# Aaron20127/human-3d-reconstruction

Hardware: AMD Instinct MI355X
Metric: images/sec whole-node, DLA-34+SMPL batch-64 512x512; top-k index bit-match (higher is better)
Workload: dtype bf16; 1 GPU; DLA-34+DCNv2 multi_pose + pose/shape heads -> sigmoid/NMS/top-100 decode -> SMPL 6890-vert LBS; 512x512, batch 64 per GPU (BASELINE configs[2]); batch_per_gpu=64, global_batch=64, K=100, smpl_people_per_image=100, parallelism=dp1 (image shards, one all-gather of dets), collective=none (one rank), steps_in_flight=3, hip_graph=False, dcn_margin=auto, images=64 distinct synthetic images (h3d_amd.synth.synth_image_batch, seed 317), weights=synthetic (h3d_amd.synth, seed 0, gain 1.25, offset_scale 0.5)

## Files before the change

human-3d-reconstruction_amd/_lib.py:

```python
import ctypes
import os

_HERE = os.path.dirname(os.path.abspath(__file__))
LIB_PATH = os.path.join(_HERE, "csrc", "libh3d_hip.so")

H3D_F32, H3D_BF16, H3D_F16, H3D_F16X3 = 0, 1, 2, 3
OP_STEM, OP_CONV, OP_DCN, OP_MAXPOOL, OP_UPADD, OP_COPY, OP_HEADS, OP_DCN_V1, OP_DCN_FUSED = 1, 2, 3, 4, 5, 6, 7, 8, 9
OP_CONV_STREAM, OP_DCN_FUSED_F16, OP_DCN_FUSED_STREAM, OP_STEM3, OP_UPDCN_F16 = 10, 11, 12, 13, 14
OP_IM2COL, OP_MAXPOOL3, OP_DEPTH2SPACE = 15, 16, 17
HEADS_MAX = 16
OUT_NHWC, OUT_NCHW_F32, OUT_NHWC_F32, OUT_NHWC_F16 = 0, 1, 2, 3
DCN_INPUT_NHWC, DCN_OUTPUT_NHWC, DCN_F32_MFMA = 1, 2, 4
ABI_VERSION = 4

DCN_AUX_BYTES = 256
DCN_FUSED_BIAS_WMAX, DCN_FUSED_BIAS_AMAX = 32, 34
OPF_DCN_MASK_FINAL, OPF_DCN_RAW_PACK, OPF_DCN_ACT_MAXIMA, TUNE_DCN_ABLATE_MASK = 0x800, 0x100000, 0x200000, 0x1f
OPF_DCN_FUSED_RAW_PACK, OPF_DCN_FUSED_SCALED_INPUT = 0x100000, 0x200000
TUNE_DCN_FUSED_X3_MARGIN2, TUNE_DCN_FUSED_X3_MARGIN6, TUNE_DCN_FUSED_X3_MARGIN4, TUNE_DCN_FUSED_X3_ABLATE_MASK = 0x2000, 0x4000, 0x8000, 0x1f
OPF_DCN_STREAM_NO_SLOTS, OPF_DCN_STREAM_WIDE_MARGIN, OPF_DCN_STREAM_SLOTS512, OPF_DCN_STREAM_F16_INPUT = 0x1000, 0x8000, 0x10000, 0x40000
OPF_DCN_STREAM_STATS, OPF_DCN_STREAM_VARIANT_MASK = 0x20000, 0x58600
TUNE_DCN_STREAM_FORCE_NARROW_WG, TUNE_DCN_STREAM_FORCE_WIDE_WG = 0x200, 0x400
TUNE_DCN_STREAM_F16_DCN5, TUNE_DCN_STREAM_F16_KEEP_DCN3, TUNE_DCN_STREAM_ABLATE_MASK = 0x4000, 0x2000, 0x1f
TUNE_DCN_STREAM_X3_MARGIN2, TUNE_DCN_STREAM_X3_MARGIN3, TUNE_DCN_STREAM_X3_MARGIN4, TUNE_DCN_STREAM_X3_ABLATE_MASK = 0x4000, 0x8000, 0x10000, 0x1f
TUNE_DCN_F16_ONE_WG_PER_CU, TUNE_DCN_F16_ABLATE_MASK = 0x100, 0xff
TUNE_CONV_STREAM_TILE_MASK, TUNE_CONV_STREAM_AUTO, TUNE_CONV_STREAM_ROUND4_RULE, TUNE_CONV_STREAM_ABLATE_MASK = 0xffff, 1, 0x10000000, 0x1f0000
TUNE_CONV_TILE, TUNE_CONV_HALO_TILE, TUNE_CONV_FORCE_GEMM, TUNE_CONV_GEMM_TILE_MASK = 0x1000, 0x2000, 0x4000, 0xf00
TUNE_CONV_X3_TILED, TUNE_CONV_X3_TILE_MASK, TUNE_CONV_X3_CK16, TUNE_CONV_X3_MT2 = 0x1000, 0x1fff, 0x2000, 0x4000
TUNE_UPADD_TAPS_GLOBAL, TUNE_UPADD_TAPS_LDS = 1, 2
TUNE_HEADS_SEPARATE_BIAS, TUNE_HEADS_ABLATE_MASK = 0x200, 0xff
TUNE_HEADS_SPARSE_LDS_PATCH, TUNE_HEADS_SPARSE_WAVES4 = 0x400, 0x800


def TUNE_DCN_STREAM_DCN5_XP(xp):
    return xp << 16


def TUNE_DCN_STREAM_DCN5_XP_OF(reserved):
    return (reserved >> 16) & 0xff


def TUNE_CONV_STREAM_TILE(variant, mt, waves):
    return variant << 12 | mt << 8 | waves


def TUNE_CONV_STREAM_ABLATE(bits):
    return bits << 16


def TUNE_CONV_STREAM_ABLATE_OF(reserved):
    return (reserved & TUNE_CONV_STREAM_ABLATE_MASK) >> 16


def TUNE_CONV_1X1_TILE(mt, th):
    return TUNE_CONV_TILE | mt << 4 | th >> 3


def TUNE_CONV_1X1_TILE_MT(reserved):
    return (reserved >> 4) & 15


def TUNE_CONV_1X1_TILE_TH(reserved):
    return (reserved & 15) * 8


def TUNE_CONV_GEMM_TILE(n):
    return n << 8


def TUNE_CONV_X3_TILE(mt, waves, th):
    return TUNE_CONV_X3_TILED | mt << 8 | waves << 4 | th >> 3

c_vp, c_i, c_fp = ctypes.c_void_p, ctypes.c_int, ctypes.c_void_p


class H3dOp(ctypes.Structure):
    _fields_ = [
        ("kind", ctypes.c_int32), ("dtype", ctypes.c_int32),
        ("in_", c_vp), ("in2", c_vp), ("w", c_vp), ("bias", c_vp), ("out", c_vp),
        ("B", ctypes.c_int32), ("H", ctypes.c_int32), ("W", ctypes.c_int32),
        ("Cin", ctypes.c_int32), ("in_cs", ctypes.c_int32), ("in2_cs", ctypes.c_int32),
        ("Ho", ctypes.c_int32), ("Wo", ctypes.c_int32),
        ("Cout", ctypes.c_int32), ("out_cs", ctypes.c_int32),
        ("ksize", ctypes.c_int32), ("stride", ctypes.c_int32), ("relu", ctypes.c_int32),
        ("out_mode", ctypes.c_int32), ("wrows", ctypes.c_int32), ("reserved", ctypes.c_int32),
        ("wexp", ctypes.c_int32), ("wexp2", ctypes.c_int32),
    ]


class _HeadEntry(ctypes.Structure):
    _fields_ = [("w2", c_vp), ("b2", c_vp), ("out", c_vp), ("C", ctypes.c_int32), ("wexp2", ctypes.c_int32)]


class H3dHeadsDesc(ctypes.Structure):
    _fields_ = [("nheads", ctypes.c_int32), ("wexp", ctypes.c_int32), ("head", _HeadEntry * HEADS_MAX)]


HEADS_LISTS_MAX = 4


class H3dHeadsList(ctypes.Structure):
    _fields_ = [("inds", c_vp), ("K", ctypes.c_int32), ("head_mask", ctypes.c_uint32)]


class H3dUpdcnDesc(ctypes.Structure):
    _fields_ = [("skip", c_vp), ("w_up", c_vp), ("w_off", c_vp), ("skip_cs", ctypes.c_int32), ("reserved", ctypes.c_int32)]


TRAIN_BRIGHTNESS, TRAIN_CONTRAST, TRAIN_SATURATION = 0, 1, 2
TRAIN_INPUT_NO_COLOR_AUG = 1


class H3dTrainImage(ctypes.Structure):
    _fields_ = [("minv", ctypes.c_double * 6), ("light", ctypes.c_double * 3), ("offset", ctypes.c_int64),
                ("h", ctypes.c_int32), ("w", ctypes.c_int32), ("row_bytes", ctypes.c_int32), ("flipped", ctypes.c_int32),
                ("order", ctypes.c_int32 * 3), ("alpha", ctypes.c_float * 3), ("one_minus_alpha", ctypes.c_float * 3),
                ("reserved", ctypes.c_int32)]


SMPL_KP_MAX_K, SMPL_KP_MAX_NV = 32, 16
RENDER_NEGATE_Z, RENDER_CULL_BACK = 1, 2
RENDER_MAX_V, RENDER_MAX_SIDE = 13120, 16384
COCO_BBOX, COCO_KEYPOINTS, COCO_ROUND2 = 0, 1, 1
COCO_MAX_D, COCO_MAX_G, COCO_SCAN_CHUNK = 128, 1024, 1024
MESH_EVAL_MAX_SWEEPS = 30
CONV_BWD_RELU, CONV_BWD_MFMA_CMAX = 1, 2048
ADAM_CAPACITY, ADAM_CHUNK = 48, 2048


class H3dAdamTensor(ctypes.Structure):
    _fields_ = [("param", c_vp), ("grad", c_vp), ("exp_avg", c_vp), ("exp_avg_sq", c_vp), ("n", ctypes.c_int64),
                ("one_minus_b1", ctypes.c_float), ("b2", ctypes.c_float), ("one_minus_b2", ctypes.c_float), ("bc2_sqrt", ctypes.c_float),
                ("eps", ctypes.c_float), ("neg_step_size", ctypes.c_float), ("weight_decay", ctypes.c_float)]


SIGNATURES = {
    "h3d_dcn_v2_forward": [c_vp] * 6 + [c_i] * 14 + [c_vp],
    "h3d_dcn_v2_forward_ws": [c_vp] * 6 + [c_i] * 14 + [c_vp, ctypes.c_size_t, c_vp],
    "h3d_dcn_v2_pack_weights": [c_vp, c_vp, c_i, c_i, c_i, c_vp, c_vp],
    "h3d_dcn_v2_pack_weights_cached": [c_vp, c_vp, c_i, c_i, c_i, c_vp, c_vp, c_vp],
    "h3d_dcn_fused_pack_f32_cached": [c_vp, c_vp, c_vp, c_vp, c_i, c_i, c_vp, c_vp, c_vp, c_vp, c_vp],
    "h3d_dcn_v2_forward_packed": [c_vp] * 5 + [c_i] * 7 + [c_vp, ctypes.c_size_t, c_vp],
    "h3d_dcn_nchw_to_nhwc_scaled": [c_vp, c_vp] + [c_i] * 4 + [c_vp, c_vp],
    "h3d_dcn_v2_backward_workspace_bytes": [c_i] * 14 + [ctypes.POINTER(ctypes.c_size_t)],
    "h3d_dcn_v2_backward": [c_vp] * 11 + [c_i] * 14 + [c_vp, ctypes.c_size_t, c_vp],
    "h3d_dcn_v2_backward_general": [c_vp] * 11 + [c_i] * 14 + [c_vp, ctypes.c_size_t, c_vp],
    "h3d_dcn_offset_mask": [c_vp] * 5 + [c_i] * 11 + [c_vp],
    "h3d_dcn_v2_psroi_pooling_forward": [c_vp] * 5 + [c_i] * 7 + [ctypes.c_float] + [c_i] * 5 + [ctypes.c_float, c_vp],
    "h3d_dcn_pooling_modulated": [c_vp] * 4 + [c_i] * 5 + [ctypes.c_float] + [c_i] * 5 + [ctypes.c_float, c_vp],
    "h3d_build_flags": [],
    "h3d_dcn_fused_ck": [c_i, c_i],
    "h3d_dcn_far_samples": [ctypes.POINTER(H3dOp), c_vp, c_vp],
    "h3d_smpl_pose_heads": [c_vp, c_vp, c_vp, c_i, c_i, c_i, c_i, c_vp, c_vp, c_vp, c_vp, c_vp, c_vp, c_vp, c_vp, c_i, c_vp],
    "h3d_smpl_coef_pack": [c_vp, c_vp, c_i, c_i, c_vp, c_vp],
    "h3d_smpl_verts3": [c_vp] * 6 + [c_i] * 5 + [c_vp, c_vp],
    "h3d_smpl_verts3_exact": [c_vp] * 6 + [c_i] * 5 + [c_vp, c_vp],
    "h3d_preprocess": [c_vp, c_i, c_i, c_i, c_i, c_vp, c_vp, c_vp, c_i, c_i, c_vp, c_vp],
    "h3d_train_input_workspace_bytes": [c_i] * 4 + [ctypes.POINTER(ctypes.c_size_t)],
    "h3d_train_input": [c_vp, ctypes.c_size_t, c_vp, c_vp, c_i, c_vp, c_vp, c_i, c_i, c_i, c_vp, ctypes.c_size_t, c_vp, c_vp, c_vp],
    "h3d_run_ops": [ctypes.POINTER(H3dOp), c_i, c_vp],
    "h3d_run_ops_timed": [ctypes.POINTER(H3dOp), c_i, c_vp, c_vp],
    "h3d_op_kernel_name": [ctypes.POINTER(H3dOp), ctypes.c_char_p, c_i],
    "h3d_heads_sparse": [ctypes.POINTER(H3dOp), c_vp, c_i, c_vp],
    "h3d_heads_sparse_lists": [ctypes.POINTER(H3dOp), c_i, ctypes.POINTER(H3dHeadsList), c_vp],
    "h3d_nchw_f32_to_nhwc": [c_vp, c_vp, c_i, c_i, c_i, c_i, c_i, c_i, c_vp],
    "h3d_nhwc_to_nchw_f32": [c_vp, c_i, c_vp, c_i, c_i, c_i, c_i, c_i, c_vp],
    "h3d_nms_topk": [c_vp, c_i, c_i, c_i, c_i, c_i, c_i, c_vp, c_vp, c_vp, c_vp, c_vp],
    "h3d_nms_topk2": [c_vp, c_i, c_vp, c_vp, c_vp, c_vp, c_vp, c_i, c_vp, c_vp, c_vp, c_vp, c_i, c_i, c_i, c_i, c_i, c_vp],
    "h3d_nms_topk_large": [c_vp, c_i, c_i, c_i, c_i, c_i, c_i, c_vp, c_vp, c_vp, c_vp, c_vp, ctypes.c_size_t, c_vp],
    "h3d_nms": [c_vp, c_i, c_i, c_i, c_i, c_vp, c_vp],
    "h3d_topk_merge": [c_vp] * 4 + [c_i] * 3 + [c_vp] * 5 + [c_vp],
    "h3d_gather_feat": [c_vp, c_vp, c_i, c_i, c_i, c_i, c_i, c_vp, c_vp],
    "h3d_multi_pose_assemble": [c_vp] * 13 + [c_i] * 5 + [c_vp, c_vp],
    "h3d_ctdet_assemble": [c_vp] * 7 + [c_i] * 6 + [c_vp, c_vp],
    "h3d_multi_pose_post_process": [c_vp] * 3 + [c_i] * 5 + [c_vp, c_vp],
    "h3d_smpl_pose": [c_vp] * 5 + [c_i] + [c_vp] * 4 + [c_i, c_vp],
    "h3d_smpl_verts": [c_vp] * 8 + [c_i] * 4 + [c_vp, c_vp],
    "h3d_smpl_verts2": [c_vp] * 7 + [c_i] * 5 + [c_vp, c_vp],
    "h3d_sigmoid_clamp": [c_vp, c_vp, ctypes.c_size_t, c_vp],
    "h3d_loss_workspace_bytes": [c_vp, c_i, ctypes.POINTER(ctypes.c_size_t)],
    "h3d_loss_forward": [c_vp, c_i, c_vp, c_vp, ctypes.c_size_t, c_vp],
    "h3d_loss_backward": [c_vp, c_i, c_vp, c_vp, c_vp],
    "h3d_smpl_backward_workspace_bytes": [c_i] * 5 + [ctypes.POINTER(ctypes.c_size_t)],
    "h3d_smpl_backward": [c_vp] * 12 + [c_i] * 4 + [c_vp, c_vp, c_vp, ctypes.c_size_t, c_vp],
    "h3d_smpl_heads_backward": [c_vp] * 3 + [c_i] * 4 + [c_vp] * 10 + [c_i] * 3 + [c_vp, c_vp, c_vp, ctypes.c_size_t, c_vp],
    "h3d_smpl_kp_loss_workspace_bytes": [c_i, c_i, ctypes.POINTER(ctypes.c_size_t)],
    "h3d_smpl_kp_loss_forward": [c_vp] * 6 + [c_i] + [c_vp] * 3 + [c_i] * 7 + [c_vp] * 4 + [ctypes.c_size_t, c_vp],
    "h3d_smpl_kp_loss_backward": [c_vp] * 6 + [c_i] + [c_vp] * 7 + [c_i] * 7 + [c_vp] * 4,
    "h3d_render_workspace_bytes": [c_i] * 3 + [ctypes.POINTER(ctypes.c_size_t)],
    "h3d_render_rasterize": [c_vp] * 6 + [c_i] * 9 + [c_vp, c_vp, c_vp, ctypes.c_size_t, c_vp],
    "h3d_render_shade": [c_vp] * 5 + [c_i] * 6 + [ctypes.c_float, ctypes.c_float, c_i, c_i, c_vp, c_vp],
    "h3d_heads_backward_workspace_bytes": [c_i] * 5 + [c_vp, ctypes.POINTER(ctypes.c_size_t)],
    "h3d_heads_backward": [c_vp] + [c_i] * 6 + [c_vp, c_vp, c_vp, ctypes.c_size_t, c_vp],
    "h3d_conv2d_backward_workspace_bytes": [c_i] * 14 + [ctypes.POINTER(ctypes.c_size_t)],
    "h3d_conv2d_backward": [c_vp, c_i, c_vp, c_vp, c_i, c_vp, c_i] + [c_vp] * 4 + [c_i] * 14 + [c_vp, ctypes.c_size_t, c_vp],
    "h3d_conv2d_backward_general": [c_vp, c_i, c_vp, c_vp, c_i, c_vp, c_i] + [c_vp] * 4 + [c_i] * 14 + [c_vp, ctypes.c_size_t, c_vp],
    "h3d_targets_workspace_bytes": [c_i] * 3 + [ctypes.POINTER(ctypes.c_size_t)],
    "h3d_multi_pose_targets": [c_vp] * 8 + [c_i] * 7 + [c_vp] * 13 + [c_i, c_vp, ctypes.c_size_t, c_vp],
    "h3d_ctdet_targets": [c_vp] * 6 + [c_i] * 6 + [c_vp] * 9 + [c_i, c_vp, ctypes.c_size_t, c_vp],
    "h3d_adam_step": [ctypes.POINTER(H3dAdamTensor), c_i, c_vp],
    "h3d_coco_match_workspace_bytes": [c_i] * 3 + [ctypes.POINTER(ctypes.c_size_t)],
    "h3d_coco_match": [c_vp, c_i] + [c_vp] * 8 + [c_i] * 6 + [c_vp, c_i, c_vp, c_i] + [c_vp] * 11 + [ctypes.c_size_t, c_vp],
    "h3d_coco_accumulate_workspace_bytes": [c_i, c_i, ctypes.POINTER(ctypes.c_size_t)],
    "h3d_coco_accumulate": [c_vp] * 8 + [c_i] * 6 + [ctypes.POINTER(ctypes.c_int32), c_i, c_vp, c_i, c_vp, c_vp, c_vp, ctypes.c_size_t, c_vp],
    "h3d_pointset_errors": [c_vp, c_i, c_vp, c_i, c_i, c_vp, c_vp, c_i, c_vp, c_vp, c_vp, c_i, c_i, c_i, c_vp, c_vp, c_vp, c_vp],
    "h3d_metric_means": [c_vp, c_vp, c_i, c_vp, c_vp, c_vp],
}

_lib = None


def lib():
    global _lib
    if _lib is None:
        if not os.path.exists(LIB_PATH):
            raise RuntimeError(
                "h3d_amd: HIP library not built (%s). Run `python -c 'import __graft_entry__ as g; "
                "g.build()'` or `make -C human-3d-reconstruction_amd/csrc`. There is no CPU fallback."
                % LIB_PATH)
        import torch
        L = ctypes.CDLL(LIB_PATH)
        L.h3d_last_error.restype = ctypes.c_char_p
        L.h3d_last_error.argtypes = []
        L.h3d_abi_version.restype = c_i
        if L.h3d_abi_version() != ABI_VERSION:
            raise RuntimeError("h3d_amd: libh3d_hip.so ABI %d != binding ABI %d"
                               % (L.h3d_abi_version(), ABI_VERSION))
        for name, args in SIGNATURES.items():
            fn = getattr(L, name)
            fn.argtypes = args
            fn.restype = c_i
        L.h3d_dcn_v2_workspace_bytes.argtypes = [c_i] * 5
        L.h3d_dcn_v2_workspace_bytes.restype = ctypes.c_size_t
        L.h3d_dcn_v2_packed_weight_bytes.argtypes = [c_i] * 3
        L.h3d_dcn_v2_packed_weight_bytes.restype = ctypes.c_size_t
        L.h3d_dcn_v2_packed_workspace_bytes.argtypes = [c_i] * 5
        L.h3d_dcn_v2_packed_workspace_bytes.restype = ctypes.c_size_t
        L.h3d_nms_topk_large_workspace_bytes.argtypes = [c_i] * 5
        L.h3d_nms_topk_large_workspace_bytes.restype = ctypes.c_size_t
        _lib = L
    return _lib


def has_extra():
    return bool(lib().h3d_build_flags() & 1)


_ERR_NAMES = {-1: "shape", -2: "dtype", -3: "launch", -4: "unsupported", -5: "argument"}


def check(rc, what):
    if rc != 0:
        msg = lib().h3d_last_error().decode("utf-8", "replace")
        raise RuntimeError("%s failed (%s error): %s" % (what, _ERR_NAMES.get(rc, rc), msg))


def workspace(size_fn, *args, device, min_bytes=0, what=None):
    import torch
    n = ctypes.c_size_t(0)
    check(size_fn(*args, ctypes.byref(n)), what or size_fn.__name__)
    nbytes = max(n.value, min_bytes)
    return torch.empty(nbytes, dtype=torch.uint8, device=device) if nbytes else None


def stream_ptr():
    import torch
    return ctypes.c_void_p(torch.cuda.current_stream().cuda_stream)


def ptr(t):
    return ctypes.c_void_p(0 if t is None else t.data_ptr())


def require_cuda(*tensors):
    for t in tensors:
        if t is not None and not t.is_cuda:
            raise RuntimeError("Not implemented on the CPU")
```

human-3d-reconstruction_amd/csrc/conv.hip:

```cpp
#include "common.h"
#include "epilogue.h"

struct ConvArgs {
    const char *in;
    const char *w;
    const float *bias;
    const char *res;
    char *out;
    int B, H, W, Cin, in_cs;
    int Ho, Wo, Cout, out_cs, res_cs;
    int relu, out_mode;
    int tiles_x, tiles_y;
    float wscale;
};

template <typename T, int KS, int STRIDE, int MT, int CK, int TH, int WAVES = 4>
struct ConvCfg {
    static constexpr int TW = 16;
    static constexpr int ES = sizeof(T);
    static constexpr int PAD = KS / 2;
    static constexpr int IN_H = (TH - 1) * STRIDE + KS;
    static constexpr int IN_W = (TW - 1) * STRIDE + KS;
    static constexpr int SB = CK * ES + 16;
    static constexpr int RB = ((IN_W * SB + 255) / 256) * 256;
// ... 316 lines not shown
int h3d_launch_gemm1(const h3d_op &op, hipStream_t st);

int h3d_launch_conv(const h3d_op &op, hipStream_t st)
{
    if (!op.in || !op.w || !op.bias || !op.out) H3D_FAIL(H3D_ERR_ARG, "conv: null pointer");
    const int es = h3d_dtype_bytes(op.dtype);
    if (!es) H3D_FAIL(H3D_ERR_DTYPE, "conv: dtype %d", op.dtype);
    if (op.Cin % 16 || op.in_cs % (16 / es) || op.Cin > op.in_cs)
        H3D_FAIL(H3D_ERR_SHAPE, "conv: Cin=%d (stride %d) must be a multiple of 16", op.Cin, op.in_cs);
    const int pad = op.ksize / 2;
    const int ho = (op.H + 2 * pad - op.ksize) / op.stride + 1;
    const int wo = (op.W + 2 * pad - op.ksize) / op.stride + 1;
    if (ho != op.Ho || wo != op.Wo)
        H3D_FAIL(H3D_ERR_SHAPE, "conv: output %dx%d does not match (H+2p-k)/s+1 = %dx%d", op.Ho, op.Wo, ho, wo);
    if (op.wrows < ((op.Cout + 127) / 128) * 128)
        H3D_FAIL(H3D_ERR_SHAPE, "conv: packed weight rows %d < Cout %d padded to 128", op.wrows, op.Cout);
    if (op.out_mode != H3D_OUT_NCHW_F32 && (op.out_cs % 4 || op.Cout > op.out_cs))
        H3D_FAIL(H3D_ERR_SHAPE, "conv: out channel stride %d must be a multiple of 4 and >= Cout %d", op.out_cs, op.Cout);
    if (op.in2 && (op.in2_cs % 4)) H3D_FAIL(H3D_ERR_SHAPE, "conv: residual channel stride %d", op.in2_cs);
    ConvArgs a;
    a.in = (const char *)op.in; a.w = (const char *)op.w; a.bias = op.bias;
    a.res = (const char *)op.in2; a.out = (char *)op.out;
    a.B = op.B; a.H = op.H; a.W = op.W; a.Cin = op.Cin; a.in_cs = op.in_cs;
    a.Ho = op.Ho; a.Wo = op.Wo; a.Cout = op.Cout; a.out_cs = op.out_cs; a.res_cs = op.in2_cs;
    a.relu = op.relu; a.out_mode = op.out_mode; a.tiles_x = a.tiles_y = 0;
    if (op.wexp < -60 || op.wexp > 60 || (op.wexp && op.dtype != H3D_F16X3)) H3D_FAIL(H3D_ERR_ARG, "conv: wexp %d (an H3D_F16X3 filter exponent)", op.wexp);
    a.wscale = ldexpf(1.f, -op.wexp);
    if (h3d_gemm1_takes(op)) return h3d_launch_gemm1(op, st);
    return h3d_by_dtype<bf16_t, f16_t, float, x3_t>(op.dtype, "conv: dtype %d", [&](auto t) { return launch_conv_t<typename decltype(t)::type>(op, a, st); });
}

template <typename T>
__global__ __launch_bounds__(256) void stem_kernel(const float *__restrict__ img, const float *__restrict__ w,
                                                   const float *__restrict__ bias, T *__restrict__ out,
                                                   int B, int H, int W, int out_cs, int tiles_x, int tiles_y)
{
    constexpr int TS = 16, HS = TS + 6;
    __shared__ float s[3][HS][HS + 1];
    const int tiles = tiles_x * tiles_y;
    const int b = blockIdx.x / tiles;
    const int t = blockIdx.x - b * tiles;
    const int ty = t / tiles_x, tx = t - ty * tiles_x;
    const int oy0 = ty * TS, ox0 = tx * TS;
    for (int i = threadIdx.x; i < 3 * HS * HS; i += 256) {
        const int c = i / (HS * HS), rem = i - c * HS * HS;
        const int iy = rem / HS, ix = rem - iy * HS;
        const int gy = oy0 - 3 + iy, gx = ox0 - 3 + ix;
        float v = 0.f;
        if (gy >= 0 && gy < H && gx >= 0 && gx < W) v = img[(((size_t)b * 3 + c) * H + gy) * W + gx];
        s[c][iy][ix] = v;
    }
    __syncthreads();
    const int py = threadIdx.x >> 4, px = threadIdx.x & 15;
    float acc[16];
#pragma unroll
    for (int o = 0; o < 16; ++o) acc[o] = bias[o];
    for (int c = 0; c < 3; ++c)
        for (int dy = 0; dy < 7; ++dy)
#pragma unroll
            for (int dx = 0; dx < 7; ++dx) {
                const float x = s[c][py + dy][px + dx];
#pragma unroll
                for (int o = 0; o < 16; ++o) acc[o] = fmaf(w[((o * 3 + c) * 7 + dy) * 7 + dx], x, acc[o]);
            }
    const int oy = oy0 + py, ox = ox0 + px;
    if (oy < H && ox < W) {
        T *op = out + (((size_t)b * H + oy) * W + ox) * out_cs;
#pragma unroll
        for (int o = 0; o < 16; o += 4)
            store4<T>(op + o, fmaxf(acc[o], 0.f), fmaxf(acc[o + 1], 0.f), fmaxf(acc[o + 2], 0.f),
                      fmaxf(acc[o + 3], 0.f));
    }
}

typedef __attribute__((ext_vector_type(4))) float f32x4_t;
template <typename T>
__global__ __launch_bounds__(256) void stem_mfma_kernel(const float *__restrict__ img, const T *__restrict__ w,
                                                        const float *__restrict__ bias, T *__restrict__ out, int B,
                                                        int H, int W, int out_cs, int tiles_x, int tiles_y)
{
    constexpr int TH = 16, TW = 64, IH = TH + 6, IW = TW + 6 + 2;
    __shared__ __attribute__((aligned(16))) uint2 s[IH][IW];
    const int tid = threadIdx.x, wv = tid >> 6, l = tid & 63, p = l & 15, q = l >> 4;
    const int tiles = tiles_x * tiles_y;
    const int b = blockIdx.x / tiles;
    const int t = blockIdx.x - b * tiles;
    const int ty = t / tiles_x, tx = t - ty * tiles_x;
    const int oy0 = ty * TH, ox0 = tx * TW;
    u32x4 fa[7];
#pragma unroll
    for (int dy = 0; dy < 7; ++dy) fa[dy] = *reinterpret_cast<const u32x4 *>(w + (p * 7 + dy) * 32 + 8 * q);
    const size_t plane = (size_t)H * W;
    const float *im = img + (size_t)b * 3 * plane;
    for (int i = tid; i < IH * IW; i += 256) {
        const int iy = i / IW, ix = i - iy * IW;
        const int gy = oy0 - 3 + iy, gx = ox0 - 3 + ix;
        float c0 = 0.f, c1 = 0.f, c2 = 0.f;
        if (gy >= 0 && gy < H && gx >= 0 && gx < W) {
            const size_t o = (size_t)gy * W + gx;
            c0 = im[o]; c1 = im[plane + o]; c2 = im[2 * plane + o];
        }
        s[iy][ix] = uint2{EP<T>::pack2(c0, c1), EP<T>::pack2(c2, 0.f)};
    }
    __syncthreads();
    float bs[4];
#pragma unroll
    for (int i = 0; i < 4; ++i) bs[i] = bias[4 * q + i];
#pragma unroll 1
    for (int g = 0; g < 16; ++g) {
        const int py = wv * 4 + (g >> 2), px0 = (g & 3) * 16;
        f32x4_t acc = {0.f, 0.f, 0.f, 0.f};
#pragma unroll
        for (int dy = 0; dy < 7; ++dy) {
            const uint2 lo = s[py + dy][px0 + p + 2 * q], hi = s[py + dy][px0 + p + 2 * q + 1];
            const u32x4 fb = {lo.x, lo.y, hi.x, hi.y};
            if constexpr (std::is_same_v<T, f16_t>)
                acc = __builtin_amdgcn_mfma_f32_16x16x32_f16(__builtin_bit_cast(f16x8_t, fa[dy]), __builtin_bit_cast(f16x8_t, fb), acc, 0, 0, 0);
            else
                acc = __builtin_amdgcn_mfma_f32_16x16x32_bf16(__builtin_bit_cast(bf16x8_t, fa[dy]), __builtin_bit_cast(bf16x8_t, fb), acc, 0, 0, 0);
        }
        const int oy = oy0 + py, ox = ox0 + px0 + p;
        if (oy < H && ox < W)
            store4<T>(out + ((size_t)(b * H + oy) * W + ox) * out_cs + 4 * q, fmaxf(acc[0] + bs[0], 0.f),
                           fmaxf(acc[1] + bs[1], 0.f), fmaxf(acc[2] + bs[2], 0.f), fmaxf(acc[3] + bs[3], 0.f));
    }
}

__global__ __launch_bounds__(256) void stem_x3_kernel(const float *__restrict__ img, const char *__restrict__ w, const float *__restrict__ bias,
                                                      float *__restrict__ out, int B, int H, int W, int out_cs, int tiles_x, int tiles_y, float wscale)
{
    constexpr int TH = 16, TW = 64, IH = TH + 6, IW = TW + 6 + 2;
    __shared__ __attribute__((aligned(16))) uint2 s_hi[IH][IW], s_lo[IH][IW];
    const int tid = threadIdx.x, wv = tid >> 6, l = tid & 63, p = l & 15, q = l >> 4;
    const int tiles = tiles_x * tiles_y;
    const int b = blockIdx.x / tiles;
    const int t = blockIdx.x - b * tiles;
    const int ty = t / tiles_x, tx = t - ty * tiles_x;
    const int oy0 = ty * TH, ox0 = tx * TW;
    u32x4 fah[7], fal[7];
#pragma unroll
    for (int dy = 0; dy < 7; ++dy) {
        const char *g = w + ((size_t)(p * 7 + dy) * 32 + 8 * q) * 4;
        fah[dy] = *reinterpret_cast<const u32x4 *>(g);
        fal[dy] = *reinterpret_cast<const u32x4 *>(g + 16);
    }
    const size_t plane = (size_t)H * W;
    const float *im = img + (size_t)b * 3 * plane;
    for (int i = tid; i < IH * IW; i += 256) {
        const int iy = i / IW, ix = i - iy * IW;
        const int gy = oy0 - 3 + iy, gx = ox0 - 3 + ix;
        u32x4 raw = {0u, 0u, 0u, 0u};
        if (gy >= 0 && gy < H && gx >= 0 && gx < W) {
            const size_t o = (size_t)gy * W + gx;
            raw = u32x4{__float_as_uint(im[o]), __float_as_uint(im[plane + o]), __float_as_uint(im[2 * plane + o]), 0u};
        }
        u32x2 hi, lo;
        x3_split4(raw, hi, lo);
        s_hi[iy][ix] = uint2{hi[0], hi[1]};
        s_lo[iy][ix] = uint2{lo[0], lo[1]};
    }
    __syncthreads();
    float bs[4];
#pragma unroll
    for (int i = 0; i < 4; ++i) bs[i] = bias[4 * q + i];
#pragma unroll 1
    for (int g = 0; g < 16; ++g) {
        const int py = wv * 4 + (g >> 2), px0 = (g & 3) * 16;
        f32x4_t acc = {0.f, 0.f, 0.f, 0.f};
#pragma unroll
        for (int dy = 0; dy < 7; ++dy) {
            const uint2 h0 = s_hi[py + dy][px0 + p + 2 * q], h1 = s_hi[py + dy][px0 + p + 2 * q + 1];
            const uint2 l0 = s_lo[py + dy][px0 + p + 2 * q], l1 = s_lo[py + dy][px0 + p + 2 * q + 1];
            const u32x4 fbh = {h0.x, h0.y, h1.x, h1.y}, fbl = {l0.x, l0.y, l1.x, l1.y};
            acc = __builtin_amdgcn_mfma_f32_16x16x32_f16(__builtin_bit_cast(f16x8_t, fal[dy]), __builtin_bit_cast(f16x8_t, fbh), acc, 0, 0, 0);
            acc = __builtin_amdgcn_mfma_f32_16x16x32_f16(__builtin_bit_cast(f16x8_t, fah[dy]), __builtin_bit_cast(f16x8_t, fbl), acc, 0, 0, 0);
            acc = __builtin_amdgcn_mfma_f32_16x16x32_f16(__builtin_bit_cast(f16x8_t, fah[dy]), __builtin_bit_cast(f16x8_t, fbh), acc, 0, 0, 0);
        }
        const int oy = oy0 + py, ox = ox0 + px0 + p;
        if (oy < H && ox < W)
            store4<float>(out + ((size_t)(b * H + oy) * W + ox) * out_cs + 4 * q, fmaxf(fmaf(acc[0], wscale, bs[0]), 0.f), fmaxf(fmaf(acc[1], wscale, bs[1]), 0.f),
                          fmaxf(fmaf(acc[2], wscale, bs[2]), 0.f), fmaxf(fmaf(acc[3], wscale, bs[3]), 0.f));
    }
}

int h3d_launch_stem_s2(const h3d_op &op, hipStream_t st);

int h3d_launch_stem(const h3d_op &op, hipStream_t st)
{
    if (!op.in || !op.w || !op.bias || !op.out) H3D_FAIL(H3D_ERR_ARG, "stem: null pointer");
    if (op.stride == 2) return h3d_launch_stem_s2(op, st);
    if (op.Cin != 3 || op.Cout != 16 || op.ksize != 7 || op.Ho != op.H || op.Wo != op.W || op.out_cs % 4)
        H3D_FAIL(H3D_ERR_SHAPE, "stem: expects 7x7 3->16 stride 1 (got k=%d %d->%d)", op.ksize, op.Cin, op.Cout);
    const int tx = cdiv(op.W, 16), ty = cdiv(op.H, 16);
    dim3 grid(op.B * tx * ty);
    if (op.dtype == H3D_BF16 || op.dtype == H3D_F16) {
        const int mx = cdiv(op.W, 64), my = cdiv(op.H, 16);
        return h3d_by_dtype<bf16_t, f16_t>(op.dtype, "stem: dtype %d", [&](auto t) {
            using T = typename decltype(t)::type;
            return h3d_launch({"stem_mfma_kernel", t}, stem_mfma_kernel<T>, dim3(op.B * mx * my), dim3(256), 0, st, (const float *)op.in, (const T *)op.w,
                              op.bias, (T *)op.out, op.B, op.H, op.W, op.out_cs, mx, my);
        });
    }
    if (op.dtype == H3D_F16X3) {
        if (op.wexp < -60 || op.wexp > 60) H3D_FAIL(H3D_ERR_ARG, "stem: wexp %d", op.wexp);
        const int mx = cdiv(op.W, 64), my = cdiv(op.H, 16);
        return h3d_launch({"stem_x3_kernel"}, stem_x3_kernel, dim3(op.B * mx * my), dim3(256), 0, st, (const float *)op.in, (const char *)op.w, op.bias, (float *)op.out,
                          op.B, op.H, op.W, op.out_cs, mx, my, ldexpf(1.f, -op.wexp));
    }
    if (op.dtype != H3D_F32 && h3d_kname{"stem_kernel", h3d_tag<float>{}}.dry()) return H3D_OK;
    return h3d_by_dtype<bf16_t, float>(op.dtype, "stem: dtype %d", [&](auto t) {
        using T = typename decltype(t)::type;
        return h3d_launch({"stem_kernel", t}, stem_kernel<T>, grid, dim3(256), 0, st, (const float *)op.in, (const float *)op.w, op.bias, (T *)op.out, op.B, op.H,
                          op.W, op.out_cs, tx, ty);
    });
}

template <typename T> struct Vec16 { static constexpr int N = 16 / sizeof(T); };

template <typename T>
__global__ void maxpool_kernel(const T *__restrict__ in, T *__restrict__ out, int B, int H, int W, int C,
                               int in_cs, int Ho, int Wo, int out_cs)
{
    constexpr int N = Vec16<T>::N;
    const int vpc = C / N;
    const size_t total = (size_t)B * Ho * Wo * vpc;
    for (size_t i = (size_t)blockIdx.x * blockDim.x + threadIdx.x; i < total; i += (size_t)gridDim.x * blockDim.x) {
        const int v = i % vpc;
        const size_t p = i / vpc;
        const int ox = p % Wo;
        const size_t q = p / Wo;
        const int oy = q % Ho, b = q / Ho;
        float m[N], x[N];
        const T *base = in + (((size_t)b * H + oy * 2) * W + ox * 2) * in_cs + v * N;
        unpack16<T>(*reinterpret_cast<const u32x4 *>(base), m);
        unpack16<T>(*reinterpret_cast<const u32x4 *>(base + in_cs), x);
#pragma unroll
        for (int k = 0; k < N; ++k) m[k] = fmaxf(m[k], x[k]);
        unpack16<T>(*reinterpret_cast<const u32x4 *>(base + (size_t)W * in_cs), x);
#pragma unroll
        for (int k = 0; k < N; ++k) m[k] = fmaxf(m[k], x[k]);
        unpack16<T>(*reinterpret_cast<const u32x4 *>(base + (size_t)W * in_cs + in_cs), x);
#pragma unroll
        for (int k = 0; k < N; ++k) m[k] = fmaxf(m[k], x[k]);
        *reinterpret_cast<u32x4 *>(out + p * out_cs + v * N) = pack16<T>(m);
    }
}

constexpr int UP_ROWS = 8;
template <typename T, bool F16OUT = false, bool WLDS = true>
__global__ __launch_bounds__(256) void upadd_kernel(const T *__restrict__ in, const T *__restrict__ skip,
                                                    const float *__restrict__ w, T *__restrict__ out, int B, int H, int W,
                                                    int C, int in_cs, int skip_cs, int Ho, int Wo, int out_cs, int f)
{
    constexpr int N = Vec16<T>::N;
    extern __shared__ __attribute__((aligned(16))) float s_w[];
    const int vpc = C / N, k = 2 * f, p = f / 2;
    const int wrow = WLDS ? C + 4 : C;
    if constexpr (WLDS) {
        const int c4 = C / 4;
        for (int i = threadIdx.x; i < k * k * c4; i += 256) {
            const int t = i / c4, j = i - t * c4;
            *reinterpret_cast<f32x4 *>(s_w + t * wrow + 4 * j) = *reinterpret_cast<const f32x4 *>(w + 4 * i);
        }
        __syncthreads();
    }
    const int ppb = 256 / vpc;
    const int v = threadIdx.x % vpc, pxl = threadIdx.x / vpc;
    const int ox = blockIdx.x * ppb + pxl;
    const int rows_per_img = (Ho + UP_ROWS - 1) / UP_ROWS;
    const int b = blockIdx.y / rows_per_img, oy0 = (blockIdx.y - b * rows_per_img) * UP_ROWS;
    if (pxl >= ppb || ox >= Wo) return;
    const int rx = (ox + p) % f;
    int ixs[2], kjs[2];
    bool xok[2];
#pragma unroll
    for (int c2 = 0; c2 < 2; ++c2) {
        kjs[c2] = rx + c2 * f;
        const int num = ox + p - kjs[c2];
        ixs[c2] = num / f;
        xok[c2] = num >= 0 && ixs[c2] < W;
    }
    for (int oy = oy0; oy < min(oy0 + UP_ROWS, Ho); ++oy) {
        const size_t pix = ((size_t)b * Ho + oy) * Wo + ox;
        const int ry = (oy + p) % f;
        u32x4 xv[4], sv;
        bool ok[4];
        int tap[4];
#pragma unroll
        for (int a = 0; a < 2; ++a) {
            const int ki = ry + a * f;
            const int num = oy + p - ki;
            const int iy = num / f;
            const bool yok = num >= 0 && iy < H;
#pragma unroll
            for (int c2 = 0; c2 < 2; ++c2) {
                const int q = a * 2 + c2;
                ok[q] = yok && xok[c2];
                tap[q] = ki * k + kjs[c2];
                xv[q] = u32x4{0u, 0u, 0u, 0u};
                if (ok[q]) xv[q] = *reinterpret_cast<const u32x4 *>(in + (((size_t)b * H + iy) * W + ixs[c2]) * in_cs + v * N);
            }
        }
        sv = *reinterpret_cast<const u32x4 *>(skip + pix * skip_cs + v * N);
        float acc[N], x[N];
#pragma unroll
        for (int n = 0; n < N; ++n) acc[n] = 0.f;
#pragma unroll
        for (int q = 0; q < 4; ++q) {
            if (!ok[q]) continue;
            unpack16<T>(xv[q], x);
            const float *wp;
            if constexpr (WLDS) wp = s_w + tap[q] * wrow + v * N;
            else wp = w + tap[q] * C + v * N;
#pragma unroll
            for (int n = 0; n < N; ++n) acc[n] = fmaf(wp[n], x[n], acc[n]);
        }
        unpack16<T>(sv, x);
#pragma unroll
        for (int n = 0; n < N; ++n) acc[n] += x[n];
        if constexpr (F16OUT) *reinterpret_cast<u32x4 *>(out + pix * out_cs + v * N) = pack16_f16(acc);
        else *reinterpret_cast<u32x4 *>(out + pix * out_cs + v * N) = pack16<T>(acc);
    }
}

template <typename T>
__global__ void copy_kernel(const T *__restrict__ in, T *__restrict__ out, size_t npix, int C, int in_cs, int out_cs)
{
    constexpr int N = Vec16<T>::N;
    const int vpc = C / N;
    const size_t total = npix * vpc;
    for (size_t i = (size_t)blockIdx.x * blockDim.x + threadIdx.x; i < total; i += (size_t)gridDim.x * blockDim.x) {
        const int v = i % vpc;
        const size_t p = i / vpc;
        *reinterpret_cast<u32x4 *>(out + p * out_cs + v * N) = *reinterpret_cast<const u32x4 *>(in + p * in_cs + v * N);
    }
}

static inline int ew_grid(size_t total) { size_t g = (total + 255) / 256; return (int)(g > 2048 * 8 ? 2048 * 8 : (g ? g : 1)); }

int h3d_launch_elementwise(const h3d_op &op, hipStream_t st)
{
    if (!op.in || !op.out) H3D_FAIL(H3D_ERR_ARG, "elementwise: null pointer");
    const int es = h3d_dtype_bytes(op.dtype);
    if (!es) H3D_FAIL(H3D_ERR_DTYPE, "elementwise: dtype %d", op.dtype);
    const int n = 16 / es;
    if (op.Cin % n || op.in_cs % n || op.out_cs % n || op.Cin != op.Cout)
        H3D_FAIL(H3D_ERR_SHAPE, "elementwise: channels %d/%d strides %d/%d must be multiples of %d", op.Cin, op.Cout,
                 op.in_cs, op.out_cs, n);
    const size_t total = (size_t)op.B * op.Ho * op.Wo * (op.Cin / n);
    dim3 grid(ew_grid(total)), blk(256);
    const bool f16out = op.kind == H3D_OP_UPADD && op.out_mode == H3D_OUT_NHWC_F16;
    if (f16out && op.dtype != H3D_BF16) H3D_FAIL(H3D_ERR_DTYPE, "upadd: fp16 output is an option of bf16 plans (fp16 plans write fp16 anyway)");
    const size_t up_wbytes = (size_t)op.ksize * op.ksize * op.Cin * sizeof(float);
    const bool up_wlds = op.reserved == H3D_TUNE_UPADD_TAPS_GLOBAL ? false : op.reserved == H3D_TUNE_UPADD_TAPS_LDS ? up_wbytes <= 64 * 1024 : (up_wbytes <= 8192 || (up_wbytes <= 16384 && op.Cin <= 64));
    return h3d_by_store_dtype<bf16_t, f16_t, float, x3_t>(op.dtype, "elementwise: dtype %d", [&](auto t) {
        using T = typename decltype(t)::type;
        const T *in = (const T *)op.in;
        T *out = (T *)op.out;
        if (op.kind == H3D_OP_MAXPOOL) {
            const auto k = h3d_bind({"maxpool_kernel", t}, maxpool_kernel<T>);
            if (k.name.dry()) return H3D_OK;
            if (op.Ho != op.H / 2 || op.Wo != op.W / 2) H3D_FAIL(H3D_ERR_SHAPE, "maxpool: output must be floor(H/2) x floor(W/2)");
            return k.launch(grid, blk, 0, st, in, out, op.B, op.H, op.W, op.Cin, op.in_cs, op.Ho, op.Wo, op.out_cs);
        }
        if (op.kind != H3D_OP_UPADD) {
            const auto k = h3d_bind({"copy_kernel", t}, copy_kernel<T>);
            if (k.name.dry()) return H3D_OK;
            if (op.Ho != op.H || op.Wo != op.W) H3D_FAIL(H3D_ERR_SHAPE, "copy: shape");
            return k.launch(grid, blk, 0, st, in, out, (size_t)op.B * op.H * op.W, op.Cin, op.in_cs, op.out_cs);
        }
        return h3d_by_values([&](auto f16o, auto wlds) {
            const auto k = h3d_bind({"upadd_kernel", t, f16o, wlds},
                                    upadd_kernel<T, f16o, wlds>);
            if (k.name.dry()) return H3D_OK;
            const int f = op.stride;
            if (!op.in2 || !op.w) H3D_FAIL(H3D_ERR_ARG, "upadd: null pointer");
            if (op.ksize != 2 * f || op.Ho != op.H * f || op.Wo != op.W * f || op.in2_cs % n)
                H3D_FAIL(H3D_ERR_SHAPE, "upadd: expects k=2f, out = f*in (k=%d f=%d)", op.ksize, f);
            const int vpc = op.Cin / n;
            if (vpc > 256) H3D_FAIL(H3D_ERR_UNSUPPORTED, "upadd: C=%d", op.Cin);
            const size_t wfl = (size_t)op.ksize * op.ksize * op.Cin;
            const size_t lds = wlds ? (wfl + 4 * (size_t)op.ksize * op.ksize) * sizeof(float) : 0;
            const dim3 ugrid(cdiv(op.Wo, 256 / vpc), op.B * cdiv(op.Ho, UP_ROWS));
            return k.launch(ugrid, blk, lds, st, in, (const T *)op.in2, (const float *)op.w, out, op.B, op.H, op.W, op.Cin, op.in_cs, op.in2_cs, op.Ho, op.Wo,
                            op.out_cs, f);
        }, std::conditional_t<std::is_same_v<T, bf16_t>, h3d_vals<false, true>, h3d_vals<false>>{}, f16out, h3d_vals<false, true>{}, up_wlds);
    });
}

template <typename T>
__global__ void nchw_to_nhwc_kernel(const float *__restrict__ src, T *__restrict__ dst, int B, int C, int HW, int dst_cs)
{
    __shared__ float tile[32][33];
    const int b = blockIdx.z, p0 = blockIdx.x * 32, c0 = blockIdx.y * 32;
    const int tx = threadIdx.x & 31, ty = threadIdx.x >> 5;
    for (int k = ty; k < 32; k += 8) {
        const int c = c0 + k, p = p0 + tx;
        tile[k][tx] = (c < C && p < HW) ? src[((size_t)b * C + c) * HW + p] : 0.f;
    }
    __syncthreads();
    for (int k = ty; k < 32; k += 8) {
        const int p = p0 + k, c = c0 + tx;
        if (p < HW && c < C) dst[((size_t)b * HW + p) * dst_cs + c] = ET<T>::from_f32(tile[tx][k]);
    }
}
template <typename T>
__global__ void nhwc_to_nchw_kernel(const T *__restrict__ src, float *__restrict__ dst, int B, int C, int HW, int src_cs)
{
    __shared__ float tile[32][33];
    const int b = blockIdx.z, p0 = blockIdx.x * 32, c0 = blockIdx.y * 32;
    const int tx = threadIdx.x & 31, ty = threadIdx.x >> 5;
    for (int k = ty; k < 32; k += 8) {
        const int p = p0 + k, c = c0 + tx;
        tile[k][tx] = (p < HW && c < C) ? ET<T>::to_f32(src[((size_t)b * HW + p) * src_cs + c]) : 0.f;
    }
    __syncthreads();
    for (int k = ty; k < 32; k += 8) {
        const int c = c0 + k, p = p0 + tx;
        if (c < C && p < HW) dst[((size_t)b * C + c) * HW + p] = tile[tx][k];
    }
}

extern "C" int h3d_nchw_f32_to_nhwc(const float *src, void *dst, int dtype, int B, int C, int H, int W, int dst_cs,
                                    void *stream)
{
    if (!src || !dst) H3D_FAIL(H3D_ERR_ARG, "nchw_to_nhwc: null pointer");
    if (B <= 0 || C <= 0 || H <= 0 || W <= 0 || dst_cs < C) H3D_FAIL(H3D_ERR_SHAPE, "nchw_to_nhwc: bad shape");
    dim3 grid(cdiv(H * W, 32), cdiv(C, 32), B);
    return h3d_by_dtype<bf16_t, f16_t, float>(dtype, "nchw_to_nhwc: dtype %d", [&](auto t) {
        using T = typename decltype(t)::type;
        return h3d_launch({"nchw_to_nhwc_kernel", t}, nchw_to_nhwc_kernel<T>, grid, dim3(256), 0, (hipStream_t)stream, src, (T *)dst, B, C, H * W, dst_cs);
    });
}

extern "C" int h3d_nhwc_to_nchw_f32(const void *src, int dtype, float *dst, int B, int C, int H, int W, int src_cs,
                                    void *stream)
{
    if (!src || !dst) H3D_FAIL(H3D_ERR_ARG, "nhwc_to_nchw: null pointer");
    if (B <= 0 || C <= 0 || H <= 0 || W <= 0 || src_cs < C) H3D_FAIL(H3D_ERR_SHAPE, "nhwc_to_nchw: bad shape");
    dim3 grid(cdiv(H * W, 32), cdiv(C, 32), B);
    return h3d_by_dtype<bf16_t, f16_t, float>(dtype, "nhwc_to_nchw: dtype %d", [&](auto t) {
        using T = typename decltype(t)::type;
        return h3d_launch({"nhwc_to_nchw_kernel", t}, nhwc_to_nchw_kernel<T>, grid, dim3(256), 0, (hipStream_t)stream, (const T *)src, dst, B, C, H * W, src_cs);
    });
}
```

human-3d-reconstruction_amd/csrc/dcn3.hip:

```cpp
#include "common.h"
#include "epilogue.h"
#include "dcn_tile.h"

struct Dcn3Args {
    const char *in;
    const char *w;
    const char *woff;
    const float *bias;
    char *out;
    int B, H, W, Cin, in_cs;
    int Cout, out_cs, relu, out_mode, wrows;
    int tiles_x, tiles_y;
    int dbg;
    int G;
    float wscale, oscale;
    const unsigned *wmax;
    int xscaled;
    int xcd;
    unsigned long long *stamps;
};

#if defined(H3D_ABLATE) && defined(DCN3_STAMP_B)
#undef H3D_STAMP
#define H3D_STAMP(wg, k) do { if ((k) == 6 && threadIdx.x == 0 && (wg) < 65536 && a.stamps) a.stamps[(wg) * H3D_NSTAMP + 6] = __builtin_readcyclecounter(); } while (0)
#define H3D_STAMP_B(s, k) do { if ((s) == nchunks + 1 && threadIdx.x == 0 && blockIdx.x < 65536 && a.stamps) a.stamps[blockIdx.x * H3D_NSTAMP + (k)] = __builtin_readcyclecounter(); } while (0)
#else
#define H3D_STAMP_B(s, k) do { } while (0)
#endif

template <typename T, int MT, int CK, int MARGIN, bool WDMA = false, int NP = 0, bool PK = false>
struct Dcn3Cfg {
    static constexpr int ES = sizeof(T);
    static constexpr int SS = SE<T>::SS;
    static constexpr int HH = 16 + 2 + 2 * MARGIN;
    static constexpr int SBH = PK ? CK * SS : CK * SS + 16;
    static constexpr int RBH = PK ? HH * SBH : ((HH * SBH + 255) / 256) * 256;
    static_assert(!PK || (CK == 16 && SS == 2 && WDMA && NP > 0 && (RBH / 16) % 2 == 0 && (RBH & 16) == 0), "packed apron: fp16 samples, 16-channel stages");
    static constexpr int WB = 9 * CK * SS + 16;
    static constexpr int BN = 32 * MT;
    static constexpr int THREADS = 512;
    static constexpr int VPP = CK * SS / 16;
    static constexpr int LDS_H = HH * RBH;
    static constexpr int WGRP = 32 * WB;
    static constexpr int WPIECES = (MT * WGRP + 1023) / 1024;
    static constexpr int OPIECES = (WGRP + 1023) / 1024;
    static constexpr int WSLOT = WDMA ? WPIECES * 1024 : BN * WB;
    static constexpr int PSLOT = CK * SS;
    static constexpr int PB = NP ? (NP * PSLOT + 255) / 256 * 256 : 0;
    static constexpr int STAGE = PB + LDS_H + WSLOT;
    static constexpr bool SINGLE = !WDMA && SS == 4 && MARGIN > 2;
    static constexpr int LDS_MAIN = WDMA ? PB + LDS_H + 2 * WSLOT : SINGLE ? STAGE : 2 * STAGE;
    static constexpr int DESC_B = SS == 4 ? 32 : 16;
    static constexpr int LDS_DESC = NP ? NP * DESC_B + 32 : 0;
    static constexpr int LDS_EPI = 8 * ((32 * (64 * MT + 16) + 1023) / 1024 * 1024);
    static constexpr int LDS = LDS_MAIN + LDS_DESC > LDS_EPI ? LDS_MAIN + LDS_DESC : LDS_EPI;
    static_assert(NP == 0 || (WDMA && (sizeof(T) == 2 || std::is_same_v<T, x3_t>)), "patches: plans with DMA'd filters (bf16 / fp16 / f16x3)");
    static_assert(NP * (CK * SS / 16) <= 1024, "at most two 16-byte patch units per thread (the second one in a second fill round)");
};


template <typename T, int MT, int CK, int MARGIN, int EPI = 0, bool WDMA = false, int NP = 0, bool PK = false, bool F16IN = false, bool STATS = false>
__global__ __launch_bounds__(512, (WDMA && MT <= 2 && sizeof(T) == 2) ? 4 : 2) void dcn3_kernel(Dcn3Args a)
{
    using C = Dcn3Cfg<T, MT, CK, MARGIN, WDMA, NP, PK>;
    using X = SE<std::conditional_t<F16IN, f16_t, T>>;
    static_assert(!F16IN || (std::is_same<T, bf16_t>::value && WDMA && NP > 0), "fp16 input: an option of the bf16 patch-slot variants");
    constexpr int ES = C::ES, SS = C::SS;
    constexpr bool ONEBUF = WDMA || C::SINGLE;
    __shared__ __attribute__((aligned(256))) char smem[C::LDS];
    char *s_w = smem + C::PB + C::LDS_H;

    const int tid = threadIdx.x;
    const int wv = tid >> 6, l = tid & 63, r = l & 31, h = l >> 5;
    const int tiles = a.tiles_x * a.tiles_y;
    const int bid = h3d_tile_id(blockIdx.x, gridDim.x, a.xcd);
    const int b = bid / tiles;
    const int t = bid - b * tiles;
    const int ty = t / a.tiles_x, tx = t - ty * a.tiles_x;
    const int oy0 = ty * 16, ox0 = tx * 16;
    const int hy0 = oy0 - 1 - MARGIN, hx0 = ox0 - 1 - MARGIN;
    const int cout0 = blockIdx.y * C::BN;
    const int py = wv * 2 + (r >> 4), px = r & 15;
    const int oy = oy0 + py, ox = ox0 + px;
    const bool live = (oy < a.H && ox < a.W);
    const char *img = a.in + (size_t)b * a.H * a.W * a.in_cs * ES;
    const int aoff = r * C::WB + 8 * h * SS;
    const int nchunks = a.Cin / CK;
    [[maybe_unused]] float wsc[2] = {1.f, 1.f}, wun = a.wscale, oun = a.oscale;
    [[maybe_unused]] bool rawf = false;
    if constexpr (std::is_same_v<T, x3_t> && !WDMA) {
        rawf = a.wmax != nullptr;
        if (rawf) {
#pragma unroll
            for (int q = 0; q < 2; ++q) {
                const float m = __uint_as_float(a.wmax[q]);
                int k = 14;
                if (m > 0.f && m < __builtin_inff()) (void)frexpf(m, &k);
                const int e = min(60, max(-60, 14 - k));
                wsc[q] = ldexpf(1.f, e);
                (q ? oun : wun) = ldexpf(1.f, -e);
            }
            if (a.xscaled) {
                const float xun = ldexpf(1.f, -dcn_act_exp(a.wmax[2], 0u));
                wun *= xun;
                oun *= xun;
            }
        }
    }
    [[maybe_unused]] const bool xraw = std::is_same_v<T, x3_t> && !WDMA && a.xscaled;
    [[maybe_unused]] auto corner_mem = [&](const char *p) {
        typename X::frag f = X::global8(p);
        if constexpr (std::is_same_v<T, x3_t>) {
            if (!xraw) {
                f.lo = __builtin_bit_cast(f32x4, X::convert16(__builtin_bit_cast(u32x4, f.lo)));
                f.hi = __builtin_bit_cast(f32x4, X::convert16(__builtin_bit_cast(u32x4, f.hi)));
            }
        }
        return f;
    };
    [[maybe_unused]] auto store_w = [&](char *dst_row_tap, int v, u32x4 raw, int which) {
        if constexpr (std::is_same_v<T, x3_t> && !WDMA) {
            if (rawf) {
#pragma unroll
                for (int i = 0; i < 4; ++i) raw[i] = __float_as_uint(__uint_as_float(raw[i]) * wsc[which]);
                x3_store4(dst_row_tap + (v >> 1) * 32, v & 1, raw);
                return;
            }
        }
        *reinterpret_cast<u32x4 *>(dst_row_tap + v * 16) = raw;
    };
    const int wvu = __builtin_amdgcn_readfirstlane(wv);
    const int off_bytes = nchunks * C::WGRP, main_bytes = nchunks * a.G * C::WGRP;
    auto issue_w = [&](int s) {
        if constexpr (WDMA) {
            char *dst = s_w + (s & 1) * C::WSLOT;
            if (s < nchunks) dcn_lds_dma<C::OPIECES>(a.woff, off_bytes, dst, s * C::WGRP, l * 16, wvu);
            else dcn_lds_dma<C::WPIECES>(a.w, main_bytes, dst, ((s - nchunks) * a.G + (int)blockIdx.y * MT) * C::WGRP, l * 16, wvu);
        }
    };

    constexpr int WV = 9 * C::VPP;
    constexpr int NH = C::HH * C::HH * C::VPP, NW = WDMA ? 0 : C::BN * WV;
    constexpr int NV = (NH + NW + C::THREADS - 1) / C::THREADS;
    u32x4 stg[NV];
    auto load_stage = [&](int s) {
        if ((H3D_DBG(a) & 8) && s > 0) return;
        const bool phaseA = s < nchunks;
        const int c0 = (phaseA ? s : s - nchunks) * CK;
        const char *wsrc = phaseA ? a.woff : a.w;
        const int wr0 = phaseA ? 0 : cout0;
        const int nrows = phaseA ? 32 : C::BN;
#pragma unroll
        for (int j = 0; j < NV; ++j) {
            const int i = tid + j * C::THREADS;
            u32x4 val = {0u, 0u, 0u, 0u};
            if (i < NH) {
                const int v = i % C::VPP, pix = i / C::VPP;
                const int iy = pix / C::HH, ix = pix - iy * C::HH;
                const int gy = hy0 + iy, gx = hx0 + ix;
                if (gy >= 0 && gy < a.H && gx >= 0 && gx < a.W)
                    val = *reinterpret_cast<const u32x4 *>(img + ((size_t)(gy * a.W + gx) * a.in_cs + c0) * ES + v * 16);
            } else if (i < NH + NW) {
                const int q0 = i - NH;
                const int row = q0 / WV, q = q0 - row * WV;
                const int tap = q / C::VPP, v = q - tap * C::VPP;
                if (row < nrows)
                    val = *reinterpret_cast<const u32x4 *>(wsrc + (((size_t)(wr0 + row) * 9 + tap) * a.Cin + c0) * SS + v * 16);
            }
            stg[j] = val;
        }
    };
    auto store_stage = [&](int s) {
        if ((H3D_DBG(a) & 8) && s > 0) return;
        char *s_h = smem + C::PB + (ONEBUF ? 0 : (s & 1) * C::STAGE);
        char *s_w = s_h + C::LDS_H;
#pragma unroll
        for (int j = 0; j < NV; ++j) {
            const int i = tid + j * C::THREADS;
            if (i < NH) {
                const int v = i % C::VPP, pix = i / C::VPP;
                const int iy = pix / C::HH, ix = pix - iy * C::HH;
                if constexpr (X::SPLIT_A) {
                    if (s < nchunks) {
                        if (xraw) x3_store4<false>(s_h + iy * C::RBH + ix * C::SBH + (v >> 1) * 32, v & 1, stg[j]);
                        else x3_store4(s_h + iy * C::RBH + ix * C::SBH + (v >> 1) * 32, v & 1, stg[j]);
                        continue;
                    }
                }
                *reinterpret_cast<u32x4 *>(s_h + iy * C::RBH + ix * C::SBH + ((PK ? (v ^ (iy & 1)) : v) * 16)) = xraw ? stg[j] : X::convert16(stg[j]);
            } else if (i < NH + NW) {
                const int q0 = i - NH;
                const int row = q0 / WV, q = q0 - row * WV;
                const int tap = q / C::VPP, v = q - tap * C::VPP;
                store_w(s_w + row * C::WB + tap * CK * SS, v, stg[j], s < nchunks ? 1 : 0);
            }
        }
    };

    constexpr bool D2 = WDMA && NP > 0;
#ifndef DCN3_TAPAHEAD
#define DCN3_TAPAHEAD 1
#endif
    constexpr bool TAPAHEAD = DCN3_TAPAHEAD && D2 && MT >= 4 && CK == 16;
    [[maybe_unused]] int avoff[NV], adst[NV];
    [[maybe_unused]] u32x4 stg2[D2 ? 2 : 1][NV];
    if constexpr (D2) {
#pragma unroll
        for (int j = 0; j < NV; ++j) {
            const int i = tid + j * C::THREADS;
            const int v = i % C::VPP, pix = i / C::VPP;
            const int iy = pix / C::HH, ix = pix - iy * C::HH;
            const int gy = hy0 + iy, gx = hx0 + ix;
            avoff[j] = (i < NH && gy >= 0 && gy < a.H && gx >= 0 && gx < a.W) ? ((gy * a.W + gx) * a.in_cs) * ES + v * 16 : 0x7ffffff0;
            adst[j] = i < NH ? iy * C::RBH + ix * C::SBH + ((PK ? (v ^ (iy & 1)) : v) * 16) : -1;
        }
    }
    [[maybe_unused]] const int img_bytes = (int)((size_t)a.H * a.W * a.in_cs * ES);
    auto load2 = [&](int s, auto P) {
        if constexpr (D2) {
            constexpr int q = decltype(P)::value;
            const int c0 = (s < nchunks ? s : s - nchunks) * CK;
#pragma unroll
            for (int j = 0; j < NV; ++j) stg2[q][j] = dcn_corner16(img, img_bytes, avoff[j], c0 * ES);
        }
    };
    auto store2 = [&](auto P, auto PHASE_A) {
        if constexpr (D2) {
            constexpr int q = decltype(P)::value;
#pragma unroll
            for (int j = 0; j < NV; ++j) {
                if constexpr (X::SPLIT_A && decltype(PHASE_A)::value) {
                    if (adst[j] >= 0) x3_store4(smem + C::PB + adst[j] - (tid & 1) * 16, tid & 1, stg2[q][j]);
                } else {
                    if (adst[j] >= 0) *reinterpret_cast<u32x4 *>(smem + C::PB + adst[j]) = X::convert16(stg2[q][j]);
                }
            }
        }
    };
    [[maybe_unused]] constexpr std::integral_constant<int, 0> I0{};
    [[maybe_unused]] constexpr std::integral_constant<int, 1> I1{};
    [[maybe_unused]] constexpr int WAIT_NV = 0x0f70 | (NV & 15) | ((NV >> 4) << 14);

    H3D_STAMP(blockIdx.x, 6);
    if constexpr (NP > 0) {
        for (int i = tid * 16; i < C::PB + C::LDS_H; i += C::THREADS * 16) *reinterpret_cast<u32x4 *>(smem + i) = u32x4{0u, 0u, 0u, 0u};
        __syncthreads();
    }
    H3D_STAMP(blockIdx.x, 0);
    f32x16 aoffs;
#pragma unroll
    for (int i = 0; i < 16; ++i) aoffs[i] = 0.f;
    const int bconv = PK ? (MARGIN + py) * C::RBH + (MARGIN + px) * C::SBH + ((h ^ ((MARGIN + py) & 1)) << 4)
                         : (MARGIN + py) * C::RBH + (MARGIN + px) * C::SBH + 8 * h * SS;
    [[maybe_unused]] const int bconv1 = (bconv ^ 16) + C::RBH;
    auto computeA = [&](int s) {
        const char *s_h = smem + C::PB + (ONEBUF ? 0 : (s & 1) * C::STAGE);
        const char *s_w = s_h + C::LDS_H + (WDMA ? (s & 1) * C::WSLOT : 0);
#pragma unroll
        for (int tap = 0; tap < 9; ++tap) {
            const int dy = tap / 3, dx = tap - dy * 3;
#pragma unroll
            for (int kk = 0; kk < CK / 16; ++kk) {
                const typename X::wfrag fa = X::lds_w(s_w + aoff + (tap * CK + kk * 16) * SS);
                const typename X::bfrag fb = X::lds_a(s_h + ((PK && dy == 1) ? bconv1 : bconv + dy * C::RBH) + dx * C::SBH + kk * 16 * SS);
                if (H3D_DBG(a) & 1) { X::keep(fa); X::keep(fb); } else X::mma(aoffs, fa, fb);
            }
        }
#ifndef DCN3_ADEPTH
#define DCN3_ADEPTH 4
#endif
        if constexpr (DCN3_ADEPTH > 0 && CK == 16 && sizeof(T) == 2) {
            constexpr int RPT = 2, MPT = 1;
            __builtin_amdgcn_sched_group_barrier(0x100, RPT * DCN3_ADEPTH, 0);
#pragma unroll
            for (int tap = 0; tap < 9; ++tap) {
                __builtin_amdgcn_sched_group_barrier(0x008, MPT, 0);
                if (tap + DCN3_ADEPTH < 9) __builtin_amdgcn_sched_group_barrier(0x100, RPT, 0);
            }
        }
    };
    if constexpr (D2) {
        issue_w(0);
        load2(0, I0);
        load2(1, I1);
        auto stepA = [&](int s, auto P) {
            if (s) __syncthreads();
            store2(P, std::true_type{});
            __builtin_amdgcn_s_waitcnt(WAIT_NV);
            __syncthreads();
            issue_w(s + 1);
            load2(s + 2, P);
            computeA(s);
        };
        for (int s = 0; s < nchunks; s += 2) { stepA(s, I0); stepA(s + 1, I1); }
    } else {
    issue_w(0);
    load_stage(0);
    for (int s = 0; s < nchunks; ++s) {
        if (ONEBUF && s) __syncthreads();
        store_stage(s);
        if constexpr (WDMA) __builtin_amdgcn_s_waitcnt(0x0f70);
        __syncthreads();
        issue_w(s + 1);
        load_stage(s + 1);
        computeA(s);
    }
    }
    {
        const float *bo = a.bias + a.wrows;
        if constexpr (std::is_same_v<T, x3_t>) {
#pragma unroll
            for (int i = 0; i < 16; ++i) aoffs[i] = fmaf(aoffs[i], oun, bo[(i & 3) + 8 * (i >> 2) + 4 * h]);
        } else {
#pragma unroll
            for (int i = 0; i < 16; ++i) aoffs[i] += bo[(i & 3) + 8 * (i >> 2) + 4 * h];
        }
    }

    H3D_STAMP(blockIdx.x, 1);
    int boff[9];
    typename X::geo geo[9];
    bool slow = false;
    [[maybe_unused]] int pmask = 0;
    {
        int my_off[5];
        typename X::geo my_geo[5];
        bool my_want[5];
        uint32_t my_hw[5];
        int my_pm = 0;
#pragma unroll
        for (int u = 0; u < 5; ++u) {
            const int ti = h ? (5 + u) / 3 : u / 3, tj = h ? (5 + u) % 3 : u % 3;
            const float h_im = (float)(oy - 1 + ti) + aoffs[3 * u];
            const float w_im = (float)(ox - 1 + tj) + aoffs[3 * u + 1];
            const bool inside = live & (u < 4 || h == 0) & (h_im > -1.f) & (w_im > -1.f) & (h_im < (float)a.H) & (w_im < (float)a.W);
            const float fh = floorf(h_im), fw = floorf(w_im);
            const int hl = (int)fh, wl = (int)fw;
            const int ry = hl - hy0, rx = wl - hx0;
            float w4[4];
            dcn_bilinear_w(h_im, w_im, fh, fw, w4);
            const float w4g[4] = {inside ? w4[0] : 0.f, inside ? w4[1] : 0.f, inside ? w4[2] : 0.f, inside ? w4[3] : 0.f};
            typename X::geo g = X::make_geo(w4g, dcn2_sigmoid(aoffs[3 * u + 2]));
            const bool inap = (unsigned)ry < (unsigned)(C::HH - 1) && (unsigned)rx < (unsigned)(C::HH - 1);
            const int ry0 = py + ti + MARGIN, rx0 = px + tj + MARGIN;
            const int off = (inside && inap) ? ry * C::RBH + rx * C::SBH + (PK ? ((ry & 1) << 4) : 0)
                                             : ry0 * C::RBH + rx0 * C::SBH + (PK ? ((ry0 & 1) << 4) : 0);
            const bool want = inside && !inap;
            my_want[u] = want;
            my_hw[u] = ((uint32_t)hl << 16) | ((uint32_t)wl & 0xffffu);
            my_off[u] = off;
            my_geo[u] = g;
        }
        if constexpr (NP > 0) {
            unsigned long long m[5];
            int cnt = 0;
#pragma unroll
            for (int u = 0; u < 5; ++u) { m[u] = __ballot(my_want[u]); cnt += __popcll(m[u]); }
            int *s_cnt = reinterpret_cast<int *>(smem + C::LDS_MAIN + NP * C::DESC_B);
            if (l == 0) s_cnt[wv] = cnt;
            __syncthreads();
            int base = 0;
#pragma unroll
            for (int w8 = 0; w8 < 8; ++w8) base += (w8 < wv) ? s_cnt[w8] : 0;
            if (cnt) {
#pragma unroll
                for (int u = 0; u < 5; ++u) {
                    const int slot = base + (int)__builtin_amdgcn_mbcnt_hi((unsigned)(m[u] >> 32), __builtin_amdgcn_mbcnt_lo((unsigned)m[u], 0u));
                    base += __popcll(m[u]);
                    if (my_want[u] && slot < NP) {
// ... 150 lines not shown
                const int voff = base2 + ((k & 1) + (k >> 1) * a.W) * a.in_cs * ES;
                v[k].v = __builtin_bit_cast(half8_t, X::convert16(dcn_corner16(img, img_bytes, ok ? voff : 0x7ffffff0, c0 * ES)));
            }
            const typename X::frag o = X::blend(v, g2);
            *reinterpret_cast<half8_t *>(s_h - C::PB + (R * C::VPP + tid) * 16) = o.v;
        }
    };

    auto tail = [&](auto P2) {
    H3D_STAMP(blockIdx.x, 2);
    f32x16 acc[MT][1];
#pragma unroll
    for (int m = 0; m < MT; ++m)
#pragma unroll
        for (int i = 0; i < 16; ++i) acc[m][0][i] = 0.f;
    auto computeB = [&](int s) {
        const char *s_h = smem + C::PB + (ONEBUF ? 0 : (s & 1) * C::STAGE);
        const char *s_w = s_h + C::LDS_H + (WDMA ? (s & 1) * C::WSLOT : 0);
#ifndef DCN3_X3_PIPE
#define DCN3_X3_PIPE 1
#endif
        if constexpr (DCN3_X3_PIPE && std::is_same_v<T, x3_t> && CK == 16 && WDMA) {
            typename X::frag v[4];
            typename X::bfrag pb[2];
            auto gather = [&](int tap) {
                const char *p00 = s_h + boff[tap], *p10 = p00 + C::RBH;
                v[0] = X::lds(p00);
                v[1] = X::lds(p00 + C::SBH);
                v[2] = X::lds(p10);
                v[3] = X::lds(p10 + C::SBH);
            };
            gather(0);
            {
                const typename X::frag fb = X::blend(v, geo[0]);
                __builtin_amdgcn_sched_barrier(0);
                gather(1);
                pb[0] = X::prep(fb);
            }
            __builtin_amdgcn_sched_barrier(0);
#pragma unroll
            for (int tap = 0; tap < 9; ++tap) {
                typename X::wfrag fa[MT];
#pragma unroll
                for (int m = 0; m < MT; ++m) fa[m] = X::lds_w(s_w + aoff + m * 32 * C::WB + tap * CK * SS);
                if (tap + 1 < 9) {
                    const typename X::frag fb = X::blend(v, geo[tap + 1]);
                    if (tap + 2 < 9) gather(tap + 2);
                    pb[(tap + 1) & 1] = X::prep(fb);
                }
#pragma unroll
                for (int m = 0; m < MT; ++m) X::mma(acc[m][0], fa[m], pb[tap & 1]);
                __builtin_amdgcn_sched_group_barrier(0x100, 2 * MT, 0);
                if (tap + 1 < 9) {
#pragma unroll
                    for (int i = 0; i < 3 * MT; ++i) {
                        __builtin_amdgcn_sched_group_barrier(0x008, 1, 0);
                        if (i == 3 * MT - 1) __builtin_amdgcn_sched_group_barrier(0x002, 24, 0);
                        else __builtin_amdgcn_sched_group_barrier(0x002, 36 / (3 * MT - 1) + 1, 0);
                        if (i == (MT > 1 ? 2 : 1) && tap + 2 < 9) __builtin_amdgcn_sched_group_barrier(0x100, 8, 0);
                    }
                } else {
                    __builtin_amdgcn_sched_group_barrier(0x008, 3 * MT, 0);
                }
            }
            return;
        }
        if constexpr (TAPAHEAD) {
            static_assert(CK == 16, "one 16-channel fragment per tap");
            typename X::frag v[2][4];
            auto gather = [&](int tap, int q) {
                const char *p00 = s_h + boff[tap];
                const char *p10 = PK ? s_h + ((boff[tap] ^ 16) + C::RBH) : p00 + C::RBH;
                v[q][0] = X::lds(p00);
                v[q][1] = X::lds(p00 + C::SBH);
                v[q][2] = X::lds(p10);
                v[q][3] = X::lds(p10 + C::SBH);
            };
            gather(0, 0);
#pragma unroll
            for (int tap = 0; tap < 9; ++tap) {
                typename X::wfrag fa[MT];
#pragma unroll
                for (int m = 0; m < MT; ++m) fa[m] = X::lds_w(s_w + aoff + m * 32 * C::WB + tap * CK * SS);
                if (tap + 1 < 9) gather(tap + 1, (tap + 1) & 1);
                __builtin_amdgcn_sched_barrier(0);
                const typename X::frag fb = X::blend(v[tap & 1], geo[tap]);
#pragma unroll
                for (int m = 0; m < MT; ++m) X::mma(acc[m][0], fa[m], fb);
            }
            return;
        }
#pragma unroll
        for (int tap = 0; tap < 9; ++tap) {
            typename X::frag fb[CK / 16];
            const char *p00 = s_h + boff[tap];
            const char *p10 = PK ? s_h + ((boff[tap] ^ 16) + C::RBH) : p00 + C::RBH;
#pragma unroll
            for (int kk = 0; kk < CK / 16; ++kk) {
                if (H3D_DBG(a) & 2) { fb[kk] = X::lds(p00 + kk * 16 * SS); continue; }
                typename X::frag v[4];
                v[0] = X::lds(p00 + kk * 16 * SS);
                v[1] = X::lds(p00 + C::SBH + kk * 16 * SS);
                v[2] = X::lds(p10 + kk * 16 * SS);
                v[3] = X::lds(p10 + C::SBH + kk * 16 * SS);
                fb[kk] = X::blend(v, geo[tap]);
            }
#pragma unroll
            for (int kk = 0; kk < CK / 16; ++kk) {
                typename X::wfrag fa[MT];
#pragma unroll
                for (int m = 0; m < MT; ++m) fa[m] = X::lds_w(s_w + aoff + m * 32 * C::WB + (tap * CK + kk * 16) * SS);
                if (H3D_DBG(a) & 4) {
#pragma unroll
                    for (int m = 0; m < MT; ++m) { X::keep(fa[m]); X::keep(fb[kk]); }
                    continue;
                }
                const typename X::bfrag pb = X::prep(fb[kk]);
#pragma unroll
                for (int m = 0; m < MT; ++m) X::mma(acc[m][0], fa[m], pb);
            }
        }
    };
    if constexpr (D2) {
        auto stepB = [&](int s, auto P, auto Q) {
            H3D_STAMP_B(s, 0);
            patch_issue(s);
            __syncthreads();
            H3D_STAMP_B(s, 1);
            store2(P, std::false_type{});
            patch_commit(smem + C::PB);
            patch_round2(s, smem + C::PB);
            __builtin_amdgcn_s_waitcnt(0x0f70);
            H3D_STAMP_B(s, 2);
            __syncthreads();
            H3D_STAMP_B(s, 3);
            if (s + 1 < 2 * nchunks) {
                issue_w(s + 1);
                if (s != nchunks) load2(s + 1, Q);
            }
            H3D_STAMP_B(s, 4);
            computeB(s);
            H3D_STAMP_B(s, 5);
        };
        for (int s = nchunks; s < 2 * nchunks; s += 2) { stepB(s, I0, I1); stepB(s + 1, I1, I0); }
    } else {
    for (int s = nchunks; s < 2 * nchunks; ++s) {
        patch_issue(s);
        if (ONEBUF) __syncthreads();
        store_stage(s);
        patch_commit(smem + C::PB + (ONEBUF ? 0 : (s & 1) * C::STAGE));
        if constexpr (WDMA) __builtin_amdgcn_s_waitcnt(0x0f70);
        __syncthreads();
        if (s + 1 < 2 * nchunks) { issue_w(s + 1); load_stage(s + 1); }
        computeB(s);
    }
    }

    H3D_STAMP(blockIdx.x, 3);
    bool do_p2 = false;
    if constexpr (decltype(P2)::value) do_p2 = NP > 0 ? overflow : (bool)__syncthreads_or(slow ? 1 : 0);
    if constexpr (decltype(P2)::value) if (do_p2) {
        if constexpr (D2 && MT < 4) {
#pragma unroll
            for (int i = 0; i < 16; ++i) aoffs[i] = 0.f;
            for (int s = 0; s < nchunks; ++s) {
                __syncthreads();
                issue_w(s);
                load2(s, I0);
                store2(I0, std::true_type{});
                __builtin_amdgcn_s_waitcnt(0x0f70);
                __syncthreads();
                computeA(s);
            }
            const float *bo = a.bias + a.wrows;
            if constexpr (std::is_same_v<T, x3_t>) {
#pragma unroll
                for (int i = 0; i < 16; ++i) aoffs[i] = fmaf(aoffs[i], oun, bo[(i & 3) + 8 * (i >> 2) + 4 * h]);
            } else {
#pragma unroll
                for (int i = 0; i < 16; ++i) aoffs[i] += bo[(i & 3) + 8 * (i >> 2) + 4 * h];
            }
        }
        if constexpr (D2) {
            constexpr int TB = SS == 4 ? 1 : 3;
            constexpr int CV = SS == 4 ? 2 : 1;
            int qb[9], qok[9], wmask = 0;
            typename X::geo qg[9];
#pragma unroll
            for (int tap = 0; tap < 9; ++tap) {
                const int ti = tap / 3, tj = tap - ti * 3;
                const DcnTapOffset d = dcn_tap_offset(aoffs, tap, r);
                const float h_im = (float)(oy - 1 + ti) + d.d_h, w_im = (float)(ox - 1 + tj) + d.d_w;
                qb[tap] = 0; qok[tap] = 0; qg[tap] = X::zero_geo();
                bool pend = false;
                if (live && h_im > -1.f && w_im > -1.f && h_im < (float)a.H && w_im < (float)a.W) {
                    const int hl = (int)floorf(h_im), wl = (int)floorf(w_im);
                    const int ry = hl - hy0, rx = wl - hx0;
                    if (!(ry >= 0 && ry + 1 < C::HH && rx >= 0 && rx + 1 < C::HH) && !((pmask >> tap) & 1)) {
                        pend = true;
                        const DcnFar fs = dcn_far(h_im, w_im, hl, wl, a.H, a.W);
                        qg[tap] = X::make_geo(fs.w, dcn2_sigmoid(d.d_m));
                        qb[tap] = ((hl * a.W + wl) * a.in_cs + 8 * h) * ES;
                        qok[tap] = fs.ok;
                    }
                }
                if (__any(pend)) wmask |= 1 << tap;
            }
            const int pxb = a.in_cs * ES, rowb = a.W * pxb;
            u32x4 pv[TB][4][CV];
            for (int c0 = 0; c0 < a.Cin; c0 += CK) {
                auto fetch = [&](int t0) {
#pragma unroll
                    for (int j = 0; j < TB; ++j) {
                        if (!((wmask >> (t0 + j)) & 1)) continue;
#pragma unroll
                        for (int k = 0; k < 4; ++k)
#pragma unroll
                            for (int cv = 0; cv < CV; ++cv)
                                pv[j][k][cv] = dcn_corner16(img, img_bytes, ((qok[t0 + j] >> k) & 1) ? qb[t0 + j] + (k & 1) * pxb + (k >> 1) * rowb + cv * 16 : 0x7ffffff0, c0 * ES);
                    }
                };
                __syncthreads();
                dcn_lds_dma<C::WPIECES>(a.w, main_bytes, s_w, ((c0 / CK) * a.G + (int)blockIdx.y * MT) * C::WGRP, l * 16, wvu);
                fetch(0);
                __builtin_amdgcn_s_waitcnt(0x0f70);
                __syncthreads();
#pragma unroll
                for (int t0 = 0; t0 < 9; t0 += TB) {
                    typename X::bfrag fbs[TB];
#pragma unroll
                    for (int j = 0; j < TB; ++j) {
                        if (!((wmask >> (t0 + j)) & 1)) continue;
                        typename X::frag v[4];
                        if constexpr (SS == 4) {
#pragma unroll
                            for (int k = 0; k < 4; ++k) { v[k].lo = __builtin_bit_cast(f32x4, X::convert16(pv[j][k][0])); v[k].hi = __builtin_bit_cast(f32x4, X::convert16(pv[j][k][CV - 1])); }
                        } else {
#pragma unroll
                            for (int k = 0; k < 4; ++k) v[k].v = __builtin_bit_cast(half8_t, X::convert16(pv[j][k][0]));
                        }
                        fbs[j] = X::prep(X::blend(v, qg[t0 + j]));
                    }
                    if (t0 + TB < 9) fetch(t0 + TB);
#pragma unroll
                    for (int j = 0; j < TB; ++j) {
                        if (!((wmask >> (t0 + j)) & 1)) continue;
                        typename X::wfrag fa[MT];
#pragma unroll
                        for (int m = 0; m < MT; ++m) fa[m] = X::lds_w(s_w + aoff + m * 32 * C::WB + ((t0 + j) * CK) * SS);
#pragma unroll
                        for (int m = 0; m < MT; ++m) X::mma(acc[m][0], fa[m], fbs[j]);
                    }
                }
            }
        } else
        for (int c0 = 0; c0 < a.Cin; c0 += CK) {
            __syncthreads();
            if constexpr (WDMA) {
                dcn_lds_dma<C::WPIECES>(a.w, main_bytes, s_w, ((c0 / CK) * a.G + (int)blockIdx.y * MT) * C::WGRP, l * 16, wvu);
                __builtin_amdgcn_s_waitcnt(0x0f70);
            } else {
                for (int i = tid; i < C::BN * WV; i += C::THREADS) {
                    const int row = i / WV, q = i - row * WV;
                    const int tap = q / C::VPP, v = q - tap * C::VPP;
                    store_w(s_w + row * C::WB + tap * CK * SS, v, *reinterpret_cast<const u32x4 *>(
                        a.w + (((size_t)(cout0 + row) * 9 + tap) * a.Cin + c0) * SS + v * 16), 0);
                }
            }
            __syncthreads();
#pragma unroll
            for (int tap = 0; tap < 9; ++tap) {
                const int ti = tap / 3, tj = tap - ti * 3;
                const DcnTapOffset d = dcn_tap_offset(aoffs, tap, r);
                typename X::frag fb[CK / 16];
#pragma unroll
                for (int kk = 0; kk < CK / 16; ++kk) fb[kk] = X::zero();
                const bool any = dcn_far_gather<X, C::HH>(fb, live && !((pmask >> tap) & 1), (float)(oy - 1 + ti) + d.d_h, (float)(ox - 1 + tj) + d.d_w, hy0, hx0, a.H, a.W,
                    [&] { return dcn2_sigmoid(d.d_m); },
                    [&](int kk, int y, int x) { return corner_mem(img + ((size_t)(y * a.W + x) * a.in_cs + c0 + kk * 16 + 8 * h) * ES); });
                if (!__any(any)) continue;
#pragma unroll
                for (int kk = 0; kk < CK / 16; ++kk) {
                    typename X::wfrag fa[MT];
#pragma unroll
                    for (int m = 0; m < MT; ++m) fa[m] = X::lds_w(s_w + aoff + m * 32 * C::WB + (tap * CK + kk * 16) * SS);
                    const typename X::bfrag pb = X::prep(fb[kk]);
#pragma unroll
                    for (int m = 0; m < MT; ++m) X::mma(acc[m][0], fa[m], pb);
                }
            }
        }
    }

    H3D_STAMP(blockIdx.x, 4);
    if constexpr (std::is_same_v<T, x3_t>) {
#pragma unroll
        for (int m = 0; m < MT; ++m)
#pragma unroll
            for (int i = 0; i < 16; ++i) acc[m][0][i] *= wun;
    }
    const EpiArgs e = dcn_epi_args(a);
    if constexpr (EPI == 2) {
        __syncthreads();
        tile_epilogue_lds<T, MT>(acc, e, b, oy0, ox0, cout0, wv, l, smem + wv * epi_lds_stride<MT>());
    } else {
        tile_epilogue<typename StoreT<T>::type, MT, 1, EPI == 1>(acc, e, b, oy0, ox0, cout0, wv, r, h);
    }
    };
    if constexpr (NP > 0 && MT >= 4) {
        if (overflow) tail(std::true_type{});
        else tail(std::false_type{});
    } else {
        tail(std::true_type{});
    }
    H3D_STAMP(blockIdx.x, 5);
}

template <typename T, int MT, int CK, int MARGIN, bool WDMA = false, int NP = 0, bool PK = false, bool F16IN = false>
static int launch_dcn3_cfg(const Dcn3Args &a0, hipStream_t st, bool stats = false)
{
    using C = Dcn3Cfg<T, MT, CK, MARGIN, WDMA, NP, PK>;
    static_assert(!(WDMA && MT <= 2 && sizeof(T) == 2) || C::LDS * 2 <= 160 * 1024, "two workgroups per CU");
    static_assert(C::LDS <= 160 * 1024, "LDS budget");
    Dcn3Args a = a0;
    a.tiles_x = cdiv(a.W, 16);
    a.tiles_y = cdiv(a.H, 16);
    a.xcd = h3d_xcd_mode();
#ifdef H3D_ABLATE
    a.stamps = h3d_stamp_buffer();
#else
    a.stamps = nullptr;
#endif
    dim3 grid(a.B * a.tiles_x * a.tiles_y, cdiv(a.Cout, C::BN));
    return dcn_by_epi<sizeof(T) == 2 && MT >= 2>(a, [&](auto e) {
        const h3d_kname name{"dcn3_kernel", h3d_tag<T>{}, MT, CK, MARGIN, e, WDMA, NP, h3d_opt(PK), h3d_opt(F16IN)};
        if constexpr (NP > 0 && sizeof(T) == 2) {
            if (stats) {
                if (name.dry()) return H3D_OK;
                return h3d_bind({"dcn3_kernel<stats>"}, dcn3_kernel<T, MT, CK, MARGIN, 1, WDMA, NP, PK, F16IN, true>).launch(dim3(grid.x), dim3(C::THREADS), 0, st, a);
            }
        }
        if constexpr (F16IN && e != 2) {
            if (name.dry()) return H3D_OK;
            H3D_FAIL(H3D_ERR_UNSUPPORTED, "dcn_fused_stream with an fp16 input: needs an NHWC output with Cout %% 8 == 0 (Cout=%d)", a.Cout);
        } else {
            return h3d_launch(name, dcn3_kernel<T, MT, CK, MARGIN, e, WDMA, NP, PK, F16IN>, grid, dim3(C::THREADS), 0, st, a);
        }
    });
}

extern "C" int h3d_dcn_fused_ck(int Cin, int Cout) { (void)Cin; (void)Cout; return 16; }

struct Dcn3Flags {
    bool no_slots, wide_margin, slots512;
    bool f16_input;
    bool narrow_wg;
    bool stats;
    bool dcn5;
    int margin;
    bool raw_pack, scaled_input;
};
static Dcn3Flags dcn3_decode(const h3d_op &op, bool wdma)
{
    const int r = op.reserved;
    Dcn3Flags f = {};
    if (op.dtype == H3D_BF16 || op.dtype == H3D_F16) {
        f.no_slots = r & H3D_OPF_DCN_STREAM_NO_SLOTS;
        f.wide_margin = r & H3D_OPF_DCN_STREAM_WIDE_MARGIN;
        f.slots512 = r & H3D_OPF_DCN_STREAM_SLOTS512;
        f.f16_input = op.dtype == H3D_BF16 && (r & H3D_OPF_DCN_STREAM_F16_INPUT);
        f.narrow_wg = h3d_dcn_narrow_wg(op);
        f.stats = r & H3D_OPF_DCN_STREAM_STATS;
        f.dcn5 = op.dtype == H3D_F16 && wdma && (r & H3D_TUNE_DCN_STREAM_F16_DCN5) && !f.no_slots && !(r & H3D_TUNE_DCN_STREAM_F16_KEEP_DCN3);
    } else if (op.dtype == H3D_F16X3 && wdma) {
        f.margin = (r & H3D_TUNE_DCN_STREAM_X3_MARGIN2) ? 2 : (r & H3D_TUNE_DCN_STREAM_X3_MARGIN3) ? 3 : (r & H3D_TUNE_DCN_STREAM_X3_MARGIN4) ? 4 : 0;
    } else if (op.dtype == H3D_F16X3) {
        f.margin = (r & H3D_TUNE_DCN_FUSED_X3_MARGIN2) ? 2 : (r & H3D_TUNE_DCN_FUSED_X3_MARGIN4) ? 4 : (r & H3D_TUNE_DCN_FUSED_X3_MARGIN6) ? 6 : 0;
        f.raw_pack = r & H3D_OPF_DCN_FUSED_RAW_PACK;
        f.scaled_input = r & H3D_OPF_DCN_FUSED_SCALED_INPUT;
    }
    return f;
}

template <typename T, bool F16IN = false>
static int launch_dcn3_lowp(const h3d_op &op, const Dcn3Flags &f, const Dcn3Args &a, bool wdma, hipStream_t st)
{
    if constexpr (F16IN) {
        if (!wdma || f.no_slots || op.Cin % 32 || op.Cout <= 32)
            H3D_FAIL(H3D_ERR_UNSUPPORTED, "dcn_fused_stream: the fp16-input option (H3D_OPF_DCN_STREAM_F16_INPUT) exists for the patch-slot variants with > 32 output channels");
    }
    if (wdma) {
        if (f.no_slots || op.Cin % 32) {
            return dcn_by_mt(op.Cout, op.Cout <= 64, [&](auto mt) { return launch_dcn3_cfg<T, decltype(mt)::value, 16, decltype(mt)::value == 4 ? 2 : 1, true>(a, st); });
        }
        const bool mt2 = op.Cout <= 64 || f.narrow_wg;
        if (f.wide_margin)
            return dcn_by_mt(op.Cout, mt2, [&](auto mt) {
                constexpr int MT = decltype(mt)::value;
                return launch_dcn3_cfg<T, MT, 16, 4, true, 256, MT < 4, MT >= 2 && F16IN>(a, st, f.stats);
            });
        if (f.slots512)
            return dcn_by_mt(op.Cout, mt2, [&](auto mt) {
                constexpr int MT = decltype(mt)::value;
                return launch_dcn3_cfg<T, MT, 16, MT < 4 ? 2 : 4, true, 512, MT < 4, MT >= 2 && F16IN>(a, st, f.stats);
            });
        return dcn_by_mt(op.Cout, mt2, [&](auto mt) {
            constexpr int MT = decltype(mt)::value;
            return launch_dcn3_cfg<T, MT, 16, MT < 4 ? 2 : 4, true, 256, false, MT >= 2 && F16IN>(a, st, f.stats);
        });
    }
    const bool mt2 = op.Cout <= 64 || f.narrow_wg;
    if (op.Cin % 32 == 0 && mt2) return dcn_by_mt<2>(op.Cout, true, [&](auto mt) { return launch_dcn3_cfg<T, decltype(mt)::value, 32, 2>(a, st); });
    return dcn_by_mt(op.Cout, mt2, [&](auto mt) { return launch_dcn3_cfg<T, decltype(mt)::value, 16, 2>(a, st); });
}

int h3d_launch_dcn5(const h3d_op &op, hipStream_t st);

int h3d_launch_dcn3(const h3d_op &op, hipStream_t st)
{
    const bool wdma = op.kind == H3D_OP_DCN_FUSED_STREAM;
    if (wdma && op.dtype != H3D_BF16 && op.dtype != H3D_F16 && op.dtype != H3D_F16X3) H3D_FAIL(H3D_ERR_DTYPE, "dcn_fused_stream: bf16 / fp16 / f16x3 plans only");
    const int es = h3d_dtype_bytes(op.dtype);
    if (const int rc = dcn_check_op(op, "dcn_fused", es, false)) return rc;
    Dcn3Args a;
    dcn_fill_args(op, a);
    a.w = (const char *)op.w; a.woff = (const char *)op.in2; a.Cin = op.Cin; a.wrows = op.wrows;
    a.dbg = op.reserved & H3D_TUNE_DCN_STREAM_ABLATE_MASK;
    a.G = op.wrows / 32;
    if (op.wexp < -60 || op.wexp > 60 || op.wexp2 < -60 || op.wexp2 > 60 || ((op.wexp || op.wexp2) && op.dtype != H3D_F16X3))
        H3D_FAIL(H3D_ERR_ARG, "dcn_fused: wexp %d / %d (H3D_F16X3 filter exponents)", op.wexp, op.wexp2);
    a.wscale = ldexpf(1.f, -op.wexp);
    a.oscale = ldexpf(1.f, -op.wexp2);
    a.wmax = nullptr;
    a.xscaled = 0;
    if (wdma && (size_t)op.H * op.W * op.in_cs * es >= 0x7ffffff0ull) H3D_FAIL(H3D_ERR_SHAPE, "dcn_fused_stream: image of 2 GiB or more");
    const Dcn3Flags f = dcn3_decode(op, wdma);
    if (f.f16_input) return launch_dcn3_lowp<bf16_t, true>(op, f, a, wdma, st);
    if (f.dcn5) {
#ifdef H3D_EXTRA
        return h3d_launch_dcn5(op, st);
#else
        H3D_FAIL(H3D_ERR_UNSUPPORTED, "dcn_fused_stream: the LDS-DMA apron variant (csrc/dcn5.hip, H3D_TUNE_DCN_STREAM_F16_DCN5) is built only by `make EXTRA=1`");
#endif
    }
    if (op.dtype == H3D_F32) {
        return dcn_by_mt<2>(op.Cout, true, [&](auto mt) { return launch_dcn3_cfg<float, decltype(mt)::value, 16, 2>(a, st); });
    }
    if (op.dtype == H3D_F16X3 && wdma) {
        if (op.Cin % 32) H3D_FAIL(H3D_ERR_UNSUPPORTED, "dcn_fused_stream (f16x3): Cin %d must be a multiple of 32 (two stages per pipeline turn); use H3D_OP_DCN_FUSED", op.Cin);
        const int margin = f.margin ? f.margin : (op.Cin == op.Cout && op.Cout > 64) ? 4 : 2;
        auto go = [&](auto m) { return dcn_by_mt<2>(op.Cout, true, [&](auto mt) { return launch_dcn3_cfg<x3_t, decltype(mt)::value, 16, decltype(m)::value, true, 256>(a, st); }); };
        if (margin == 4) return go(std::integral_constant<int, 4>{});
        if (margin == 3) return go(std::integral_constant<int, 3>{});
        return go(std::integral_constant<int, 2>{});
    }
    if (op.dtype == H3D_F16X3) {
        if (f.raw_pack) {
            if (op.wexp || op.wexp2) H3D_FAIL(H3D_ERR_ARG, "dcn_fused (f16x3, raw filters): wexp must be 0 (the scale comes from the pack's maxima)");
            a.wmax = (const unsigned *)(op.bias + op.wrows + H3D_DCN_FUSED_BIAS_WMAX);
            a.xscaled = f.scaled_input;
        }
        const int margin = f.margin ? f.margin : (op.Cout <= 64 && op.H >= 64) ? 6 : 4;
        auto go = [&](auto m) { return dcn_by_mt<2>(op.Cout, true, [&](auto mt) { return launch_dcn3_cfg<x3_t, decltype(mt)::value, 16, decltype(m)::value>(a, st); }); };
        if (margin == 2) return go(std::integral_constant<int, 2>{});
        if (margin == 6) return go(std::integral_constant<int, 6>{});
        return go(std::integral_constant<int, 4>{});
    }
    return h3d_by_dtype<bf16_t, f16_t>(op.dtype, "dcn_fused: dtype %d", [&](auto t) { return launch_dcn3_lowp<typename decltype(t)::type>(op, f, a, wdma, st); });
}

extern "C" int h3d_dcn_far_samples(const h3d_op *op_in, int32_t *per_tile, void *stream)
{
    if (!op_in || !per_tile) H3D_FAIL(H3D_ERR_ARG, "dcn_far_samples: null pointer");
    if (op_in->kind != H3D_OP_DCN_FUSED_STREAM || (op_in->dtype != H3D_BF16 && op_in->dtype != H3D_F16) || op_in->Cin % 32 || (op_in->reserved & H3D_OPF_DCN_STREAM_NO_SLOTS))
        H3D_FAIL(H3D_ERR_UNSUPPORTED, "dcn_far_samples: a 2-byte H3D_OP_DCN_FUSED_STREAM op of a patch-slot variant (Cin %% 32 == 0)");
    h3d_op op = *op_in;
    op.reserved = (op.reserved & H3D_OPF_DCN_STREAM_VARIANT_MASK) | H3D_OPF_DCN_STREAM_STATS;
    op.out = per_tile;
    op.out_mode = H3D_OUT_NHWC;
    return h3d_launch_dcn3(op, (hipStream_t)stream);
}
```

human-3d-reconstruction_amd/csrc/epilogue.h:

```cpp
#pragma once
#include "common.h"

struct EpiArgs {
    const float *bias;
    const char *res;
    char *out;
    int Ho, Wo, Cout, out_cs, res_cs, relu, out_mode;
};

template <typename T, int MT, int NT, bool FAST = false>
__device__ __forceinline__ void tile_epilogue(f32x16 (&acc)[MT][NT], const EpiArgs &a, int b, int oy0, int ox0,
                                              int cout0, int wv, int r, int h)
{
    using E = ET<T>;
    if constexpr (FAST) {
        const bool has_res = a.res != nullptr;
        const float lo = a.relu ? 0.f : -__builtin_inff();
#pragma unroll
        for (int n = 0; n < NT; ++n) {
            const int py = wv * (2 * NT) + n * 2 + (r >> 4), px = r & 15;
            const int oy = oy0 + py, ox = ox0 + px;
            if (oy >= a.Ho || ox >= a.Wo) continue;
            const size_t opix = ((size_t)b * a.Ho + oy) * a.Wo + ox;
            T *op = reinterpret_cast<T *>(a.out) + opix * a.out_cs + cout0 + 4 * h;
            const T *rp = reinterpret_cast<const T *>(a.res) + opix * a.res_cs + cout0 + 4 * h;
            const float *bp = a.bias + cout0 + 4 * h;
#pragma unroll
            for (int m = 0; m < MT; ++m) {
                float4 bias4[4];
#pragma unroll
                for (int g = 0; g < 4; ++g) bias4[g] = *reinterpret_cast<const float4 *>(bp + m * 32 + 8 * g);
#pragma unroll
                for (int g = 0; g < 4; ++g) {
                    const int co = m * 32 + 8 * g;
                    if (cout0 + co + 4 * h >= a.Cout) continue;
                    const float4 bv = bias4[g];
                    float v0 = acc[m][n][4 * g + 0] + bv.x, v1 = acc[m][n][4 * g + 1] + bv.y;
                    float v2 = acc[m][n][4 * g + 2] + bv.z, v3 = acc[m][n][4 * g + 3] + bv.w;
                    if (has_res) {
                        float rv[4];
                        load4<T>(rp + co, rv);
                        v0 += rv[0]; v1 += rv[1]; v2 += rv[2]; v3 += rv[3];
                    }
                    store4<T>(op + co, fmaxf(v0, lo), fmaxf(v1, lo), fmaxf(v2, lo), fmaxf(v3, lo));
                }
            }
        }
        return;
    }
#pragma unroll
    for (int n = 0; n < NT; ++n) {
        const int py = wv * (2 * NT) + n * 2 + (r >> 4), px = r & 15;
        const int oy = oy0 + py, ox = ox0 + px;
        if (oy >= a.Ho || ox >= a.Wo) continue;
        const size_t opix = ((size_t)b * a.Ho + oy) * a.Wo + ox;
#pragma unroll
        for (int m = 0; m < MT; ++m) {
#pragma unroll
            for (int g = 0; g < 4; ++g) {
                const int c = cout0 + m * 32 + 8 * g + 4 * h;
                if (c >= a.Cout) continue;
                float v[4];
#pragma unroll
                for (int i = 0; i < 4; ++i) v[i] = acc[m][n][4 * g + i] + a.bias[c + i];
                const bool full = (c + 4 <= a.Cout);
                if (a.res) {
                    const T *rp = reinterpret_cast<const T *>(a.res) + opix * a.res_cs + c;
                    if (full) {
                        float rv[4];
                        load4<T>(rp, rv);
#pragma unroll
                        for (int i = 0; i < 4; ++i) v[i] += rv[i];
                    } else {
                        for (int i = 0; i < 4 && c + i < a.Cout; ++i) v[i] += E::to_f32(rp[i]);
                    }
                }
                if (a.relu) {
#pragma unroll
                    for (int i = 0; i < 4; ++i) v[i] = fmaxf(v[i], 0.f);
                }
                if (a.out_mode == H3D_OUT_NHWC) {
                    T *op = reinterpret_cast<T *>(a.out) + opix * a.out_cs + c;
                    if (full) store4<T>(op, v[0], v[1], v[2], v[3]);
                    else for (int i = 0; i < 4 && c + i < a.Cout; ++i) op[i] = E::from_f32(v[i]);
                } else if (a.out_mode == H3D_OUT_NHWC_F32) {
                    float *op = reinterpret_cast<float *>(a.out) + opix * a.out_cs + c;
                    if (full) store4<float>(op, v[0], v[1], v[2], v[3]);
                    else for (int i = 0; i < 4 && c + i < a.Cout; ++i) op[i] = v[i];
                } else {
                    float *op = reinterpret_cast<float *>(a.out);
                    for (int i = 0; i < 4 && c + i < a.Cout; ++i)
                        op[(((size_t)b * a.Cout + c + i) * a.Ho + oy) * a.Wo + ox] = v[i];
                }
            }
        }
    }
}

template <int MT, int NT = 1> constexpr int epi_lds_stride() { return (NT * 32 * (64 * MT + 16) + 1023) / 1024 * 1024; }

template <typename T, int MT, int NT, bool HASRES>
__device__ __forceinline__ void tile_epilogue_lds_impl(f32x16 (&acc)[MT][NT], const EpiArgs &a, int b, int oy0, int ox0,
                                                       int cout0, int wv, int l, char *lw)
{
    constexpr int ROWB = 64 * MT + 16;
    constexpr int SPP = 4 * MT;
    constexpr int NPX = 32 * NT;
    const int r = l & 31, h = l >> 5;
    if constexpr (HASRES) {
        const size_t img_bytes = (size_t)a.Ho * a.Wo * a.res_cs * 2;
        const auto rs = __builtin_amdgcn_make_buffer_rsrc((void *)(a.res + (size_t)b * img_bytes), 0, (int)img_bytes, 0x00020000);
        constexpr int PIECES = (NPX * ROWB + 1023) / 1024;
#pragma unroll
        for (int pc = 0; pc < PIECES; ++pc) {
            const int q = pc * 64 + l;
            const int p = q / (SPP + 1), sl = q - p * (SPP + 1);
            const int oy = oy0 + 2 * NT * wv + (p >> 4), ox = ox0 + (p & 15);
            const bool ok = p < NPX && sl < SPP && oy < a.Ho && ox < a.Wo && cout0 + sl * 8 < a.Cout;
            const int voff = ok ? ((oy * a.Wo + ox) * a.res_cs + cout0 + sl * 8) * 2 : 0x7ffffff0;
            __builtin_amdgcn_raw_ptr_buffer_load_lds(rs, (__attribute__((address_space(3))) void *)(lw + pc * 1024), 16, voff, 0, 0, 0);
        }
        __builtin_amdgcn_s_waitcnt(0x0f70);
        __builtin_amdgcn_wave_barrier();
    }
    {
        const float *bp = a.bias + cout0 + 4 * h;
        const float lo = a.relu ? 0.f : -__builtin_inff();
#pragma unroll
        for (int m = 0; m < MT; ++m) {
            float4 bias4[4];
#pragma unroll
            for (int g = 0; g < 4; ++g) bias4[g] = *reinterpret_cast<const float4 *>(bp + m * 32 + 8 * g);
#pragma unroll
            for (int n = 0; n < NT; ++n)
#pragma unroll
                for (int g = 0; g < 4; ++g) {
                    const int co = m * 32 + 8 * g;
                    const float4 bv = bias4[g];
                    float v0 = acc[m][n][4 * g + 0] + bv.x, v1 = acc[m][n][4 * g + 1] + bv.y;
                    float v2 = acc[m][n][4 * g + 2] + bv.z, v3 = acc[m][n][4 * g + 3] + bv.w;
                    char *slot = lw + (n * 32 + r) * ROWB + (co + 4 * h) * 2;
                    if constexpr (HASRES) {
                        const u32x2 rr = *reinterpret_cast<const u32x2 *>(slot);
                        float r0, r1, r2, r3;
                        EP<T>::unpack2(rr[0], r0, r1);
                        EP<T>::unpack2(rr[1], r2, r3);
                        v0 += r0; v1 += r1; v2 += r2; v3 += r3;
                    }
                    const u32x2 pk = {EP<T>::pack2(EP<T>::clamp(v0, lo), EP<T>::clamp(v1, lo)), EP<T>::pack2(EP<T>::clamp(v2, lo), EP<T>::clamp(v3, lo))};
                    *reinterpret_cast<u32x2 *>(slot) = pk;
                }
        }
    }
    __builtin_amdgcn_s_waitcnt(0xc07f);
    __builtin_amdgcn_wave_barrier();
#pragma unroll
    for (int it = 0; it < NT * SPP / 2; ++it) {
        const int q = it * 64 + l;
        const int p = q / SPP, sl = q - p * SPP;
        const int oy = oy0 + 2 * NT * wv + (p >> 4), ox = ox0 + (p & 15);
        if (oy < a.Ho && ox < a.Wo && cout0 + sl * 8 < a.Cout) {
            const u32x4 v = *reinterpret_cast<const u32x4 *>(lw + p * ROWB + sl * 16);
            const size_t opix = ((size_t)b * a.Ho + oy) * a.Wo + ox;
            *reinterpret_cast<u32x4 *>(a.out + (opix * a.out_cs + cout0 + sl * 8) * 2) = v;
        }
    }
}

template <typename T, int MT, int NT = 1>
__device__ __forceinline__ void tile_epilogue_lds(f32x16 (&acc)[MT][NT], const EpiArgs &a, int b, int oy0, int ox0,
                                                  int cout0, int wv, int l, char *lw)
{
    static_assert(sizeof(T) == 2, "2-byte NHWC outputs");
    if (a.res) tile_epilogue_lds_impl<T, MT, NT, true>(acc, a, b, oy0, ox0, cout0, wv, l, lw);
    else tile_epilogue_lds_impl<T, MT, NT, false>(acc, a, b, oy0, ox0, cout0, wv, l, lw);
}
```

human-3d-reconstruction_amd/csrc/ops.hip:

```cpp
#include "common.h"
#include <stdlib.h>

static thread_local char g_err[512] = "";

void h3d_set_error(const char *fmt, ...)
{
    va_list ap;
    va_start(ap, fmt);
    vsnprintf(g_err, sizeof(g_err), fmt, ap);
    va_end(ap);
}

static thread_local char g_kname[160] = "";
static thread_local bool g_dry = false;

bool h3d_note_kernel(const char *fmt, ...)
{
    va_list ap;
    va_start(ap, fmt);
    vsnprintf(g_kname, sizeof(g_kname), fmt, ap);
    va_end(ap);
    return g_dry;
}

#ifdef H3D_ABLATE
unsigned long long *h3d_stamp_buffer()
{
    static unsigned long long *buf = [] { void *p = nullptr; (void)hipMalloc(&p, sizeof(unsigned long long) * 65536 * H3D_NSTAMP); return (unsigned long long *)p; }();
    return buf;
}
extern "C" int h3d_debug_stamps(unsigned long long *dst, int n)
{
    return hipMemcpy(dst, h3d_stamp_buffer(), sizeof(unsigned long long) * n, hipMemcpyDeviceToHost) == hipSuccess ? 0 : -1;
}
#endif

int h3d_xcd_mode()
{
    static const int mode = [] { const char *e = getenv("H3D_XCD"); return e ? atoi(e) : 1; }();
    return mode;
}

extern "C" const char *h3d_last_error(void) { return g_err; }
extern "C" int h3d_abi_version(void) { return H3D_ABI_VERSION; }
extern "C" int h3d_build_flags(void)
{
    int f = 0;
#ifdef H3D_EXTRA
    f |= H3D_BUILD_EXTRA;
#endif
#ifdef H3D_ABLATE
    f |= H3D_BUILD_ABLATE;
#endif
    return f;
}

int h3d_launch_conv(const h3d_op &op, hipStream_t st);
int h3d_launch_stem(const h3d_op &op, hipStream_t st);
int h3d_launch_elementwise(const h3d_op &op, hipStream_t st);
int h3d_launch_dcn(const h3d_op &op, hipStream_t st);
int h3d_launch_heads(const h3d_op &op, hipStream_t st);
int h3d_launch_dcn2(const h3d_op &op, hipStream_t st);
int h3d_launch_dcn3(const h3d_op &op, hipStream_t st);
int h3d_launch_conv_stream(const h3d_op &op, hipStream_t st);
int h3d_launch_dcn4(const h3d_op &op, hipStream_t st);
int h3d_launch_updcn(const h3d_op &op, hipStream_t st);
int h3d_launch_stem3(const h3d_op &op, hipStream_t st);
int h3d_launch_extra(const h3d_op &op, hipStream_t st);

static int run_one(const h3d_op &op, int i, hipStream_t st);

extern "C" int h3d_op_kernel_name(const h3d_op *op, char *buf, int buflen)
{
    if (!op || !buf || buflen <= 0) H3D_FAIL(H3D_ERR_ARG, "op_kernel_name: null argument");
    g_dry = true;
    g_kname[0] = 0;
    const int rc = run_one(*op, 0, nullptr);
    g_dry = false;
    snprintf(buf, buflen, "%s", g_kname);
    return rc;
}

extern "C" int h3d_run_ops_timed(const h3d_op *ops, int n, void *stream, float *ms)
{
    if (!ops || n <= 0 || !ms) H3D_FAIL(H3D_ERR_ARG, "run_ops_timed: null argument");
    hipStream_t st = (hipStream_t)stream;
    hipEvent_t *ev = (hipEvent_t *)malloc(sizeof(hipEvent_t) * (n + 1));
    if (!ev) H3D_FAIL(H3D_ERR_ARG, "run_ops_timed: out of host memory");
    for (int i = 0; i <= n; ++i) (void)hipEventCreate(&ev[i]);
    int rc = H3D_OK;
    (void)hipEventRecord(ev[0], st);
    for (int i = 0; i < n && rc == H3D_OK; ++i) {
        rc = run_one(ops[i], i, st);
        (void)hipEventRecord(ev[i + 1], st);
    }
    if (rc == H3D_OK) {
        (void)hipEventSynchronize(ev[n]);
        for (int i = 0; i < n; ++i) (void)hipEventElapsedTime(&ms[i], ev[i], ev[i + 1]);
    }
    for (int i = 0; i <= n; ++i) (void)hipEventDestroy(ev[i]);
    free(ev);
    return rc;
}

extern "C" int h3d_run_ops(const h3d_op *ops, int n, void *stream)
{
    if (!ops || n < 0) H3D_FAIL(H3D_ERR_ARG, "run_ops: null plan");
    hipStream_t st = (hipStream_t)stream;
    for (int i = 0; i < n; ++i) {
        const int rc = run_one(ops[i], i, st);
        if (rc != H3D_OK) return rc;
    }
    return H3D_OK;
}

static int run_one(const h3d_op &op, int i, hipStream_t st)
{
    int rc;
    if (op.B <= 0 || op.H <= 0 || op.W <= 0 || op.Ho <= 0 || op.Wo <= 0 || op.Cin <= 0 || op.Cout <= 0) {
        h3d_set_error("op %d (kind %d): non-positive dimension", i, op.kind);
        return H3D_ERR_SHAPE;
    }
    switch (op.kind) {
    case H3D_OP_STEM: rc = h3d_launch_stem(op, st); break;
    case H3D_OP_STEM3: rc = h3d_launch_stem3(op, st); break;
    case H3D_OP_CONV: rc = h3d_launch_conv(op, st); break;
    case H3D_OP_CONV_STREAM: rc = h3d_launch_conv_stream(op, st); break;
    case H3D_OP_DCN: rc = h3d_launch_dcn2(op, st); break;
#ifdef H3D_EXTRA
    case H3D_OP_DCN_V1: rc = h3d_launch_dcn(op, st); break;
    case H3D_OP_DCN_FUSED_F16: rc = h3d_launch_dcn4(op, st); break;
    case H3D_OP_UPDCN_F16: rc = h3d_launch_updcn(op, st); break;
#else
    case H3D_OP_DCN_V1:
    case H3D_OP_DCN_FUSED_F16:
    case H3D_OP_UPDCN_F16:
        h3d_set_error("op %d (kind %d): a superseded kernel generation, built only by `make EXTRA=1` (csrc/Makefile)", i, op.kind);
        return H3D_ERR_UNSUPPORTED;
#endif
    case H3D_OP_DCN_FUSED:
    case H3D_OP_DCN_FUSED_STREAM: rc = h3d_launch_dcn3(op, st); break;
    case H3D_OP_HEADS: rc = h3d_launch_heads(op, st); break;
    case H3D_OP_MAXPOOL:
    case H3D_OP_UPADD:
    case H3D_OP_COPY: rc = h3d_launch_elementwise(op, st); break;
    case H3D_OP_IM2COL:
    case H3D_OP_MAXPOOL3:
    case H3D_OP_DEPTH2SPACE: rc = h3d_launch_extra(op, st); break;
    default: h3d_set_error("op %d: unknown kind %d", i, op.kind); return H3D_ERR_ARG;
    }
    if (rc != H3D_OK) {
        char tmp[400];
        snprintf(tmp, sizeof(tmp), "%s", h3d_last_error());
        h3d_set_error("op %d (kind %d): %s", i, op.kind, tmp);
    }
    return rc;
}
```

human-3d-reconstruction_amd/detector.py:

```python
import torch

from . import _lib, decode, smpl as _smpl
from .model import create_model
from .utils import _transpose_and_gather_feat

MULTI_POSE_HEADS = {"hm": 1, "wh": 2, "hps": 34, "reg": 2, "hm_hp": 17, "hp_offset": 2}
CTDET_HEADS = {"hm": 80, "wh": 2, "reg": 2}
SMPL_HEADS = {"pose": 72, "shape": 10}
WHOLE_MAP_HEADS = ("hm", "hm_hp", "hp_offset")
PEAK_HEADS = ("hp_offset",)


class LazyHeads(dict):

    def __init__(self, maps, completer):
        super().__init__(maps)
        self._completer = completer

    @property
    def complete(self):
        return self._completer is None

    def rearm(self, completer):
        self._completer = completer

    def _complete(self):
        c = self._completer
        if c is not None:
            c()
            self._completer = None

    def __getitem__(self, k):
        self._complete()
        return super().__getitem__(k)

    def get(self, k, default=None):
        self._complete()
        return super().get(k, default)

    def items(self):
        self._complete()
        return super().items()

    def values(self):
        self._complete()
        return super().values()

    def __iter__(self):
        self._complete()
        return super().__iter__()

    def __contains__(self, k):
        self._complete()
        return super().__contains__(k)

    def copy(self):
        self._complete()
        return dict(super().items())


class Opt:

    def __init__(self, **kw):
        self.task = "multi_pose"
        self.arch = "dla_34"
        self.head_conv = 256
        self.down_ratio = 4
        self.K = 100
        self.not_use_dcn = False
        self.input_h = self.input_w = 512
        self.reg_offset = True
        self.hm_hp = True
        self.reg_hp_offset = True
        self.flip_test = False
        self.flip_idx = [[1, 2], [3, 4], [5, 6], [7, 8], [9, 10], [11, 12], [13, 14], [15, 16]]
        self.smpl = False
        self.smpl_people = None
        self.smpl_cam = False
        self.dtype = "bf16"
        for k, v in kw.items():
            setattr(self, k, v)
        self.output_h, self.output_w = self.input_h // self.down_ratio, self.input_w // self.down_ratio
        if self.task == "ctdet":
            self.num_classes = getattr(self, "num_classes", 80)
            self.cat_spec_wh = getattr(self, "cat_spec_wh", False)
            heads = {"hm": self.num_classes, "wh": 2 if not self.cat_spec_wh else 2 * self.num_classes}
            if self.reg_offset:
                heads["reg"] = 2
        elif self.task == "multi_pose":
            self.num_classes = 1
            heads = {"hm": 1, "wh": 2, "hps": 34}
            if self.reg_offset:
                heads["reg"] = 2
            if self.hm_hp:
                heads["hm_hp"] = 17
            if self.reg_hp_offset:
                heads["hp_offset"] = 2
            if self.smpl:
                heads.update(SMPL_HEADS)
                if self.smpl_cam:
                    heads["cam"] = 3
        else:
            raise ValueError("task not defined!")
        self.heads = heads


class MultiPoseDetector:
    def __init__(self, opt, state_dict=None, smpl_model=None, device="cuda"):
        if opt.task != "multi_pose":
            raise ValueError("task not defined!")
        self.opt = opt
        self.device = torch.device(device)
        self.model = create_model(opt.arch, opt.heads, opt.head_conv, opt.not_use_dcn, dtype=opt.dtype)
        if state_dict is not None:
            self.model.load_state_dict(state_dict, strict=True)
        self.model.to(self.device).eval()
        self.smpl_model = smpl_model
        self.fused_tail = True
        self.sparse_heads = True
        if opt.arch.replace("-", "_") in ("dla_34", "dla34") and opt.dtype in ("bf16", "f16"):
            self.model.engine_flags["split_heads"] = tuple(h for h in opt.heads if h in WHOLE_MAP_HEADS)
            self.model.engine_flags["peak_heads"] = tuple(h for h in opt.heads if h in PEAK_HEADS)
        if opt.smpl and smpl_model is None:
            self.smpl_model = _smpl.SMPLModel.synthetic()

    @torch.no_grad()
    def run(self, images, meta=None, slot=0, graph=False):
        if graph and meta is None:
            return self._run_graph(images, slot)
        opt = self.opt
        plan = None
        if self.sparse_heads and not opt.flip_test and images.is_cuda and not self.model.training:
            plan = self.model.engine(images.device).forward_eager(images, slot)
        if plan is not None:
            out = plan.outputs
            top = decode._multi_pose_topk(out["hm"], out.get("hm_hp") if opt.hm_hp else None, opt.K, logits=True)
            if plan.sparse_masks[1] and top["hm_inds"] is not None:
                plan.run_sparse_lists(top["inds"], opt.K, top["hm_inds"].view(top["inds"].shape[0], -1), top["hm_inds"].shape[1] * opt.K)
            else:
                plan.run_sparse(top["inds"], opt.K)
            dets, aux = decode._multi_pose_assemble(top, out["wh"], out["hps"], out.get("reg") if opt.reg_offset else None,
                                                    out.get("hp_offset") if opt.reg_hp_offset else None, return_aux=True)
            heads = LazyHeads(out, None)
        else:
            if opt.flip_test:
                out = self._flip_test_heads(images, slot)
            else:
                out = self.model(images, slot)[-1]
            dets, aux = decode.multi_pose_decode_logits(
                out["hm"], out["wh"], out["hps"], reg=out.get("reg") if opt.reg_offset else None,
                hm_hp=out.get("hm_hp") if opt.hm_hp else None,
                hp_offset=out.get("hp_offset") if opt.reg_hp_offset else None, K=opt.K, return_aux=True)
            heads = out
        res = {"dets": dets, "inds": aux["inds"], "heads": heads}
        if opt.smpl:
            n = opt.smpl_people or opt.K
            B = aux["inds"].shape[0]
            fusable = all(out[k].dtype == torch.float32 and out[k].is_contiguous() for k in ("pose", "shape"))
            if B * n >= 64 and self.fused_tail and fusable:
                verts, joints = _smpl.lbs_from_heads(self.smpl_model, out["pose"], out["shape"], aux["inds"], n, return_joints=True,
                                                     exact=opt.dtype in ("f32", "f16x3"))
            else:
                inds = aux["inds"][:, :n].contiguous()
                thetas = _transpose_and_gather_feat(out["pose"], inds).view(B * n, 72)
                betas = _transpose_and_gather_feat(out["shape"], inds).view(B * n, 10)
                verts, joints = _smpl.lbs(self.smpl_model, betas, thetas, return_joints=True,
                                          kernel="auto_exact" if opt.dtype in ("f32", "f16x3") else "auto")
            res["verts"] = verts.view(B, n, -1, 3)
            res["joints"] = joints.view(B, n, 24, 3)
        if meta is not None:
            res["results"] = multi_pose_post_process(dets, meta["c"], meta["s"], out["hm"].shape[2],
                                                     out["hm"].shape[3])
        if plan is not None and not torch.cuda.is_current_stream_capturing():
            heads.rearm(_heads_completer(plan))
        return res


def _heads_completer(plan):
    done = torch.cuda.Event()
    done.record()

    def complete():
        cur = torch.cuda.current_stream()
        cur.wait_event(done)
        plan.run_deferred()
        plan.pending = torch.cuda.Event()
        plan.pending.record(cur)
    return complete


def _run_graph(self, images, slot):
    _lib.require_cuda(images)
    if not hasattr(self, "_graphs"):
        self._graphs = {}
    key = (tuple(images.shape), slot)
    ent = self._graphs.get(key)
    if ent is None:
        static_in = images.detach().clone().float().contiguous()
        self.run(static_in, slot=slot)
        torch.cuda.current_stream().synchronize()
        g = torch.cuda.CUDAGraph()
        with torch.cuda.graph(g):
            res = self.run(static_in, slot=slot)
        ent = self._graphs[key] = (g, static_in, res)
    g, static_in, res = ent
    if images.data_ptr() != static_in.data_ptr():
        static_in.copy_(images)
    B, _, H, W = static_in.shape
    plan = self.model.engine(static_in.device).plans.get((B, H, W) if slot == 0 else (B, H, W, slot))
    if isinstance(res["heads"], LazyHeads) and plan is not None and plan.pending is not None:
        torch.cuda.current_stream().wait_event(plan.pending)
        plan.pending = None
    g.replay()
    if isinstance(res["heads"], LazyHeads):
        res["heads"].rearm(_heads_completer(plan))
    return res


MultiPoseDetector._run_graph = _run_graph


class CtdetDetector:

    def __init__(self, opt, state_dict=None, device="cuda"):
        if opt.task != "ctdet":
            raise ValueError("task not defined!")
        self.opt = opt
        self.device = torch.device(device)
        self.model = create_model(opt.arch, opt.heads, opt.head_conv, opt.not_use_dcn, dtype=opt.dtype)
        if state_dict is not None:
            self.model.load_state_dict(state_dict, strict=True)
        self.model.to(self.device).eval()

    @torch.no_grad()
    def run(self, images, meta=None, slot=0):
        from .utils import _sigmoid
        opt = self.opt
        out = self.model(images, slot)[-1]
        hm = _sigmoid(out["hm"].clone())
        dets = decode.ctdet_decode(hm, out["wh"], reg=out.get("reg") if opt.reg_offset else None,
                                   cat_spec_wh=opt.cat_spec_wh, K=opt.K)
        res = {"dets": dets, "heads": out}
        if meta is not None:
            res["results"] = ctdet_post_process(dets, meta["c"], meta["s"], out["hm"].shape[2], out["hm"].shape[3],
                                                out["hm"].shape[1])
        return res


def make_detector(opt, state_dict=None, device="cuda", **kw):
    if opt.task == "multi_pose":
        return MultiPoseDetector(opt, state_dict, device=device, **kw)
    if opt.task == "ctdet":
        return CtdetDetector(opt, state_dict, device=device)
    raise ValueError("task not defined!")


def ctdet_post_process(dets, c, s, h, w, num_classes):
    _lib.require_cuda(dets)
    dets = dets.contiguous().float()
    B, K, D = dets.shape
    if D != 6:
        raise RuntimeError("ctdet_post_process: dets [B,K,6] expected, got %s" % (tuple(dets.shape),))
    c = torch.as_tensor(c, dtype=torch.float32, device=dets.device).contiguous().view(B, 2)
    s = torch.as_tensor(s, dtype=torch.float32, device=dets.device).contiguous().view(-1)
    if s.numel() == 2 * B:
        s = s.view(B, 2)[:, 0].contiguous()
    out = torch.empty(B, K, 5, dtype=torch.float32, device=dets.device)
    _lib.check(_lib.lib().h3d_multi_pose_post_process(_lib.ptr(dets), _lib.ptr(c), _lib.ptr(s), B, K, 0, int(h), int(w),
                                                      _lib.ptr(out), _lib.stream_ptr()), "ctdet_post_process")
    boxes = out.cpu().numpy()
    classes = dets[:, :, 5].cpu().numpy()
    ret = []
    for i in range(B):
        ret.append({j + 1: boxes[i, classes[i] == j].tolist() for j in range(num_classes)})
    return ret


def _flip_test_heads(self, images, slot=0):
    from .utils import _sigmoid, flip_lr, flip_lr_off, flip_tensor
    B = images.shape[0]
    out = self.model(torch.cat([images, torch.flip(images, [3])], 0).contiguous(), slot)[-1]
    idx = self.opt.flip_idx
    res = {}
    for k, v in out.items():
        a, b = v[:B], v[B:]
        if k in ("hm", "hm_hp"):
            pa = _sigmoid(a.clone())
            pb = _sigmoid(b.clone())
            pb = flip_tensor(pb) if k == "hm" else flip_lr(pb, idx)
            p = (pa + pb) / 2
            res[k] = torch.log(p / (1 - p))
        elif k == "wh":
            res[k] = (a + flip_tensor(b)) / 2
        elif k == "hps":
            res[k] = (a + flip_lr_off(b, idx)) / 2
        else:
            res[k] = a.contiguous()
    return res


MultiPoseDetector._flip_test_heads = _flip_test_heads


def run_frames(detector, frames):
    from . import preprocess
    inp, c, s = preprocess.pre_process(frames, input_res=detector.opt.input_h)
    return detector.run(inp, meta={"c": c, "s": s})


def multi_pose_post_process(dets, c, s, h, w):
    _lib.require_cuda(dets)
    dets = dets.contiguous().float()
    B, K, D = dets.shape
    J = (D - 6) // 2
    c = torch.as_tensor(c, dtype=torch.float32, device=dets.device).contiguous().view(B, 2)
    s = torch.as_tensor(s, dtype=torch.float32, device=dets.device).contiguous().view(-1)
    if s.numel() == 2 * B:
        s = s.view(B, 2)[:, 0].contiguous()
    out = torch.empty(B, K, 5 + 2 * J, dtype=torch.float32, device=dets.device)
    _lib.check(_lib.lib().h3d_multi_pose_post_process(_lib.ptr(dets), _lib.ptr(c), _lib.ptr(s), B, K, J, int(h), int(w),
                                                      _lib.ptr(out), _lib.stream_ptr()), "multi_pose_post_process")
    return out


def gather_detections(dets, group=None, n_images=None, force=False):
    import torch.distributed as dist
    if not dist.is_available() or not dist.is_initialized() or (dist.get_world_size(group) == 1 and not force):
        return dets
    world = dist.get_world_size(group)
    dets = dets.contiguous()
    if n_images is None or n_images % world == 0:
        if n_images is not None and dets.shape[0] != n_images // world:
            raise RuntimeError("gather_detections: this rank holds %d images, shard_batch(%d, ., %d) gives %d"
                               % (dets.shape[0], n_images, world, n_images // world))
        out = torch.empty((world * dets.shape[0],) + tuple(dets.shape[1:]), dtype=dets.dtype, device=dets.device)
        dist.all_gather_into_tensor(out, dets, group=group)
        return out
    rows = -(-n_images // world)
    lo, hi = shard_batch(n_images, dist.get_rank(group), world)
    if dets.shape[0] != hi - lo:
        raise RuntimeError("gather_detections: this rank holds %d images, shard_batch(%d, %d, %d) gives %d"
                           % (dets.shape[0], n_images, dist.get_rank(group), world, hi - lo))
    mine = dets.new_zeros((rows,) + tuple(dets.shape[1:]))
    mine[:hi - lo] = dets
    out = torch.empty((world * rows,) + tuple(dets.shape[1:]), dtype=dets.dtype, device=dets.device)
    dist.all_gather_into_tensor(out, mine, group=group)
    out = out.view((world, rows) + tuple(dets.shape[1:]))
    sizes = [shard_batch(n_images, r, world) for r in range(world)]
    return torch.cat([out[r, :b - a] for r, (a, b) in enumerate(sizes)], 0)


def shard_batch(n_images, rank, world):
    base, rem = divmod(n_images, world)
    lo = rank * base + min(rank, rem)
    return lo, lo + base + (1 if rank < rem else 0)
```

human-3d-reconstruction_amd/plan.py:

```python
import ctypes

import torch

from . import _lib, arch, arch_hg, arch_res
from ._lib import H3dOp
from .weights import _TORCH_DT, LOWP

_H3D_DT = {"bf16": _lib.H3D_BF16, "f16": _lib.H3D_F16, "f32": _lib.H3D_F32, "f16x3": _lib.H3D_F16X3}
DCN_F16IN = _lib.OPF_DCN_STREAM_F16_INPUT


class View:
    __slots__ = ("buf", "H", "W", "C", "cs", "coff", "es")

    def __init__(self, buf, H, W, C, cs, coff, es):
        self.buf, self.H, self.W, self.C, self.cs, self.coff, self.es = buf, H, W, C, cs, coff, es

    @property
    def ptr(self):
        return self.buf.data_ptr() + self.coff * self.es

    def slice(self, c0, c):
        assert c0 + c <= self.C
        return View(self.buf, self.H, self.W, c, self.cs, self.coff + c0, self.es)


class Plan:

    FLAGS = dict(
        fuse_heads=True,
        fuse_offsets=True,
        stream_convs=True,
        stream_dcn=False,
        stream_s2=True,
        stream_dcn3=True,
        dcn_patches=True,
        dense_dcn3=True,
        dense_dcn3_min_tiles=512,
        fuse_upnode=True,
        fuse_upnode_min_f=2,
        dcn_slots512=0,
        dcn_wide_margin=0,
        node_f16=True,
        share_pool=True,
        fuse_stem=True,
        fuse_stem_proj=False,
        mixed_heads=0,
        wide_heads_m2=0,
        x3_dcn_patches=True,
        stem_s2_direct=True,
        conv1x1_th16_min_cin=0,
        lower_heads=True,
        split_heads=(),
        peak_heads=(),
    )

    def __init__(self, pw, B, H, W, **flags):
        unknown = set(flags) - set(self.FLAGS)
        if unknown:
            raise TypeError("unknown lowering flags: %s" % sorted(unknown))
        for k, v in self.FLAGS.items():
            setattr(self, k, flags.get(k, v))
        self.stream_s2_min_cin = 64
        if pw.arch == "hourglass" and (H % 128 or W % 128):
            raise RuntimeError("Hourglass-104: input height/width must be multiples of 128 (got %dx%d): the published test "
                               "code pads to (x|127)+1" % (H, W))
        if H % 32 or W % 32:
            raise RuntimeError("input height/width must be multiples of 32 (got %dx%d): the reference pads "
                               "to (x|31)+1 (datasets/coco.py:160-163)" % (H, W))
        self.pw, self.B, self.H, self.W = pw, B, H, W
        self.dtype = pw.dtype
        self.es = 2 if pw.dtype in LOWP else 4
        self.ops = []
        self.dcn_layers = []
        self.keep = []
        self.images = torch.empty(B, 3, H, W, dtype=torch.float32, device=pw.device)
        self.image = View(self.images, H, W, 3, 3, 0, 4)
        self.outputs = {}
        self.all_outputs = None
        self._out_at = {}
        self.n_eager = None
        self.sparse_op = None
        self._sparse_at = {}
        self.sparse_masks = (0, 0)
        self.pending = None
        if pw.arch == "hourglass":
            self._lower_hourglass()
        elif pw.arch == "resdcn101":
            self._lower_resdcn()
        else:
            self._lower()
        self.op_array = (H3dOp * len(self.ops))(*self.ops)

    def _alloc(self, H, W, C, dtype=None):
        td = _TORCH_DT[self.dtype] if dtype is None else dtype
        buf = torch.empty(self.B, H, W, C, dtype=td, device=self.pw.device)
        self.keep.append(buf)
        return View(buf, H, W, C, C, 0, buf.element_size())

    def _new_output(self, head, c, H, W, at):
        o = torch.empty(self.B, c, H, W, dtype=torch.float32, device=self.pw.device)
        self.outputs[head], self._out_at[head] = o, at
        return View(o, H, W, c, c, 0, 4)

    def _op(self, kind, x=None, out=None, x2=None, emit=True, **kw):
        op = H3dOp()
        op.kind, op.dtype, op.B = kind, _H3D_DT[self.dtype], self.B
        if x is not None:
            op.in_, op.H, op.W, op.Cin, op.in_cs = x.ptr, x.H, x.W, x.C, x.cs
        if out is not None:
            op.out, op.Ho, op.Wo, op.Cout, op.out_cs = out.ptr, out.H, out.W, out.C, out.cs
        if x2 is not None:
            op.in2, op.in2_cs = x2.ptr, x2.cs
        for k, v in kw.items():
            setattr(op, k, v)
        if not emit:
            return op
        self.ops.append(op)
        return len(self.ops) - 1

    def conv(self, x, wkey, out=None, bkey=None, bn=None, stride=1, relu=True, res=None, out_mode=_lib.OUT_NHWC,
             pad_cout_to=None):
        wshape = self.pw.sd[wkey].shape
        if (self.stream_convs and self.pw.dtype in LOWP and wshape[2] == 3 and wshape[1] % 16 == 0
                and (stride == 1 or (stride == 2 and wshape[1] >= self.stream_s2_min_cin and self.stream_s2))
                and out_mode == _lib.OUT_NHWC and pad_cout_to is None):
            return self._conv_stream(x, wkey, out, bkey, bn, relu, res, stride)
        wp, bp, cout, cin, k, rows = self.pw.conv(wkey, bkey, bn, pad_cout_to)
        assert cin == x.C, (wkey, cin, x.C)
        Ho = (x.H + 2 * (k // 2) - k) // stride + 1
        Wo = (x.W + 2 * (k // 2) - k) // stride + 1
        if out_mode == _lib.OUT_NHWC_F32:
            out = self._alloc(Ho, Wo, cout, torch.float32)
        elif out is None:
            out = self._alloc(Ho, Wo, cout)
        assert (out.H, out.W, out.C) == (Ho, Wo, cout), (wkey, out.H, out.W, out.C, Ho, Wo, cout)
        tune = 0
        if (k == 1 and stride == 1 and self.conv1x1_th16_min_cin and cin >= self.conv1x1_th16_min_cin and cin % 64 == 0
                and cout > 32 and self.pw.dtype in LOWP):
            tune = _lib.TUNE_CONV_1X1_TILE(4 if cout > 64 else 2, 16)
        self._op(_lib.OP_CONV, x, out, res, w=wp.data_ptr(), bias=bp.data_ptr(), ksize=k, stride=stride, relu=int(relu),
                 out_mode=out_mode, wrows=rows, reserved=tune, wexp=self.pw.wexp.get(wp.data_ptr(), 0))
        return out

    def _conv_stream(self, x, wkey, out, bkey, bn, relu, res, stride=1):
        wimg, bp, cout, cin, rows = self.pw.conv_stream(wkey, bkey, bn)
        assert cin == x.C, (wkey, cin, x.C)
        Ho, Wo = (x.H - 1) // stride + 1, (x.W - 1) // stride + 1
        if out is None:
            out = self._alloc(Ho, Wo, cout)
        assert (out.H, out.W, out.C) == (Ho, Wo, cout), (wkey, out.H, out.W, out.C)
        self._op(_lib.OP_CONV_STREAM, x, out, res, w=wimg.data_ptr(), bias=bp.data_ptr(), ksize=3, stride=stride, relu=int(relu),
                 out_mode=_lib.OUT_NHWC, wrows=rows)
        return out

    def dcn(self, x, om, wkey, bkey, bn):
        wp, bp, cout, cin, k, rows = self.pw.conv(wkey, bkey, bn, as_half=True)
        assert cin == x.C and k == 3
        out = self._alloc(x.H, x.W, cout)
        self._op(_lib.OP_DCN, x, out, om, w=wp.data_ptr(), bias=bp.data_ptr(), ksize=3, stride=1, relu=1, out_mode=_lib.OUT_NHWC,
                 wrows=rows)
        return out

    def pool(self, x, out=None):
        if out is None:
            out = self._alloc(x.H // 2, x.W // 2, x.C)
        assert out.C == x.C
        self._op(_lib.OP_MAXPOOL, x, out, ksize=2, stride=2)
        return out

    def upadd(self, x, skip, wkey, f16=False):
        w, k = self.pw.up(wkey)
        f = k // 2
        out = self._alloc(x.H * f, x.W * f, x.C)
        assert (skip.H, skip.W, skip.C) == (out.H, out.W, out.C), wkey
        self._op(_lib.OP_UPADD, x, out, skip, w=w.data_ptr(), ksize=k, stride=f, out_mode=_lib.OUT_NHWC_F16 if f16 else _lib.OUT_NHWC)
        return out

    def _block(self, x, p, stride, residual, out):
        t = self.conv(x, p + ".conv1.weight", bn=p + ".bn1", stride=stride)
        return self.conv(t, p + ".conv2.weight", bn=p + ".bn2", res=residual, out=out)

    def _tree1(self, x, p, cin, cout, stride, level_root, out, cat=None, bottom=None, residual=None):
        Ho, Wo = x.H // stride, x.W // stride
        if cat is None:
            cat = self._alloc(Ho, Wo, 2 * cout + (cin if level_root else 0))
        s_x2, s_x1 = cat.slice(0, cout), cat.slice(cout, cout)
        if residual is not None:
            assert stride > 1 and not level_root and cin != cout and (residual.H, residual.W, residual.C) == (Ho, Wo, cout)
        elif bottom is not None:
            assert stride > 1 and not level_root and (bottom.H, bottom.W, bottom.C) == (Ho, Wo, cin)
        elif stride > 1:
            bottom = self.pool(x, cat.slice(2 * cout, cin) if level_root else None)
        else:
            bottom = x
        if residual is not None:
            pass
        elif cin != cout:
            residual = self.conv(bottom, p + ".project.0.weight", bn=p + ".project.1", relu=False)
        else:
            residual = bottom
        self._block(x, p + ".tree1", stride, residual, s_x1)
        self._block(s_x1, p + ".tree2", 1, s_x1, s_x2)
        return self.conv(cat, p + ".root.conv.weight", bn=p + ".root.bn", out=out)

    def _tree2(self, x, p, cin, cout, out):
        Ho, Wo = x.H // 2, x.W // 2
        cat = self._alloc(Ho, Wo, 2 * cout + cin + cout)
        pooled = self.pool(x, cat.slice(2 * cout, cin))
        x1 = self._tree1(x, p + ".tree1", cin, cout, 2, False, cat.slice(2 * cout + cin, cout),
                         bottom=pooled if self.share_pool else None)
        return self._tree1(x1, p + ".tree2", cout, cout, 1, False, out, cat=cat)

    def _dcn_f16_ok(self, p):
        w = self.pw.sd[p + ".conv.weight"]
        return (self.pw.use_dcn and self.fuse_offsets and self.stream_dcn and self.pw.dtype == "bf16"
                and w.shape[1] == 64 and w.shape[0] <= 64)

    def _node_f16_ok(self, p):
        w = self.pw.sd[p + ".conv.weight"]
        return (self.node_f16 and self.pw.use_dcn and self.fuse_offsets and self.pw.dtype == "bf16" and self.stream_dcn3 and self.dcn_patches
                and w.shape[1] % 32 == 0 and w.shape[0] > 32 and w.shape[0] % 8 == 0)

    def _deform(self, x, p, x_is_f16=False, in_f16=False):
        pw = self.pw
        cout, cin = pw.sd[p + ".conv.weight"].shape[:2]
        fused = pw.use_dcn and self.fuse_offsets
        kw, has_variants = {}, False
        if x_is_f16:
            kind, pack = _lib.OP_DCN_FUSED_F16, pw.dcn_stream(p)
        elif (fused and pw.dtype in LOWP
                and (self.stream_dcn3 or (self.dense_dcn3 and cout <= 64
                                          and self.B * ((x.H + 15) // 16) * ((x.W + 15) // 16) >= self.dense_dcn3_min_tiles))):
            kind, pack = _lib.OP_DCN_FUSED_STREAM, pw.dcn_stream(p, int(_lib.lib().h3d_dcn_fused_ck(int(cin), int(cout))))
            var = 0
            if self.dcn_patches and cin % 32 == 0:
                var = _lib.OPF_DCN_STREAM_WIDE_MARGIN if self.dcn_wide_margin else _lib.OPF_DCN_STREAM_SLOTS512 if self.dcn_slots512 else pw.dcn_variant.get(p, 0)
            kw = dict(reserved=(var | (DCN_F16IN if in_f16 else 0)) if self.dcn_patches else _lib.OPF_DCN_STREAM_NO_SLOTS)
            has_variants = True
        else:
            assert not in_f16, p
            if fused and pw.dtype == "f16x3" and self.x3_dcn_patches and cin % 32 == 0:
                kind, pack = _lib.OP_DCN_FUSED_STREAM, pw.dcn_stream_x3(p)
                kw = dict(wexp=pw.wexp[pack[0].data_ptr()], wexp2=pw.wexp[pack[1].data_ptr()])
            elif fused:
                kind, pack = _lib.OP_DCN_FUSED, pw.dcn_fused(p)
                kw = dict(wexp=pw.wexp.get(pack[0].data_ptr(), 0), wexp2=pw.wexp.get(pack[1].data_ptr(), 0))
            elif pw.use_dcn:
                if pw.dtype == "f16":
                    raise RuntimeError("fp16 plans run the fused DeformConv kernel only (fuse_offsets=False is a bf16 / f32 debugging path)")
                om = self.conv(x, p + ".conv.conv_offset_mask.weight", bkey=p + ".conv.conv_offset_mask.bias",
                               relu=False, out_mode=_lib.OUT_NHWC_F32, pad_cout_to=32)
                return self.dcn(x, om, p + ".conv.weight", p + ".conv.bias", p + ".actf.0")
            else:
                return self.conv(x, p + ".conv.weight", bkey=p + ".conv.bias", bn=p + ".actf.0")
        wmain, woff, bias, cout, cin, rows = pack
        assert cin == x.C, (p, cin, x.C)
        out = self._alloc(x.H, x.W, cout)
        i = self._op(kind, x, out, in2=woff.data_ptr(), w=wmain.data_ptr(), bias=bias.data_ptr(), ksize=3, stride=1, relu=1,
                     out_mode=_lib.OUT_NHWC, wrows=rows, **kw)
        if has_variants:
            self.dcn_layers.append((p, i))
        return out

    def _ida(self, layers, p, startp, endp):
        for i in range(startp + 1, endp):
            k = i - startp
            y = self._deform(layers[i], "%s.proj_%d" % (p, k))
            f16 = self._dcn_f16_ok("%s.node_%d" % (p, k))
            if f16 and self.fuse_upnode and self.pw.up("%s.up_%d.weight" % (p, k))[1] // 2 >= self.fuse_upnode_min_f:
                layers[i] = self._updcn(y, layers[i - 1], "%s.up_%d.weight" % (p, k), "%s.node_%d" % (p, k))
                continue
            nf16 = not f16 and self._node_f16_ok("%s.node_%d" % (p, k))
            y = self.upadd(y, layers[i - 1], "%s.up_%d.weight" % (p, k), f16=f16 or nf16)
            layers[i] = self._deform(y, "%s.node_%d" % (p, k), x_is_f16=f16, in_f16=nf16)

    def _updcn(self, x, skip, wkey, p):
        wup, k = self.pw.up(wkey)
        f = k // 2
        wimg, woimg, bias, cout, cin, rows = self.pw.dcn_stream(p)
        assert (skip.H, skip.W, skip.C) == (x.H * f, x.W * f, x.C) and cin == x.C == 64, wkey
        out = self._alloc(skip.H, skip.W, cout)
        desc = _lib.H3dUpdcnDesc()
        desc.skip, desc.w_up, desc.w_off, desc.skip_cs = skip.ptr, wup.data_ptr(), woimg.data_ptr(), skip.cs
        self.keep.append(desc)
        self._op(_lib.OP_UPDCN_F16, x, out, in2=ctypes.addressof(desc), w=wimg.data_ptr(), bias=bias.data_ptr(), ksize=3, stride=f,
                 relu=1, out_mode=_lib.OUT_NHWC, wrows=rows)
        return out

    def _lower(self):
        H, W = self.H, self.W
        C = arch.CHANNELS
        y0 = res2 = None
        if self.fuse_stem and self.pw.dtype == "f16x3" and C[0] == 16 and C[1] == 32:
            y1 = self._alloc((H - 1) // 2 + 1, (W - 1) // 2 + 1, C[1])
            w, b = self.pw.stem3_x3()
            self._op(_lib.OP_STEM3, self.image, y1, w=w.data_ptr(), bias=b.data_ptr(), ksize=7, stride=2, relu=1)
        elif self.fuse_stem and self.pw.dtype in LOWP and C[0] == 16 and C[1] == 32 and W % 4 == 0:
            y1 = self._alloc((H - 1) // 2 + 1, (W - 1) // 2 + 1, C[1])
            proj = self.fuse_stem_proj and C[2] == 64 and y1.H % 2 == 0 and y1.W % 2 == 0
            w, b = self.pw.stem3(proj)
            res2 = self._alloc(y1.H // 2, y1.W // 2, C[2]) if proj else None
            self._op(_lib.OP_STEM3, self.image, y1, res2, w=w.data_ptr(), bias=b.data_ptr(), ksize=7, stride=2, relu=1)
        else:
            w, b = self.pw.stem()
            x = self._alloc(H, W, C[0])
            self._op(_lib.OP_STEM, self.image, x, w=w.data_ptr(), bias=b.data_ptr(), ksize=7, stride=1, relu=1,
                     wexp=self.pw.wexp.get(w.data_ptr(), 0))
            y0 = self.conv(x, "base.level0.0.weight", bn="base.level0.1")
            y1 = self.conv(y0, "base.level1.0.weight", bn="base.level1.1", stride=2)
        y2 = self._tree1(y1, "base.level2", C[1], C[2], 2, False, None, residual=res2)
        y3 = self._tree2(y2, "base.level3", C[2], C[3], None)
        y4 = self._tree2(y3, "base.level4", C[3], C[4], None)
        y5 = self._tree1(y4, "base.level5", C[4], C[5], 2, True, None)
        layers = [y0, y1, y2, y3, y4, y5]
        outs = [layers[-1]]
        for i in range(3):
            self._ida(layers, "dla_up.ida_%d" % i, len(layers) - i - 2, len(layers))
            outs.insert(0, layers[-1])
        ys = [outs[0], outs[1], outs[2]]
        self._ida(ys, "ida_up", 0, 3)
        self.feat = ys[-1]
        if self.lower_heads:
            self._lower_heads(self.feat)

    def _lower_heads(self, feat):
        Ho, Wo = feat.H, feat.W
        fused = (self.pw.head_conv > 0 and self.pw.head_conv % 64 == 0 and feat.C == 64 and
                 len(self.pw.heads) <= _lib.HEADS_MAX and max(self.pw.heads.values()) <= 96 and self.fuse_heads)
        if fused:
            def heads_op(names, emit=True):
                w1, b1, per = self.pw.fused_heads(tuple(names))
                desc = _lib.H3dHeadsDesc()
                desc.nheads = len(per)
                desc.wexp = self.pw.wexp.get(w1.data_ptr(), 0)
                for i, (head, c, w2, b2) in enumerate(per):
                    if head in self.outputs:
                        optr, self._sparse_at[head] = self.outputs[head].data_ptr(), (desc, i)
                    else:
                        optr = self._new_output(head, c, Ho, Wo, (desc, i)).ptr
                    desc.head[i].w2, desc.head[i].b2, desc.head[i].out, desc.head[i].C = w2.data_ptr(), b2.data_ptr(), optr, c
                    desc.head[i].wexp2 = self.pw.wexp.get(w2.data_ptr(), 0)
                self.keep.append(desc)
                return self._op(_lib.OP_HEADS, feat, in2=ctypes.addressof(desc), w=w1.data_ptr(), bias=b1.data_ptr(),
                                Ho=Ho, Wo=Wo, Cout=self.pw.head_conv, ksize=3, stride=1, emit=emit)

            peak = tuple(self.peak_heads or ())
            eager = tuple(h for h in self.pw.heads if h in tuple(self.split_heads or ()) and h not in peak)
            deferred = tuple(h for h in self.pw.heads if h not in eager)
            split = bool(eager) and bool(deferred) and self.pw.dtype in LOWP
            if split:
                heads_op(eager)
                self.n_eager = len(self.ops)
            groups = {}
            for head, c in self.pw.heads.items():
                if split and head in eager:
                    continue
                m2 = (c + 31) // 32
                groups.setdefault(0 if self.mixed_heads else 1 if m2 == 1 else self.wide_heads_m2 or m2, []).append(head)
            for m2 in sorted(groups):
                heads_op(groups[m2])
            if split:
                self.sparse_op = heads_op(deferred, emit=False)
                pk = sum(1 << i for i, h in enumerate(deferred) if h in peak)
                self.sparse_masks = ((1 << len(deferred)) - 1 - pk, pk)
            self.outputs = {h: self.outputs[h] for h in self.pw.heads}
            return
        for head in self.pw.heads:
            if self.pw.head_conv > 0:
                t = self.conv(feat, head + ".0.weight", bkey=head + ".0.bias")
                self._head_conv(t, head, head + ".2.weight", head + ".2.bias")
            else:
                self._head_conv(feat, head, head + ".weight", head + ".bias")

    def _head_conv(self, x, head, wkey, bkey):
        o = self._new_output(head, self.pw.heads[head], x.H, x.W, len(self.ops))
        self.conv(x, wkey, out=o, bkey=bkey, relu=False, out_mode=_lib.OUT_NCHW_F32)

    def _stem_s2(self, wkey, bkey, bn, cout):
        Ho, Wo = (self.H - 1) // 2 + 1, (self.W - 1) // 2 + 1
        if self.dtype in LOWP and self.stem_s2_direct:
            w, b = self.pw.stem_s2(wkey, bkey, bn)
            x = self._alloc(Ho, Wo, cout)
            self._op(_lib.OP_STEM, self.image, x, w=w.data_ptr(), bias=b.data_ptr(), ksize=7, stride=2, relu=1)
            return x
        patches = self._alloc(Ho, Wo, 160)
        self._op(_lib.OP_IM2COL, self.image, patches, ksize=7, stride=2)
        return self.conv(patches, self.pw.im2col_key(wkey), bkey=bkey, bn=bn)

    def _lower_resdcn(self):
        x = self._stem_s2("conv1.weight", None, "bn1", 64)
        y = self._alloc((x.H - 1) // 2 + 1, (x.W - 1) // 2 + 1, x.C)
        self._op(_lib.OP_MAXPOOL3, x, y, ksize=3, stride=2)
        x = y
        for p, cin, planes, stride, down in arch_res.blocks(101):
            t = self.conv(x, p + ".conv1.weight", bn=p + ".bn1")
            t = self.conv(t, p + ".conv2.weight", bn=p + ".bn2", stride=stride)
            res = self.conv(x, p + ".downsample.0.weight", bn=p + ".downsample.1", stride=stride, relu=False) if down else x
            x = self.conv(t, p + ".conv3.weight", bn=p + ".bn3", res=res)
        for i, planes in enumerate(arch_res.DECONV):
            x = self._deform(x, "deconv_layers.%d" % (6 * i))
            wkey, bn = self.pw.deconv4_as_conv3("deconv_layers.%d.weight" % (6 * i + 3), "deconv_layers.%d" % (6 * i + 4))
            t = self.conv(x, wkey, bn=bn)
            assert t.C == 4 * planes
            x = self._alloc(2 * t.H, 2 * t.W, planes)
            self._op(_lib.OP_DEPTH2SPACE, t, x, ksize=1, stride=1)
        self.feat = x
        if self.lower_heads:
            self._lower_heads(x)

    def _hg_residual(self, x, p, cin, cout, stride):
        t = self.conv(x, p + ".conv1.weight", bn=p + ".bn1", stride=stride)
        skip = x
        if arch_hg.residual_has_skip(cin, cout, stride):
            skip = self.conv(x, p + ".skip.0.weight", bn=p + ".skip.1", stride=stride, relu=False)
        return self.conv(t, p + ".conv2.weight", bn=p + ".bn2", res=skip)

    def _hg_seq(self, x, p, kind, cin, cout, modules):
        for j, (ci, co, st) in enumerate(arch_hg.layer_specs(kind, cin, cout, modules)):
            x = self._hg_residual(x, "%s.%d" % (p, j), ci, co, st)
        return x

    def _hg_kp(self, x, p, n, dims, modules):
        up1 = self._hg_seq(x, p + ".up1", "layer", dims[0], dims[0], modules[0])
        low1 = self._hg_seq(x, p + ".low1", "hg", dims[0], dims[1], modules[0])
        if n > 1:
            low2 = self._hg_kp(low1, p + ".low2", n - 1, dims[1:], modules[1:])
        else:
            low2 = self._hg_seq(low1, p + ".low2", "layer", dims[1], dims[1], modules[1])
        low3 = self._hg_seq(low2, p + ".low3", "revr", dims[1], dims[0], modules[0])
        return self.upadd(low3, up1, self.pw.nearest_up_key(dims[0]))

    def _lower_hourglass(self):
        nstack = 2
        inter = self._stem_s2("pre.0.conv.weight", None, "pre.0.bn", arch_hg.PRE_DIM)
        inter = self._hg_residual(inter, "pre.1", arch_hg.PRE_DIM, arch_hg.DIMS[0], 2)
        self.all_outputs = []
        for i in range(nstack):
            kp = self._hg_kp(inter, "kps.%d" % i, arch_hg.N, arch_hg.DIMS, arch_hg.MODULES)
            cnv = self.conv(kp, "cnvs.%d.conv.weight" % i, bn="cnvs.%d.bn" % i)
            self.outputs = {}
            for head in self.pw.heads:
                t = self.conv(cnv, "%s.%d.0.conv.weight" % (head, i), bkey="%s.%d.0.conv.bias" % (head, i))
                self._head_conv(t, head, "%s.%d.1.weight" % (head, i), "%s.%d.1.bias" % (head, i))
            self.all_outputs.append(self.outputs)
            if i < nstack - 1:
                a = self.conv(inter, "inters_.%d.0.weight" % i, bn="inters_.%d.1" % i, relu=False)
                inter = self.conv(cnv, "cnvs_.%d.0.weight" % i, bn="cnvs_.%d.1" % i, res=a)
                inter = self._hg_residual(inter, "inters.%d" % i, arch_hg.DIMS[0], arch_hg.DIMS[0], 1)

    def retarget_outputs(self, views):
        for h, v in views.items():
            assert v.is_contiguous() and tuple(v.shape) == tuple(self.outputs[h].shape)
        for h in self.outputs:
            at = self._out_at[h]
            if isinstance(at, int):
                self.op_array[at].out = views[h].data_ptr()
            else:
                at[0].head[at[1]].out = views[h].data_ptr()
            if h in self._sparse_at:
                at = self._sparse_at[h]
                at[0].head[at[1]].out = views[h].data_ptr()
        self.outputs = dict(views)

    def _run_range(self, first, n):
        if self.pending is not None:
            torch.cuda.current_stream().wait_event(self.pending)
            self.pending = None
        if n > 0:
            ops = self.op_array if first == 0 else ctypes.byref(self.op_array[first])
            rc = _lib.lib().h3d_run_ops(ops, n, _lib.stream_ptr())
            _lib.check(rc, "h3d_run_ops")
        return self.outputs

    def run(self):
        return self._run_range(0, len(self.ops))

    def run_eager(self):
        return self._run_range(0, self.n_eager)

    def run_sparse(self, inds, K):
        _lib.require_cuda(inds)
        if inds.dtype != torch.int64 or not inds.is_contiguous() or tuple(inds.shape) != (self.B, K):
            raise RuntimeError("run_sparse: contiguous int64 inds [%d,%d] expected, got %s %s" % (self.B, K, tuple(inds.shape), inds.dtype))
        if not self.sparse_masks[1]:
            _lib.check(_lib.lib().h3d_heads_sparse(ctypes.byref(self.sparse_op), _lib.ptr(inds), int(K), _lib.stream_ptr()), "h3d_heads_sparse")
        elif self.sparse_masks[0]:
            self._sparse_lists("run_sparse", (inds, K, self.sparse_masks[0]))

    def _sparse_lists(self, what, *lists):
        arr = (_lib.H3dHeadsList * len(lists))()
        for e, (inds, K, mask) in zip(arr, lists):
            _lib.require_cuda(inds)
            if inds.dtype != torch.int64 or not inds.is_contiguous() or tuple(inds.shape) != (self.B, K):
                raise RuntimeError("%s: contiguous int64 inds [%d,%d] expected, got %s %s" % (what, self.B, K, tuple(inds.shape), inds.dtype))
            e.inds, e.K, e.head_mask = inds.data_ptr(), int(K), mask
        _lib.check(_lib.lib().h3d_heads_sparse_lists(ctypes.byref(self.sparse_op), len(lists), arr, _lib.stream_ptr()), "h3d_heads_sparse_lists")

    def run_sparse_lists(self, inds, K, peak_inds, PK):
        if self.sparse_op is None or not self.sparse_masks[1]:
            raise RuntimeError("run_sparse_lists: this plan was lowered without peak_heads (dtype %s)" % self.dtype)
        self._sparse_lists("run_sparse_lists", *([(inds, K, self.sparse_masks[0])] if self.sparse_masks[0] else []), (peak_inds, PK, self.sparse_masks[1]))

    def run_deferred(self):
        return self._run_range(self.n_eager, len(self.ops) - self.n_eager)
```

include/h3d.h:

```cpp
#ifndef H3D_H
#define H3D_H

#include <stddef.h>
#include <stdint.h>

#ifdef __cplusplus
extern "C" {
#endif

#define H3D_OK 0
#define H3D_ERR_SHAPE (-1)
#define H3D_ERR_DTYPE (-2)
#define H3D_ERR_LAUNCH (-3)
#define H3D_ERR_UNSUPPORTED (-4)
#define H3D_ERR_ARG (-5)

#define H3D_F32 0
#define H3D_BF16 1
#define H3D_F16 2
#define H3D_F16X3 3

const char *h3d_last_error(void);
int h3d_abi_version(void);
#define H3D_ABI_VERSION 4
#define H3D_BUILD_EXTRA 1
#define H3D_BUILD_ABLATE 2
int h3d_build_flags(void);

int h3d_dcn_v2_forward(const float *input, const float *weight, const float *bias,
                       const float *offset, const float *mask, float *output,
                       int B, int C, int H, int W, int Cout,
                       int kernel_h, int kernel_w, int stride_h, int stride_w,
                       int pad_h, int pad_w, int dilation_h, int dilation_w,
                       int deformable_group, void *stream);

int h3d_dcn_v2_backward_workspace_bytes(int B, int C, int H, int W, int Cout, int kernel_h, int kernel_w,
                                        int stride_h, int stride_w, int pad_h, int pad_w, int dilation_h, int dilation_w,
                                        int deformable_group, size_t *bytes);
int h3d_dcn_v2_backward(const float *input, const float *weight, const float *bias, const float *offset, const float *mask,
                        const float *grad_output,
                        float *grad_input, float *grad_offset, float *grad_mask, float *grad_weight, float *grad_bias,
                        int B, int C, int H, int W, int Cout, int kernel_h, int kernel_w, int stride_h, int stride_w,
                        int pad_h, int pad_w, int dilation_h, int dilation_w, int deformable_group,
                        void *workspace, size_t workspace_bytes, void *stream);
int h3d_dcn_v2_backward_general(const float *input, const float *weight, const float *bias, const float *offset, const float *mask,
                                const float *grad_output,
                                float *grad_input, float *grad_offset, float *grad_mask, float *grad_weight, float *grad_bias,
                                int B, int C, int H, int W, int Cout, int kernel_h, int kernel_w, int stride_h, int stride_w,
                                int pad_h, int pad_w, int dilation_h, int dilation_w, int deformable_group,
                                void *workspace, size_t workspace_bytes, void *stream);

int h3d_dcn_offset_mask(const float *input, const float *off_weight, const float *off_bias, float *offset, float *mask,
                        int B, int C, int H, int W, int kernel_h, int kernel_w, int stride_h, int stride_w,
                        int pad_h, int pad_w, int deformable_group, void *stream);

size_t h3d_dcn_v2_workspace_bytes(int B, int C, int H, int W, int Cout);
int h3d_dcn_v2_forward_ws(const float *input, const float *weight, const float *bias,
                          const float *offset, const float *mask, float *output,
                          int B, int C, int H, int W, int Cout,
                          int kernel_h, int kernel_w, int stride_h, int stride_w,
                          int pad_h, int pad_w, int dilation_h, int dilation_w,
                          int deformable_group, void *workspace, size_t workspace_bytes, void *stream);

#define H3D_DCN_INPUT_NHWC 1
#define H3D_DCN_OUTPUT_NHWC 2
#define H3D_DCN_F32_MFMA 4
size_t h3d_dcn_v2_packed_weight_bytes(int Cout, int C, int dtype);
int h3d_dcn_v2_pack_weights(const float *weight, const float *bias, int Cout, int C, int dtype, void *packed, void *stream);
int h3d_dcn_v2_pack_weights_cached(const float *weight, const float *bias, int Cout, int C, int dtype, void *packed, void *state,
                                   void *stream);
int h3d_dcn_fused_pack_f32_cached(const float *weight, const float *bias, const float *off_weight, const float *off_bias, int Cout, int C,
                                  float *wp, float *wo, float *bias_out, void *state, void *stream);
size_t h3d_dcn_v2_packed_workspace_bytes(int B, int C, int H, int W, int flags);
int h3d_dcn_nchw_to_nhwc_scaled(const float *src, float *dst, int B, int C, int H, int W, unsigned *amax, void *stream);
int h3d_dcn_v2_forward_packed(const void *input, const void *packed, const float *offset, const float *mask, void *output,
                              int B, int C, int H, int W, int Cout, int dtype, int flags,
                              void *workspace, size_t workspace_bytes, void *stream);

int h3d_dcn_v2_psroi_pooling_forward(const float *input, const float *bbox, const float *trans, float *output, float *output_count,
                                     int B, int C, int H, int W, int num_bbox, int channels_trans, int no_trans, float spatial_scale,
                                     int output_dim, int group_size, int pooled_size, int part_size, int sample_per_part,
                                     float trans_std, void *stream);
int h3d_dcn_pooling_modulated(const float *input, const float *bbox, const float *offset_mask, float *output, int B, int C, int H,
                              int W, int num_bbox, float spatial_scale, int output_dim, int group_size, int pooled_size, int part_size,
                              int sample_per_part, float trans_std, void *stream);

enum {
    H3D_OP_STEM = 1,
    H3D_OP_CONV = 2,
    H3D_OP_DCN = 3,
    H3D_OP_MAXPOOL = 4,
    H3D_OP_UPADD = 5,
    H3D_OP_COPY = 6,
    H3D_OP_DCN_FUSED = 9,
    H3D_OP_CONV_STREAM = 10,
    H3D_OP_DCN_FUSED_F16 = 11,
    H3D_OP_DCN_FUSED_STREAM = 12,
    H3D_OP_STEM3 = 13,
    H3D_OP_DCN_V1 = 8,
    H3D_OP_UPDCN_F16 = 14,
    H3D_OP_IM2COL = 15,
    H3D_OP_MAXPOOL3 = 16,
    H3D_OP_DEPTH2SPACE = 17,
    H3D_OP_HEADS = 7
};

#define H3D_HEADS_MAX 16
typedef struct h3d_heads_desc {
    int32_t nheads;
    int32_t wexp;
    struct {
        const void *w2;
        const float *b2;
        float *out;
        int32_t C;
        int32_t wexp2;
    } head[H3D_HEADS_MAX];
} h3d_heads_desc;
typedef struct h3d_updcn_desc {
    const void *skip;
    const float *w_up;
    const void *w_off;
    int32_t skip_cs;
    int32_t reserved;
} h3d_updcn_desc;
enum { H3D_OUT_NHWC = 0, H3D_OUT_NCHW_F32 = 1, H3D_OUT_NHWC_F32 = 2,
       H3D_OUT_NHWC_F16 = 3  };

typedef struct h3d_op {
    int32_t kind;
    int32_t dtype;
    const void *in;
    const void *in2;
    const void *w;
    const float *bias;
    void *out;
    int32_t B, H, W;
    int32_t Cin, in_cs;
    int32_t in2_cs;
    int32_t Ho, Wo;
    int32_t Cout, out_cs;
    int32_t ksize;
    int32_t stride;
    int32_t relu;
    int32_t out_mode;
    int32_t wrows;
    int32_t reserved;
    int32_t wexp;
    int32_t wexp2;
} h3d_op;


#define H3D_DCN_AUX_BYTES 256
#define H3D_DCN_FUSED_BIAS_WMAX 32
#define H3D_DCN_FUSED_BIAS_AMAX 34

enum {
    H3D_OPF_DCN_MASK_FINAL = 0x800,
    H3D_OPF_DCN_RAW_PACK = 0x100000,
    H3D_OPF_DCN_ACT_MAXIMA = 0x200000,
    H3D_TUNE_DCN_ABLATE_MASK = 0x1f
};

enum {
    H3D_OPF_DCN_FUSED_RAW_PACK = 0x100000,
    H3D_OPF_DCN_FUSED_SCALED_INPUT = 0x200000,
    H3D_TUNE_DCN_FUSED_X3_MARGIN2 = 0x2000,
    H3D_TUNE_DCN_FUSED_X3_MARGIN6 = 0x4000,
    H3D_TUNE_DCN_FUSED_X3_MARGIN4 = 0x8000,
    H3D_TUNE_DCN_FUSED_X3_ABLATE_MASK = 0x1f
};

enum {
    H3D_OPF_DCN_STREAM_NO_SLOTS = 0x1000,
    H3D_OPF_DCN_STREAM_WIDE_MARGIN = 0x8000,
    H3D_OPF_DCN_STREAM_SLOTS512 = 0x10000,
    H3D_OPF_DCN_STREAM_F16_INPUT = 0x40000,
    H3D_OPF_DCN_STREAM_STATS = 0x20000,
    H3D_OPF_DCN_STREAM_VARIANT_MASK = 0x58600,
    H3D_TUNE_DCN_STREAM_FORCE_NARROW_WG = 0x200,
    H3D_TUNE_DCN_STREAM_FORCE_WIDE_WG = 0x400,
    H3D_TUNE_DCN_STREAM_F16_DCN5 = 0x4000,
    H3D_TUNE_DCN_STREAM_F16_KEEP_DCN3 = 0x2000,
    H3D_TUNE_DCN_STREAM_ABLATE_MASK = 0x1f
};
#define H3D_TUNE_DCN_STREAM_DCN5_XP(xp) ((xp) << 16)
#define H3D_TUNE_DCN_STREAM_DCN5_XP_OF(reserved) (((reserved) >> 16) & 0xff)

enum {
    H3D_TUNE_DCN_STREAM_X3_MARGIN2 = 0x4000,
    H3D_TUNE_DCN_STREAM_X3_MARGIN3 = 0x8000,
    H3D_TUNE_DCN_STREAM_X3_MARGIN4 = 0x10000,
    H3D_TUNE_DCN_STREAM_X3_ABLATE_MASK = 0x1f
};

enum {
    H3D_TUNE_DCN_F16_ONE_WG_PER_CU = 0x100,
    H3D_TUNE_DCN_F16_ABLATE_MASK = 0xff
};

#define H3D_TUNE_CONV_STREAM_TILE(variant, mt, waves) ((variant) << 12 | (mt) << 8 | (waves))
#define H3D_TUNE_CONV_STREAM_ABLATE(bits) ((bits) << 16)
#define H3D_TUNE_CONV_STREAM_ABLATE_OF(reserved) (((reserved) & H3D_TUNE_CONV_STREAM_ABLATE_MASK) >> 16)
enum {
    H3D_TUNE_CONV_STREAM_TILE_MASK = 0xffff,
    H3D_TUNE_CONV_STREAM_AUTO = 1,
    H3D_TUNE_CONV_STREAM_ROUND4_RULE = 0x10000000,
    H3D_TUNE_CONV_STREAM_ABLATE_MASK = 0x1f0000
};

#define H3D_TUNE_CONV_1X1_TILE(mt, th) (H3D_TUNE_CONV_TILE | (mt) << 4 | (th) >> 3)
#define H3D_TUNE_CONV_1X1_TILE_MT(reserved) (((reserved) >> 4) & 15)
#define H3D_TUNE_CONV_1X1_TILE_TH(reserved) (((reserved) & 15) * 8)
#define H3D_TUNE_CONV_GEMM_TILE(n) ((n) << 8)
enum {
    H3D_TUNE_CONV_TILE = 0x1000,
    H3D_TUNE_CONV_HALO_TILE = 0x2000,
    H3D_TUNE_CONV_FORCE_GEMM = 0x4000,
    H3D_TUNE_CONV_GEMM_TILE_MASK = 0xf00
};
#define H3D_TUNE_CONV_X3_TILE(mt, waves, th) (H3D_TUNE_CONV_X3_TILED | (mt) << 8 | (waves) << 4 | (th) >> 3)
enum {
    H3D_TUNE_CONV_X3_TILED = 0x1000,
    H3D_TUNE_CONV_X3_TILE_MASK = 0x1fff,
    H3D_TUNE_CONV_X3_CK16 = 0x2000,
    H3D_TUNE_CONV_X3_MT2 = 0x4000
};

enum {
    H3D_TUNE_UPADD_TAPS_GLOBAL = 1,
    H3D_TUNE_UPADD_TAPS_LDS = 2
};

enum {
    H3D_TUNE_HEADS_SEPARATE_BIAS = 0x200,
    H3D_TUNE_HEADS_SPARSE_LDS_PATCH = 0x400,
    H3D_TUNE_HEADS_SPARSE_WAVES4 = 0x800,
    H3D_TUNE_HEADS_ABLATE_MASK = 0xff
};

int h3d_dcn_fused_ck(int Cin, int Cout);

int h3d_dcn_far_samples(const h3d_op *op, int32_t *per_tile, void *stream);

int h3d_run_ops(const h3d_op *ops, int n, void *stream);

int h3d_run_ops_timed(const h3d_op *ops, int n, void *stream, float *ms);
int h3d_op_kernel_name(const h3d_op *op, char *buf, int buflen);

int h3d_heads_sparse(const h3d_op *op, const int64_t *inds, int K, void *stream);

#define H3D_HEADS_LISTS_MAX 4
typedef struct h3d_heads_list {
    const int64_t *inds;
    int32_t K;
    uint32_t head_mask;
} h3d_heads_list;
int h3d_heads_sparse_lists(const h3d_op *op, int nlists, const h3d_heads_list *lists, void *stream);

int h3d_nchw_f32_to_nhwc(const float *src, void *dst, int dtype, int B, int C, int H, int W,
                         int dst_cs, void *stream);
int h3d_nhwc_to_nchw_f32(const void *src, int dtype, float *dst, int B, int C, int H, int W,
                         int src_cs, void *stream);

typedef struct h3d_heads_bwd_head {
    const float *w1, *b1, *w2;
    const float *grad_out;
    float *grad_w1, *grad_b1, *grad_w2, *grad_b2;
    int32_t C;
    int32_t reserved;
} h3d_heads_bwd_head;
int h3d_heads_backward_workspace_bytes(int B, int H, int W, int head_conv, int nheads, const int *C, size_t *bytes);
int h3d_heads_backward(const float *feat, int in_cs, int B, int H, int W, int head_conv, int nheads, const h3d_heads_bwd_head *heads,
                       float *grad_feat, void *workspace, size_t workspace_bytes, void *stream);

enum {
    H3D_CONV_BWD_RELU = 1
};
#define H3D_CONV_BWD_MFMA_CMAX 2048
int h3d_conv2d_backward_workspace_bytes(int B, int C, int H, int W, int Cout, int kh, int kw, int sh, int sw, int ph, int pw, int dh, int dw,
                                        int flags, size_t *bytes);
int h3d_conv2d_backward(const float *x, int x_cs, const float *weight, const float *y, int y_cs, const float *grad_y, int gy_cs,
                        float *grad_x, float *grad_res, float *grad_weight, float *grad_bias, int B, int C, int H, int W, int Cout,
                        int kh, int kw, int sh, int sw, int ph, int pw, int dh, int dw, int flags, void *workspace, size_t workspace_bytes,
                        void *stream);
int h3d_conv2d_backward_general(const float *x, int x_cs, const float *weight, const float *y, int y_cs, const float *grad_y, int gy_cs,
                                float *grad_x, float *grad_res, float *grad_weight, float *grad_bias, int B, int C, int H, int W, int Cout,
                                int kh, int kw, int sh, int sw, int ph, int pw, int dh, int dw, int flags, void *workspace,
                                size_t workspace_bytes, void *stream);


#define H3D_NMS_SIGMOID 1
#define H3D_NMS_SKIP 2
int h3d_nms_topk(const float *heat, int B, int C, int H, int W, int K, int flags,
                 float *scores, int64_t *inds, float *ys, float *xs, void *stream);
int h3d_nms_topk2(const float *heat_a, int Ca, float *scores_a, int64_t *inds_a, float *ys_a, float *xs_a,
                  const float *heat_b, int Cb, float *scores_b, int64_t *inds_b, float *ys_b, float *xs_b,
                  int B, int H, int W, int K, int flags, void *stream);

size_t h3d_nms_topk_large_workspace_bytes(int B, int C, int H, int W, int K);
int h3d_nms_topk_large(const float *heat, int B, int C, int H, int W, int K, int flags,
                       float *scores, int64_t *inds, float *ys, float *xs,
                       void *workspace, size_t workspace_bytes, void *stream);

int h3d_nms(const float *heat, int B, int C, int H, int W, float *out, void *stream);
int h3d_sigmoid_clamp(const float *in, float *out, size_t n, void *stream);

int h3d_topk_merge(const float *scores, const int64_t *inds, const float *ys, const float *xs,
                   int B, int C, int K, float *o_score, int64_t *o_ind, int32_t *o_cls,
                   float *o_y, float *o_x, void *stream);

int h3d_gather_feat(const float *feat, const int64_t *ind, int B, int C, int HW, int N,
                    int channels_last, float *out, void *stream);

int h3d_multi_pose_assemble(const float *c_score, const int64_t *c_ind, const int32_t *c_cls,
                            const float *c_y, const float *c_x,
                            const float *hp_score, const int64_t *hp_ind, const float *hp_y,
                            const float *hp_x,
                            const float *wh, const float *hps, const float *reg,
                            const float *hp_offset,
                            int B, int J, int H, int W, int K, float *dets, void *stream);

int h3d_ctdet_assemble(const float *c_score, const int64_t *c_ind, const int32_t *c_cls,
                       const float *c_y, const float *c_x, const float *wh, const float *reg,
                       int B, int C, int H, int W, int K, int cat_spec_wh, float *dets,
                       void *stream);

int h3d_preprocess(const uint8_t *images, int B, int h, int w, int row_bytes, const double *minv,
                   const float *mean, const float *stdv, int res_h, int res_w, float *out, void *stream);

struct h3d_train_image {
    double minv[6];
    double light[3];
    int64_t offset;
    int32_t h, w, row_bytes;
    int32_t flipped;
    int32_t order[3];
    float alpha[3];
    float one_minus_alpha[3];
    int32_t reserved;
};
#define H3D_TRAIN_BRIGHTNESS 0
#define H3D_TRAIN_CONTRAST 1
#define H3D_TRAIN_SATURATION 2
#define H3D_TRAIN_INPUT_NO_COLOR_AUG 1
int h3d_train_input_workspace_bytes(int B, int res_h, int res_w, int options, size_t *bytes);
int h3d_train_input(const uint8_t *images, size_t images_bytes, const struct h3d_train_image *desc,
                    const struct h3d_train_image *desc_dev, int B, const float *mean, const float *stdv, int res_h, int res_w,
                    int options, void *workspace, size_t workspace_bytes, float *out, float *gs_mean_out, void *stream);

int h3d_multi_pose_post_process(const float *dets, const float *c, const float *s, int B, int K,
                                int J, int out_h, int out_w, float *out, void *stream);

int h3d_smpl_pose(const float *betas, const float *thetas, const float *j_template,
                  const float *j_shapedirs, const int32_t *parents, int P,
                  float *pose_feat, float *A, float *joints, float *coefT, int Ppad, void *stream);
int h3d_smpl_pose_heads(const float *pose_map, const float *shape_map, const int64_t *inds, int B, int K, int n, int HW,
                        const float *j_template, const float *j_shapedirs, const int32_t *parents, float *betas_out,
                        float *pose_feat, float *A, float *joints, void *coefK3, int Ppad, void *stream);
int h3d_smpl_coef_pack(const float *betas, const float *pose_feat, int P, int Ppad, void *coefK3, void *stream);
int h3d_smpl_verts3(const void *coefK3, const float *A, const float *v_template, const void *dirsK3,
                    const int32_t *lbs_idx, const float *lbs_w, int nnz, int P, int Ppad, int V, int Vpad,
                    float *verts, void *stream);
int h3d_smpl_verts3_exact(const void *coefK3, const float *A, const float *v_template, const void *dirsK3,
                          const int32_t *lbs_idx, const float *lbs_w, int nnz, int P, int Ppad, int V, int Vpad,
                          float *verts, void *stream);
int h3d_smpl_verts(const float *betas, const float *pose_feat, const float *A,
                   const float *v_template, const float *shapedirsT, const float *posedirsT,
                   const int32_t *lbs_idx, const float *lbs_w, int nnz, int P, int V, int Vpad,
                   float *verts, void *stream);
int h3d_smpl_verts2(const float *coefT, const float *A, const float *v_template,
                    const float *shapedirsT, const float *posedirsT, const int32_t *lbs_idx,
                    const float *lbs_w, int nnz, int P, int Ppad, int V, int Vpad, float *verts,
                    void *stream);

int h3d_smpl_backward_workspace_bytes(int P, int V, int Vpad, int nnz, int want_verts, size_t *bytes);
int h3d_smpl_backward(const float *betas, const float *thetas, const float *grad_verts, const float *grad_joints,
                      const float *j_template, const float *j_shapedirs, const int32_t *parents, const float *v_template,
                      const void *dirsK3, const void *dirsV3, const int32_t *lbs_idx, const float *lbs_w, int nnz, int P, int V, int Vpad,
                      float *grad_betas, float *grad_thetas, void *workspace, size_t workspace_bytes, void *stream);
int h3d_smpl_heads_backward(const float *pose_map, const float *shape_map, const int64_t *inds, int B, int K, int n, int HW,
                            const float *grad_verts, const float *grad_joints, const float *j_template, const float *j_shapedirs,
                            const int32_t *parents, const float *v_template, const void *dirsK3, const void *dirsV3,
                            const int32_t *lbs_idx, const float *lbs_w, int nnz, int V, int Vpad, float *grad_pose_map,
                            float *grad_shape_map, void *workspace, size_t workspace_bytes, void *stream);

#define H3D_SMPL_KP_MAX_K 32
#define H3D_SMPL_KP_MAX_NV 16
int h3d_smpl_kp_loss_workspace_bytes(int B, int n, size_t *bytes);
int h3d_smpl_kp_loss_forward(const float *joints, const float *verts, const float *cam_map, const int64_t *ind, const float *hps,
                             const void *hps_mask, int mask_type, const float *joint_w, const int32_t *vert_idx, const float *vert_w,
                             int B, int max_objs, int n, int HW, int K, int NV, int V, float *kp3d, float *pred, float *stats,
                             void *workspace, size_t workspace_bytes, void *stream);
int h3d_smpl_kp_loss_backward(const float *kp3d, const float *pred, const float *cam_map, const int64_t *ind, const float *hps,
                              const void *hps_mask, int mask_type, const float *stats, const float *grad_out, const float *joint_w,
                              const int32_t *inv_vertex, const int32_t *inv_start, const int32_t *inv_k, const float *inv_w, int n_touched,
                              int B, int max_objs, int n, int HW, int K, int V, float *grad_joints, float *grad_verts, float *grad_cam_map,
                              void *stream);

#define H3D_RENDER_NEGATE_Z 1
#define H3D_RENDER_CULL_BACK 2
#define H3D_RENDER_MAX_V 13120
#define H3D_RENDER_MAX_SIDE 16384
int h3d_render_workspace_bytes(int B, int Hr, int Wr, size_t *bytes);
int h3d_render_rasterize(const float *verts, const int32_t *faces, const float *cam_map, const int64_t *ind, const uint8_t *valid,
                         const float *dz, int B, int max_objs, int n, int V, int F, int H, int W, int up, int flags, int32_t *face_id,
                         float *depth, void *workspace, size_t workspace_bytes, void *stream);
int h3d_render_shade(const void *keys, const float *verts, const int32_t *faces, const uint8_t *colour, const uint8_t *image, int B, int n,
                     int V, int F, int Hr, int Wr, float alpha, float ambient, int default_colour, int background, uint8_t *rgb,
                     void *stream);

enum { H3D_LOSS_FOCAL = 1, H3D_LOSS_REG_L1 = 2, H3D_LOSS_REG_WEIGHTED_L1 = 3, H3D_LOSS_NORM_REG_L1 = 4, H3D_LOSS_REG_SL1 = 5 };
enum { H3D_LOSS_MASK_U8 = 0, H3D_LOSS_MASK_F32 = 1 };
#define H3D_LOSS_FROM_LOGITS 1
#define H3D_LOSS_TUNE_GRID8 0x100
#define H3D_LOSS_MAX_TERMS 16
typedef struct h3d_loss_term {
    int32_t kind;
    int32_t flags;
    const float *x;
    const float *gt;
    float *pred;
    const int64_t *ind;
    const void *mask;
    float *grad;
    int64_t n;
    int32_t B, C, HW, M;
    int32_t mask_type;
    float weight;
} h3d_loss_term;
int h3d_loss_workspace_bytes(const h3d_loss_term *terms, int n_terms, size_t *bytes);
int h3d_loss_forward(const h3d_loss_term *terms, int n_terms, float *stats, void *workspace, size_t workspace_bytes, void *stream);
int h3d_loss_backward(const h3d_loss_term *terms, int n_terms, const float *stats, const float *coef, void *stream);

#define H3D_TARGETS_MSE_LOSS 1
#define H3D_TARGETS_DENSE_HP 2
#define H3D_TARGETS_DENSE_WH 4
#define H3D_TARGETS_MAX_JOINTS 64
#define H3D_TARGETS_MAX_OBJS 512
int h3d_targets_workspace_bytes(int B, int max_objs, int num_joints, size_t *bytes);
int h3d_multi_pose_targets(const float *boxes, const float *keypoints, const int32_t *num, const double *trans, const int32_t *rot_flag,
                           const int32_t *flipped, const int32_t *width, const int32_t *flip_pairs, int n_flip_pairs, int B, int M, int J,
                           int Hout, int Wout, int max_objs, float *hm, float *hm_hp, float *wh, float *reg, int64_t *ind,
                           uint8_t *reg_mask, float *kps, uint8_t *kps_mask, float *hp_offset, int64_t *hp_ind, int64_t *hp_mask,
                           float *gt_det, int32_t *gt_count, int options, void *workspace, size_t workspace_bytes, void *stream);
int h3d_ctdet_targets(const float *boxes, const int32_t *cls, const int32_t *num, const double *trans, const int32_t *flipped,
                      const int32_t *width, int B, int M, int Hout, int Wout, int num_classes, int max_objs, float *hm, float *wh,
                      float *reg, int64_t *ind, uint8_t *reg_mask, float *cat_spec_wh, uint8_t *cat_spec_mask, float *gt_det,
                      int32_t *gt_count, int options, void *workspace, size_t workspace_bytes, void *stream);

#define H3D_ADAM_CAPACITY 48
#define H3D_ADAM_CHUNK 2048
typedef struct h3d_adam_tensor {
    float *param;
    const float *grad;
    float *exp_avg;
    float *exp_avg_sq;
    int64_t n;
    float one_minus_b1, b2, one_minus_b2, bc2_sqrt, eps, neg_step_size, weight_decay;
} h3d_adam_tensor;
int h3d_adam_step(const h3d_adam_tensor *tensors , int n_tensors, void *stream);

#define H3D_COCO_BBOX 0
#define H3D_COCO_KEYPOINTS 1
#define H3D_COCO_ROUND2 1
#define H3D_COCO_MAX_D 128
#define H3D_COCO_MAX_G 1024
#define H3D_COCO_MAX_A 4
#define H3D_COCO_MAX_LANES 64
#define H3D_COCO_MAX_M 4
#define H3D_COCO_MAX_R 128
#define H3D_COCO_SCAN_CHUNK 1024
int h3d_coco_match_workspace_bytes(int N, int D, int G, size_t *bytes);
int h3d_coco_match(const float *dets, int det_stride, const int32_t *det_cls, const int32_t *det_num, const double *gt_boxes,
                   const double *gt_keypoints, const double *gt_area, const uint8_t *gt_iscrowd, const int32_t *gt_cls,
                   const int32_t *gt_num, int N, int D, int G, int iou_type, int flags, int max_det, const double *area_rng, int A,
                   const double *iou_thrs, int T, const double *kp_vars, double *ious, int32_t *dt_match, uint8_t *dt_ignore,
                   uint8_t *gt_ignore, double *dt_score, int32_t *dt_rank, double *dt_box, double *dt_area, double *dt_keypoints,
                   void *workspace, size_t workspace_bytes, void *stream);
int h3d_coco_accumulate_workspace_bytes(int K, int A, size_t *bytes);
int h3d_coco_accumulate(const int64_t *order, const int32_t *seg_start, const int32_t *dt_rank, const int32_t *dt_match,
                        const uint8_t *dt_ignore, const uint8_t *gt_ignore, const int32_t *gt_cls, const int32_t *gt_num, int N, int D,
                        int G, int K, int A, int T, const int32_t *max_dets , int M, const double *rec_thrs, int R,
                        double *precision, double *recall, void *workspace, size_t workspace_bytes, void *stream);

#define H3D_MESH_EVAL_MAX_SWEEPS 30
int h3d_pointset_errors(const float *pred, int Np, const float *gt, int Ng, int n, const int32_t *pred_idx, const int32_t *gt_idx, int P,
                        const uint8_t *weight, const float *pred_root, const float *gt_root, int nr, int root_a, int root_b, double *err,
                        int32_t *count, double *transform, void *stream);
int h3d_metric_means(const double *err, const int32_t *count, int P, double *means, int32_t *n_pairs, void *stream);

#ifdef __cplusplus
}
#endif
#endif
```

Measured before the change: 10640 images/s.

## Fold IDA up-sample-and-add into the preceding DCN stream kernel epilogue

When a DCN stream op's output is consumed only as the skip input of the following up-sample-plus-add op, the DCN kernel's LDS-transposed epilogue now computes the transposed-conv up-sample taps and adds them to the tile in place of writing the DCN result. The plan reorders IDA projections so those skip tensors are private, and the runtime recognises the flagged pair and skips the separate upadd launch. This removes one full-resolution write and read of the skip tensor plus one kernel launch per folded pair. In exchange the epilogue grows in register pressure and global loads, and the plan and scheduling logic become more complex.

```diff
diff --git a/human-3d-reconstruction_amd/_lib.py b/human-3d-reconstruction_amd/_lib.py
--- a/human-3d-reconstruction_amd/_lib.py
+++ b/human-3d-reconstruction_amd/_lib.py
@@ -27,7 +27,7 @@
 TUNE_CONV_STREAM_TILE_MASK, TUNE_CONV_STREAM_AUTO, TUNE_CONV_STREAM_ROUND4_RULE, TUNE_CONV_STREAM_ABLATE_MASK = 0xffff, 1, 0x10000000, 0x1f0000
 TUNE_CONV_TILE, TUNE_CONV_HALO_TILE, TUNE_CONV_FORCE_GEMM, TUNE_CONV_GEMM_TILE_MASK = 0x1000, 0x2000, 0x4000, 0xf00
 TUNE_CONV_X3_TILED, TUNE_CONV_X3_TILE_MASK, TUNE_CONV_X3_CK16, TUNE_CONV_X3_MT2 = 0x1000, 0x1fff, 0x2000, 0x4000
-TUNE_UPADD_TAPS_GLOBAL, TUNE_UPADD_TAPS_LDS = 1, 2
+TUNE_UPADD_TAPS_GLOBAL, TUNE_UPADD_TAPS_LDS, OPF_UPADD_FOLDED = 1, 2, 0x100
 TUNE_HEADS_SEPARATE_BIAS, TUNE_HEADS_ABLATE_MASK = 0x200, 0xff
 TUNE_HEADS_SPARSE_LDS_PATCH, TUNE_HEADS_SPARSE_WAVES4 = 0x400, 0x800
 
diff --git a/human-3d-reconstruction_amd/csrc/conv.hip b/human-3d-reconstruction_amd/csrc/conv.hip
--- a/human-3d-reconstruction_amd/csrc/conv.hip
+++ b/human-3d-reconstruction_amd/csrc/conv.hip
@@ -642,24 +642,10 @@
             }
         }
         sv = *reinterpret_cast<const u32x4 *>(skip + pix * skip_cs + v * N);
-        float acc[N], x[N];
-#pragma unroll
-        for (int n = 0; n < N; ++n) acc[n] = 0.f;
-#pragma unroll
-        for (int q = 0; q < 4; ++q) {
-            if (!ok[q]) continue;
-            unpack16<T>(xv[q], x);
-            const float *wp;
-            if constexpr (WLDS) wp = s_w + tap[q] * wrow + v * N;
-            else wp = w + tap[q] * C + v * N;
-#pragma unroll
-            for (int n = 0; n < N; ++n) acc[n] = fmaf(wp[n], x[n], acc[n]);
-        }
-        unpack16<T>(sv, x);
-#pragma unroll
-        for (int n = 0; n < N; ++n) acc[n] += x[n];
-        if constexpr (F16OUT) *reinterpret_cast<u32x4 *>(out + pix * out_cs + v * N) = pack16_f16(acc);
-        else *reinterpret_cast<u32x4 *>(out + pix * out_cs + v * N) = pack16<T>(acc);
+        u32x4 o;
+        if constexpr (WLDS) o = upadd_vec<T>([&](int q, int n) { return s_w[tap[q] * wrow + v * N + n]; }, ok, xv, sv, F16OUT);
+        else o = upadd_vec<T>([&](int q, int n) { return w[tap[q] * C + v * N + n]; }, ok, xv, sv, F16OUT);
+        *reinterpret_cast<u32x4 *>(out + pix * out_cs + v * N) = o;
     }
 }
 
@@ -692,7 +678,8 @@
     const bool f16out = op.kind == H3D_OP_UPADD && op.out_mode == H3D_OUT_NHWC_F16;
     if (f16out && op.dtype != H3D_BF16) H3D_FAIL(H3D_ERR_DTYPE, "upadd: fp16 output is an option of bf16 plans (fp16 plans write fp16 anyway)");
     const size_t up_wbytes = (size_t)op.ksize * op.ksize * op.Cin * sizeof(float);
-    const bool up_wlds = op.reserved == H3D_TUNE_UPADD_TAPS_GLOBAL ? false : op.reserved == H3D_TUNE_UPADD_TAPS_LDS ? up_wbytes <= 64 * 1024 : (up_wbytes <= 8192 || (up_wbytes <= 16384 && op.Cin <= 64));
+    const int up_tune = op.reserved & ~H3D_OPF_UPADD_FOLDED;
+    const bool up_wlds = up_tune == H3D_TUNE_UPADD_TAPS_GLOBAL ? false : up_tune == H3D_TUNE_UPADD_TAPS_LDS ? up_wbytes <= 64 * 1024 : (up_wbytes <= 8192 || (up_wbytes <= 16384 && op.Cin <= 64));
     return h3d_by_store_dtype<bf16_t, f16_t, float, x3_t>(op.dtype, "elementwise: dtype %d", [&](auto t) {
         using T = typename decltype(t)::type;
         const T *in = (const T *)op.in;
diff --git a/human-3d-reconstruction_amd/csrc/dcn3.hip b/human-3d-reconstruction_amd/csrc/dcn3.hip
--- a/human-3d-reconstruction_amd/csrc/dcn3.hip
+++ b/human-3d-reconstruction_amd/csrc/dcn3.hip
@@ -18,6 +18,7 @@
     int xscaled;
     int xcd;
     unsigned long long *stamps;
+    UpFoldArgs up;
 };
 
 #if defined(H3D_ABLATE) && defined(DCN3_STAMP_B)
@@ -59,12 +60,13 @@
 };
 
 
-template <typename T, int MT, int CK, int MARGIN, int EPI = 0, bool WDMA = false, int NP = 0, bool PK = false, bool F16IN = false, bool STATS = false>
+template <typename T, int MT, int CK, int MARGIN, int EPI = 0, bool WDMA = false, int NP = 0, bool PK = false, bool F16IN = false, bool STATS = false, bool FOLD = false>
 __global__ __launch_bounds__(512, (WDMA && MT <= 2 && sizeof(T) == 2) ? 4 : 2) void dcn3_kernel(Dcn3Args a)
 {
     using C = Dcn3Cfg<T, MT, CK, MARGIN, WDMA, NP, PK>;
     using X = SE<std::conditional_t<F16IN, f16_t, T>>;
     static_assert(!F16IN || (std::is_same<T, bf16_t>::value && WDMA && NP > 0), "fp16 input: an option of the bf16 patch-slot variants");
+    static_assert(!FOLD || (sizeof(T) == 2 && WDMA && NP > 0 && EPI == 2 && !STATS), "folded up-sample + add: the 2-byte patch-slot variants with the LDS-transposed epilogue");
     constexpr int ES = C::ES, SS = C::SS;
     constexpr bool ONEBUF = WDMA || C::SINGLE;
     __shared__ __attribute__((aligned(256))) char smem[C::LDS];
@@ -821,7 +823,8 @@
     const EpiArgs e = dcn_epi_args(a);
     if constexpr (EPI == 2) {
         __syncthreads();
-        tile_epilogue_lds<T, MT>(acc, e, b, oy0, ox0, cout0, wv, l, smem + wv * epi_lds_stride<MT>());
+        if constexpr (FOLD) tile_epilogue_lds_fold<T, MT>(acc, e, a.up, b, oy0, ox0, cout0, wv, l, smem + wv * epi_lds_stride<MT>());
+        else tile_epilogue_lds<T, MT>(acc, e, b, oy0, ox0, cout0, wv, l, smem + wv * epi_lds_stride<MT>());
     } else {
         tile_epilogue<typename StoreT<T>::type, MT, 1, EPI == 1>(acc, e, b, oy0, ox0, cout0, wv, r, h);
     }
@@ -836,7 +839,7 @@
 }
 
 template <typename T, int MT, int CK, int MARGIN, bool WDMA = false, int NP = 0, bool PK = false, bool F16IN = false>
-static int launch_dcn3_cfg(const Dcn3Args &a0, hipStream_t st, bool stats = false)
+static int launch_dcn3_cfg(const Dcn3Args &a0, hipStream_t st, bool stats = false, bool *folded = nullptr)
 {
     using C = Dcn3Cfg<T, MT, CK, MARGIN, WDMA, NP, PK>;
     static_assert(!(WDMA && MT <= 2 && sizeof(T) == 2) || C::LDS * 2 <= 160 * 1024, "two workgroups per CU");
@@ -859,6 +862,14 @@
                 return h3d_bind({"dcn3_kernel<stats>"}, dcn3_kernel<T, MT, CK, MARGIN, 1, WDMA, NP, PK, F16IN, true>).launch(dim3(grid.x), dim3(C::THREADS), 0, st, a);
             }
         }
+        if constexpr (WDMA && NP > 0 && sizeof(T) == 2 && MT == 2 && e == 2) {
+            if (a.up.out && !stats) {
+                const h3d_kname fname{"dcn3_kernel", h3d_tag<T>{}, MT, CK, MARGIN, e, WDMA, NP, h3d_opt(PK), h3d_opt(F16IN), h3d_opt(false), h3d_opt(true)};
+                if (fname.dry()) return H3D_OK;
+                if (folded) *folded = true;
+                return h3d_bind(fname, dcn3_kernel<T, MT, CK, MARGIN, 2, WDMA, NP, PK, F16IN, false, true>).launch(grid, dim3(C::THREADS), 0, st, a);
+            }
+        }
         if constexpr (F16IN && e != 2) {
             if (name.dry()) return H3D_OK;
             H3D_FAIL(H3D_ERR_UNSUPPORTED, "dcn_fused_stream with an fp16 input: needs an NHWC output with Cout %% 8 == 0 (Cout=%d)", a.Cout);
@@ -876,6 +887,7 @@
     bool narrow_wg;
     bool stats;
     bool dcn5;
+    bool *folded;
     int margin;
     bool raw_pack, scaled_input;
 };
@@ -916,16 +928,16 @@
         if (f.wide_margin)
             return dcn_by_mt(op.Cout, mt2, [&](auto mt) {
                 constexpr int MT = decltype(mt)::value;
-                return launch_dcn3_cfg<T, MT, 16, 4, true, 256, MT < 4, MT >= 2 && F16IN>(a, st, f.stats);
+                return launch_dcn3_cfg<T, MT, 16, 4, true, 256, MT < 4, MT >= 2 && F16IN>(a, st, f.stats, f.folded);
             });
         if (f.slots512)
             return dcn_by_mt(op.Cout, mt2, [&](auto mt) {
                 constexpr int MT = decltype(mt)::value;
-                return launch_dcn3_cfg<T, MT, 16, MT < 4 ? 2 : 4, true, 512, MT < 4, MT >= 2 && F16IN>(a, st, f.stats);
+                return launch_dcn3_cfg<T, MT, 16, MT < 4 ? 2 : 4, true, 512, MT < 4, MT >= 2 && F16IN>(a, st, f.stats, f.folded);
             });
         return dcn_by_mt(op.Cout, mt2, [&](auto mt) {
             constexpr int MT = decltype(mt)::value;
-            return launch_dcn3_cfg<T, MT, 16, MT < 4 ? 2 : 4, true, 256, false, MT >= 2 && F16IN>(a, st, f.stats);
+            return launch_dcn3_cfg<T, MT, 16, MT < 4 ? 2 : 4, true, 256, false, MT >= 2 && F16IN>(a, st, f.stats, f.folded);
         });
     }
     const bool mt2 = op.Cout <= 64 || f.narrow_wg;
@@ -935,7 +947,33 @@
 
 int h3d_launch_dcn5(const h3d_op &op, hipStream_t st);
 
-int h3d_launch_dcn3(const h3d_op &op, hipStream_t st)
+static int launch_dcn3(const h3d_op &op, hipStream_t st, const UpFoldArgs &up, bool *folded);
+int h3d_launch_dcn3(const h3d_op &op, hipStream_t st) { return launch_dcn3(op, st, UpFoldArgs{}, nullptr); }
+
+int h3d_launch_dcn3_fold(const h3d_op &op, const h3d_op &up, hipStream_t st, bool *folded)
+{
+    *folded = false;
+    UpFoldArgs u = {};
+    const int f = up.stride;
+    const bool f16out = up.out_mode == H3D_OUT_NHWC_F16;
+    const bool ok = (op.dtype == H3D_BF16 || op.dtype == H3D_F16) && up.dtype == op.dtype && up.in && up.w && up.out && up.in2 == op.out &&
+                    (up.out_mode == H3D_OUT_NHWC || (f16out && op.dtype == H3D_BF16)) && op.out_mode == H3D_OUT_NHWC &&
+                    up.B == op.B && up.Ho == op.H && up.Wo == op.W && up.Cin == op.Cout && up.Cout == op.Cout && up.in2_cs == op.out_cs &&
+                    (f == 2 || f == 4 || f == 8) && up.ksize == 2 * f && up.Ho == up.H * f && up.Wo == up.W * f &&
+                    op.Cout % 8 == 0 && up.in_cs % 8 == 0 && up.out_cs % 8 == 0 && up.in_cs >= up.Cin && up.out_cs >= up.Cout &&
+                    ((uintptr_t)up.in & 15) == 0 && ((uintptr_t)up.out & 15) == 0 && ((uintptr_t)up.w & 15) == 0 &&
+                    (size_t)up.H * up.W * up.in_cs * 2 < 0x7fffffffull && (size_t)up.Ho * up.Wo * up.out_cs * 2 < 0x7fffffffull &&
+                    (size_t)up.W * up.in_cs * 2 < (1u << 24) && (size_t)up.Wo * up.out_cs * 2 < (1u << 24) && up.ksize * up.ksize * up.Cin < (1 << 24);
+    if (ok) {
+        u.x = (const char *)up.in; u.w = (const float *)up.w; u.out = (char *)up.out;
+        u.H = up.H; u.W = up.W; u.x_cs = up.in_cs; u.out_cs = up.out_cs; u.C = up.Cin;
+        u.fs = f == 2 ? 1 : f == 4 ? 2 : 3;
+        u.f16out = f16out;
+    }
+    return launch_dcn3(op, st, u, folded);
+}
+
+static int launch_dcn3(const h3d_op &op, hipStream_t st, const UpFoldArgs &up, bool *folded)
 {
     const bool wdma = op.kind == H3D_OP_DCN_FUSED_STREAM;
     if (wdma && op.dtype != H3D_BF16 && op.dtype != H3D_F16 && op.dtype != H3D_F16X3) H3D_FAIL(H3D_ERR_DTYPE, "dcn_fused_stream: bf16 / fp16 / f16x3 plans only");
@@ -952,8 +990,10 @@
     a.oscale = ldexpf(1.f, -op.wexp2);
     a.wmax = nullptr;
     a.xscaled = 0;
+    a.up = up;
     if (wdma && (size_t)op.H * op.W * op.in_cs * es >= 0x7ffffff0ull) H3D_FAIL(H3D_ERR_SHAPE, "dcn_fused_stream: image of 2 GiB or more");
-    const Dcn3Flags f = dcn3_decode(op, wdma);
+    Dcn3Flags f = dcn3_decode(op, wdma);
+    f.folded = folded;
     if (f.f16_input) return launch_dcn3_lowp<bf16_t, true>(op, f, a, wdma, st);
     if (f.dcn5) {
 #ifdef H3D_EXTRA
diff --git a/human-3d-reconstruction_amd/csrc/epilogue.h b/human-3d-reconstruction_amd/csrc/epilogue.h
--- a/human-3d-reconstruction_amd/csrc/epilogue.h
+++ b/human-3d-reconstruction_amd/csrc/epilogue.h
@@ -99,9 +99,41 @@
 
 template <int MT, int NT = 1> constexpr int epi_lds_stride() { return (NT * 32 * (64 * MT + 16) + 1023) / 1024 * 1024; }
 
-template <typename T, int MT, int NT, bool HASRES>
+template <typename T, typename WS>
+__device__ __forceinline__ u32x4 upadd_vec(WS w, const bool (&ok)[4], const u32x4 (&xv)[4], const u32x4 &sv, bool f16out)
+{
+    constexpr int N = 16 / sizeof(T);
+    float acc[N], x[N];
+#pragma unroll
+    for (int n = 0; n < N; ++n) acc[n] = 0.f;
+#pragma unroll
+    for (int q = 0; q < 4; ++q) {
+        if (!ok[q]) continue;
+        unpack16<T>(xv[q], x);
+#pragma unroll
+        for (int n = 0; n < N; ++n) acc[n] = fmaf(w(q, n), x[n], acc[n]);
+    }
+    unpack16<T>(sv, x);
+#pragma unroll
+    for (int n = 0; n < N; ++n) acc[n] += x[n];
+    if constexpr (sizeof(T) == 2) {
+        if (f16out) return pack16_f16(acc);
+    }
+    return pack16<T>(acc);
+}
+
+struct UpFoldArgs {
+    const char *x;
+    const float *w;
+    char *out;
+    int H, W, x_cs, out_cs, C;
+    int fs;
+    int f16out;
+};
+
+template <typename T, int MT, int NT, bool HASRES, bool FOLD = false>
 __device__ __forceinline__ void tile_epilogue_lds_impl(f32x16 (&acc)[MT][NT], const EpiArgs &a, int b, int oy0, int ox0,
-                                                       int cout0, int wv, int l, char *lw)
+                                                       int cout0, int wv, int l, char *lw, const UpFoldArgs &u = UpFoldArgs{})
 {
     constexpr int ROWB = 64 * MT + 16;
     constexpr int SPP = 4 * MT;
@@ -123,6 +155,37 @@
         __builtin_amdgcn_s_waitcnt(0x0f70);
         __builtin_amdgcn_wave_barrier();
     }
+    [[maybe_unused]] u32x4 fxv[2][4];
+    [[maybe_unused]] bool fok[2][4];
+    [[maybe_unused]] int fwo[2][4];
+    [[maybe_unused]] const char *fxb = nullptr;
+    [[maybe_unused]] int fxrow = 0, fxpx = 0, fch = 0;
+    if constexpr (FOLD) {
+        static_assert(64 % SPP == 0, "a lane keeps its 16-byte slot through the store iterations");
+        fxb = u.x + (size_t)b * u.H * u.W * u.x_cs * 2;
+        fxrow = u.W * u.x_cs * 2;
+        fxpx = u.x_cs * 2;
+        fch = cout0 + (l % SPP) * 8;
+    }
+    [[maybe_unused]] auto fold_fetch = [&](int it) {
+        const int p = it * (64 / SPP) + l / SPP;
+        const int oy = oy0 + 2 * NT * wv + (p >> 4), ox = ox0 + (p & 15);
+        const bool live = oy < a.Ho && ox < a.Wo && fch < a.Cout;
+        const int f = 1 << u.fs;
+        const int ry = (oy + (f >> 1)) & (f - 1), rx = (ox + (f >> 1)) & (f - 1);
+        const int iy0 = (oy + (f >> 1)) >> u.fs, ix0 = (ox + (f >> 1)) >> u.fs;
+        const int off00 = (int)(__umul24(iy0, fxrow) + __umul24(ix0, fxpx)) + fch * 2;
+        const int w00 = (int)__umul24((ry << (u.fs + 1)) + rx, u.C);
+#pragma unroll
+        for (int t = 0; t < 4; ++t) {
+            const int iy = iy0 - (t >> 1), ix = ix0 - (t & 1);
+            const bool ok = live && (unsigned)iy < (unsigned)u.H && (unsigned)ix < (unsigned)u.W;
+            fok[it & 1][t] = ok;
+            fwo[it & 1][t] = w00 + (((t >> 1) << (2 * u.fs + 1)) + ((t & 1) << u.fs)) * u.C;
+            if (ok) fxv[it & 1][t] = *reinterpret_cast<const u32x4 *>(fxb + (off00 - (t >> 1) * fxrow - (t & 1) * fxpx));
+        }
+    };
+    if constexpr (FOLD) fold_fetch(0);
     {
         const float *bp = a.bias + cout0 + 4 * h;
         const float lo = a.relu ? 0.f : -__builtin_inff();
@@ -154,6 +217,24 @@
     }
     __builtin_amdgcn_s_waitcnt(0xc07f);
     __builtin_amdgcn_wave_barrier();
+    if constexpr (FOLD) {
+        char *ob = u.out + (size_t)b * a.Ho * a.Wo * u.out_cs * 2;
+        const int orow = a.Wo * u.out_cs * 2, opx = u.out_cs * 2;
+        const float *wb = u.w + fch;
+#pragma unroll
+        for (int it = 0; it < NT * SPP / 2; ++it) {
+            if (it + 1 < NT * SPP / 2) fold_fetch(it + 1);
+            const int p = it * (64 / SPP) + l / SPP;
+            const int oy = oy0 + 2 * NT * wv + (p >> 4), ox = ox0 + (p & 15);
+            if (oy < a.Ho && ox < a.Wo && fch < a.Cout) {
+                const u32x4 v = *reinterpret_cast<const u32x4 *>(lw + p * ROWB + (l % SPP) * 16);
+                const auto &wo = fwo[it & 1];
+                *reinterpret_cast<u32x4 *>(ob + (int)(__umul24(oy, orow) + __umul24(ox, opx)) + fch * 2) =
+                    upadd_vec<T>([&](int q, int n) { return wb[wo[q] + n]; }, fok[it & 1], fxv[it & 1], v, u.f16out != 0);
+            }
+        }
+        return;
+    }
 #pragma unroll
     for (int it = 0; it < NT * SPP / 2; ++it) {
         const int q = it * 64 + l;
@@ -175,3 +256,11 @@
     if (a.res) tile_epilogue_lds_impl<T, MT, NT, true>(acc, a, b, oy0, ox0, cout0, wv, l, lw);
     else tile_epilogue_lds_impl<T, MT, NT, false>(acc, a, b, oy0, ox0, cout0, wv, l, lw);
 }
+
+template <typename T, int MT, int NT = 1>
+__device__ __forceinline__ void tile_epilogue_lds_fold(f32x16 (&acc)[MT][NT], const EpiArgs &a, const UpFoldArgs &u, int b, int oy0, int ox0,
+                                                       int cout0, int wv, int l, char *lw)
+{
+    static_assert(sizeof(T) == 2, "2-byte NHWC outputs");
+    tile_epilogue_lds_impl<T, MT, NT, false, true>(acc, a, b, oy0, ox0, cout0, wv, l, lw, u);
+}
diff --git a/human-3d-reconstruction_amd/csrc/ops.hip b/human-3d-reconstruction_amd/csrc/ops.hip
--- a/human-3d-reconstruction_amd/csrc/ops.hip
+++ b/human-3d-reconstruction_amd/csrc/ops.hip
@@ -62,13 +62,23 @@
 int h3d_launch_heads(const h3d_op &op, hipStream_t st);
 int h3d_launch_dcn2(const h3d_op &op, hipStream_t st);
 int h3d_launch_dcn3(const h3d_op &op, hipStream_t st);
+int h3d_launch_dcn3_fold(const h3d_op &op, const h3d_op &up, hipStream_t st, bool *folded);
 int h3d_launch_conv_stream(const h3d_op &op, hipStream_t st);
 int h3d_launch_dcn4(const h3d_op &op, hipStream_t st);
 int h3d_launch_updcn(const h3d_op &op, hipStream_t st);
 int h3d_launch_stem3(const h3d_op &op, hipStream_t st);
 int h3d_launch_extra(const h3d_op &op, hipStream_t st);
 
-static int run_one(const h3d_op &op, int i, hipStream_t st);
+static int run_one(const h3d_op &op, int i, hipStream_t st, const h3d_op *up = nullptr, bool *folded = nullptr);
+
+static int run_at(const h3d_op *ops, int i, int n, hipStream_t st, bool *folded)
+{
+    *folded = false;
+    if (i + 1 < n && ops[i].kind == H3D_OP_DCN_FUSED_STREAM && ops[i + 1].kind == H3D_OP_UPADD && (ops[i + 1].reserved & H3D_OPF_UPADD_FOLDED) &&
+        ops[i].out && ops[i + 1].in2 == ops[i].out)
+        return run_one(ops[i], i, st, &ops[i + 1], folded);
+    return run_one(ops[i], i, st);
+}
 
 extern "C" int h3d_op_kernel_name(const h3d_op *op, char *buf, int buflen)
 {
@@ -90,13 +100,23 @@
     for (int i = 0; i <= n; ++i) (void)hipEventCreate(&ev[i]);
     int rc = H3D_OK;
     (void)hipEventRecord(ev[0], st);
+    for (int i = 0; i < n; ++i) ms[i] = 0.f;
     for (int i = 0; i < n && rc == H3D_OK; ++i) {
-        rc = run_one(ops[i], i, st);
+        bool folded = false;
+        rc = run_at(ops, i, n, st, &folded);
         (void)hipEventRecord(ev[i + 1], st);
+        if (folded) {
+            ++i;
+            ms[i] = -1.f;
+            (void)hipEventRecord(ev[i + 1], st);
+        }
     }
     if (rc == H3D_OK) {
         (void)hipEventSynchronize(ev[n]);
-        for (int i = 0; i < n; ++i) (void)hipEventElapsedTime(&ms[i], ev[i], ev[i + 1]);
+        for (int i = 0; i < n; ++i) {
+            if (ms[i] < 0.f) ms[i] = 0.f;
+            else (void)hipEventElapsedTime(&ms[i], ev[i], ev[i + 1]);
+        }
     }
     for (int i = 0; i <= n; ++i) (void)hipEventDestroy(ev[i]);
     free(ev);
@@ -108,13 +128,15 @@
     if (!ops || n < 0) H3D_FAIL(H3D_ERR_ARG, "run_ops: null plan");
     hipStream_t st = (hipStream_t)stream;
     for (int i = 0; i < n; ++i) {
-        const int rc = run_one(ops[i], i, st);
+        bool folded = false;
+        const int rc = run_at(ops, i, n, st, &folded);
         if (rc != H3D_OK) return rc;
+        if (folded) ++i;
     }
     return H3D_OK;
 }
 
-static int run_one(const h3d_op &op, int i, hipStream_t st)
+static int run_one(const h3d_op &op, int i, hipStream_t st, const h3d_op *up, bool *folded)
 {
     int rc;
     if (op.B <= 0 || op.H <= 0 || op.W <= 0 || op.Ho <= 0 || op.Wo <= 0 || op.Cin <= 0 || op.Cout <= 0) {
@@ -139,7 +161,7 @@
         return H3D_ERR_UNSUPPORTED;
 #endif
     case H3D_OP_DCN_FUSED:
-    case H3D_OP_DCN_FUSED_STREAM: rc = h3d_launch_dcn3(op, st); break;
+    case H3D_OP_DCN_FUSED_STREAM: rc = up ? h3d_launch_dcn3_fold(op, *up, st, folded) : h3d_launch_dcn3(op, st); break;
     case H3D_OP_HEADS: rc = h3d_launch_heads(op, st); break;
     case H3D_OP_MAXPOOL:
     case H3D_OP_UPADD:
diff --git a/human-3d-reconstruction_amd/detector.py b/human-3d-reconstruction_amd/detector.py
--- a/human-3d-reconstruction_amd/detector.py
+++ b/human-3d-reconstruction_amd/detector.py
@@ -121,6 +121,7 @@
         if opt.arch.replace("-", "_") in ("dla_34", "dla34") and opt.dtype in ("bf16", "f16"):
             self.model.engine_flags["split_heads"] = tuple(h for h in opt.heads if h in WHOLE_MAP_HEADS)
             self.model.engine_flags["peak_heads"] = tuple(h for h in opt.heads if h in PEAK_HEADS)
+            self.model.engine_flags["fold_upadd"] = True
         if opt.smpl and smpl_model is None:
             self.smpl_model = _smpl.SMPLModel.synthetic()
 
diff --git a/human-3d-reconstruction_amd/plan.py b/human-3d-reconstruction_amd/plan.py
--- a/human-3d-reconstruction_amd/plan.py
+++ b/human-3d-reconstruction_amd/plan.py
@@ -52,6 +52,7 @@
         conv1x1_th16_min_cin=0,
         lower_heads=True,
         split_heads=(),
+        fold_upadd=False,
         peak_heads=(),
     )
 
@@ -169,12 +170,15 @@
         self._op(_lib.OP_MAXPOOL, x, out, ksize=2, stride=2)
         return out
 
-    def upadd(self, x, skip, wkey, f16=False):
+    def upadd(self, x, skip, wkey, f16=False, private_skip=False):
         w, k = self.pw.up(wkey)
         f = k // 2
         out = self._alloc(x.H * f, x.W * f, x.C)
         assert (skip.H, skip.W, skip.C) == (out.H, out.W, out.C), wkey
-        self._op(_lib.OP_UPADD, x, out, skip, w=w.data_ptr(), ksize=k, stride=f, out_mode=_lib.OUT_NHWC_F16 if f16 else _lib.OUT_NHWC)
+        fold = (private_skip and self.ops and self.ops[-1].kind == _lib.OP_DCN_FUSED_STREAM and self.ops[-1].out == skip.ptr
+                and (skip.coff, skip.cs) == (0, skip.C))
+        self._op(_lib.OP_UPADD, x, out, skip, w=w.data_ptr(), ksize=k, stride=f, out_mode=_lib.OUT_NHWC_F16 if f16 else _lib.OUT_NHWC,
+                 reserved=_lib.OPF_UPADD_FOLDED if fold else 0)
         return out
 
     def _block(self, x, p, stride, residual, out):
@@ -263,16 +267,21 @@
             self.dcn_layers.append((p, i))
         return out
 
-    def _ida(self, layers, p, startp, endp):
+    def _ida_projs(self, layers, p, startp, endp):
+        return [self._deform(layers[i], "%s.proj_%d" % (p, i - startp)) for i in range(startp + 1, endp)]
+
+    def _ida(self, layers, p, startp, endp, private=(), projs=None):
+        if self.fold_upadd and projs is None:
+            projs = self._ida_projs(layers, p, startp, endp)
         for i in range(startp + 1, endp):
             k = i - startp
-            y = self._deform(layers[i], "%s.proj_%d" % (p, k))
+            y = projs[k - 1] if projs is not None else self._deform(layers[i], "%s.proj_%d" % (p, k))
             f16 = self._dcn_f16_ok("%s.node_%d" % (p, k))
             if f16 and self.fuse_upnode and self.pw.up("%s.up_%d.weight" % (p, k))[1] // 2 >= self.fuse_upnode_min_f:
                 layers[i] = self._updcn(y, layers[i - 1], "%s.up_%d.weight" % (p, k), "%s.node_%d" % (p, k))
                 continue
             nf16 = not f16 and self._node_f16_ok("%s.node_%d" % (p, k))
-            y = self.upadd(y, layers[i - 1], "%s.up_%d.weight" % (p, k), f16=f16 or nf16)
+            y = self.upadd(y, layers[i - 1], "%s.up_%d.weight" % (p, k), f16=f16 or nf16, private_skip=self.fold_upadd and k in private)
             layers[i] = self._deform(y, "%s.node_%d" % (p, k), x_is_f16=f16, in_f16=nf16)
 
     def _updcn(self, x, skip, wkey, p):
@@ -315,11 +324,16 @@
         y5 = self._tree1(y4, "base.level5", C[4], C[5], 2, True, None)
         layers = [y0, y1, y2, y3, y4, y5]
         outs = [layers[-1]]
+        pre = None
         for i in range(3):
-            self._ida(layers, "dla_up.ida_%d" % i, len(layers) - i - 2, len(layers))
+            startp, private = len(layers) - i - 2, ()
+            if self.fold_upadd and i == 2:
+                pre = self._ida_projs([None, outs[0], outs[1]], "ida_up", 0, 3)
+                private = tuple(range(2, len(layers) - startp))
+            self._ida(layers, "dla_up.ida_%d" % i, startp, len(layers), private=private)
             outs.insert(0, layers[-1])
         ys = [outs[0], outs[1], outs[2]]
-        self._ida(ys, "ida_up", 0, 3)
+        self._ida(ys, "ida_up", 0, 3, private=(1, 2), projs=pre)
         self.feat = ys[-1]
         if self.lower_heads:
             self._lower_heads(self.feat)
diff --git a/include/h3d.h b/include/h3d.h
--- a/include/h3d.h
+++ b/include/h3d.h
@@ -229,7 +229,8 @@
 
 enum {
     H3D_TUNE_UPADD_TAPS_GLOBAL = 1,
-    H3D_TUNE_UPADD_TAPS_LDS = 2
+    H3D_TUNE_UPADD_TAPS_LDS = 2,
+    H3D_OPF_UPADD_FOLDED = 0x100
 };
 
 enum {
```

After: 10870 images/s (median of 6 runs). +2.2%, better.
